# pszenher/Distributional_RL_Decision_and_Control

Measured on AMD Instinct MI355X. Metric: env-steps/sec/GPU @4096 envs; IQN learn-steps/sec at 1/2/4/8 GPUs, higher is better.
Workload: dtype f64-env/bf16-learner; 1 GPU; BASELINE config 2: 4096 envs x 5 robots, 4 buoys, 55m map; fused rollout + AC-IQN learn (B=4096, N=N'=32) per step; envs_per_gpu=4096, robots=5, obstacles=4, global_batch=4096, num_tau=32, parallelism=dp1, hip_graphs=True, dp_rehearsal=False, unroll=2, chained=True, fused_reset=True, env_groups=0, target_after_env=False, push_after_actor=True, target_in_fused=True

## Files before the change

distributional_rl_decision_and_control_amd/_abi.py:

```python
import ctypes as C
import os

import numpy as np

HERE = os.path.dirname(os.path.abspath(__file__))
LIB_PATH = os.environ.get("ASVRL_LIB", os.path.join(HERE, "lib", "libasvrl.so"))
LIB_PATH_F32 = os.path.join(HERE, "lib", "libasvrl_f32.so")
OPERANDS = {"bf16": (LIB_PATH, 2), "f32": (LIB_PATH_F32, 4)}
ABI_VERSION = 29

SELF_DIM, OBJ_DIM, MAX_OBJ = 7, 5, 5
OBS_DIM = 40
TR_DIM = 88
PER_DIM = 48

F_X, F_Y, F_THETA, F_VR0, F_VR1, F_VR2, F_V0, F_V1, F_V2, F_TL, F_TR, F_LP, F_RP, F_GX, F_GY, F_PHI, F_RET = range(17)
NUM_FIELDS = 17

FLAG_DEACTIVATED, FLAG_COLLISION, FLAG_REACH_GOAL, FLAG_COLREGS = 1, 2, 4, 8

INFO_NORMAL, INFO_TOO_LONG, INFO_COLLISION, INFO_REACH_GOAL, INFO_DEACT_COLLISION, INFO_DEACT_GOAL = range(6)
INFO_ABSENT = 255
INFO_STRINGS = {
    INFO_NORMAL: "normal",
# ... 25 lines not shown
    _fields_ = [("n_envs", C.c_int32), ("max_robots", C.c_int32), ("max_obs", C.c_int32), ("max_cores", C.c_int32),
                ("rs", C.c_void_p), ("rflags", C.c_void_p), ("n_robots", C.c_void_p), ("n_obs", C.c_void_p),
                ("n_cores", C.c_void_p), ("ep_ts", C.c_void_p), ("obstacles", C.c_void_p), ("cores", C.c_void_p),
                ("robot_params", C.c_void_p)]


class AsvStepCtl(C.Structure):
    _fields_ = [("is_continuous", C.c_int32), ("do_dynamics", C.c_int32), ("trainer_deactivate", C.c_int32),
                ("noise_mode", C.c_int32), ("seed", C.c_uint64), ("counter", C.c_uint64),
                ("counter_dev", C.c_void_p), ("gamma", C.c_double), ("env_mask", C.c_void_p)]


class AsvStepOut(C.Structure):
    _fields_ = [("obs", C.c_void_p), ("obs64", C.c_void_p), ("obj_cnt", C.c_void_p), ("reward", C.c_void_p),
                ("done", C.c_void_p), ("info", C.c_void_p), ("env_done", C.c_void_p), ("stats", C.c_void_p)]


class AsvResetCfg(C.Structure):
    _fields_ = [("num_robots", C.c_int32), ("num_obs", C.c_int32), ("num_cores", C.c_int32), ("_pad0", C.c_int32),
                ("min_start_goal_dis", C.c_double), ("width", C.c_double), ("height", C.c_double),
                ("clear_r", C.c_double), ("obs_r_lo", C.c_double), ("obs_r_hi", C.c_double), ("v_lo", C.c_double),
                ("v_hi", C.c_double), ("v_rel_max", C.c_double), ("p_rel", C.c_double)]


class AsvEnvLaunch(C.Structure):
    _fields_ = [("layout", C.c_int32), ("block", C.c_int32), ("envs_per_block", C.c_int32), ("max_groups", C.c_int32)]


ENV_LAYOUT_AUTO, ENV_LAYOUT_PAIRS, ENV_LAYOUT_SWEEP = 0, 1, 2


class AsvRollout(C.Structure):
    _fields_ = [("n_steps", C.c_int32), ("hold_done", C.c_int32)] + \
               [(n, C.c_void_p) for n in ("actions", "noise", "reward", "done", "info", "env_done", "obs", "obj_cnt",
                                          "rs", "steps_run")]


class AsvCriticWeights(C.Structure):
    _fields_ = [(n, C.c_void_p) for n in ("wc_frag", "w1_frag", "w2_frag", "w2t_frag", "w1t_frag", "bc", "b1", "b2",
                                          "wo", "bo", "self_w", "self_b", "obj_w", "obj_b", "ae_w", "ae_b")]


class AsvCriticActs(C.Structure):
    _fields_ = [(n, C.c_void_p) for n in ("cos", "h0", "dzc", "h1g", "dz1", "h2", "dz2", "dq", "wout_part")]


class AsvCriticParts(C.Structure):
    _fields_ = [(n, C.c_void_p) for n in ("cos_emb", "hidden", "hidden2", "out", "enc", "aenc")]


_VP, _I32, _I64, _U64, _F, _D = C.c_void_p, C.c_int32, C.c_int64, C.c_uint64, C.c_float, C.c_double
_SCHEDULE = [("step_dev", _VP), ("eps_steps_per_count", _D), ("eps_total", _D), ("eps_fraction", _D),
             ("eps_initial", _D), ("eps_final", _D), ("seed", _U64)]


def fill_schedule(s, step_dev, eps, seed):
    s.step_dev = step_dev.data_ptr() if step_dev is not None else None
    s.eps_steps_per_count, s.eps_total, s.eps_fraction, s.eps_initial, s.eps_final = (float(v) for v in eps)
    s.seed = int(seed) & 0xFFFFFFFFFFFFFFFF


class AsvCriticIO(C.Structure):
    _fields_ = [("F", _VP), ("G", _VP), ("obs", _VP), ("ld_obs", _I64), ("act", _VP), ("ld_act", _I64), ("xb", _VP),
                ("taus", _VP), ("B", _I32), ("N", _I32), ("Np", _I32), ("kappa", C.c_float),
                ("q_targets", _VP), ("q_next", _VP), ("rewards", _VP), ("dones", _VP), ("ld_rd", _I64),
                ("gamma", C.c_float), ("dq", C.c_float), ("q", _VP), ("row_loss", _VP), ("dF", _VP), ("dG", _VP),
                ("dzF", _VP), ("dzG", _VP), ("w_ae", _VP), ("dA", _VP), ("tile_loss", _VP),
                ("loss_scale", C.c_float)]


IQN_MAX_ACTIONS = 32


class AsvIqnHead(C.Structure):
    _fields_ = [("wo_frag", _VP), ("wo", _VP), ("bo", _VP), ("n_actions", _I32)]


class AsvIqnIO(C.Structure):
    _fields_ = [("F", _VP), ("obs", _VP), ("ld_obs", _I64), ("xb", _VP), ("taus", _VP), ("B", _I32), ("N", _I32),
                ("Np", _I32), ("kappa", C.c_float), ("q_next", _VP), ("actions", _VP), ("rewards", _VP),
                ("dones", _VP), ("ld_rd", _I64),
                ("gamma", C.c_float), ("q", _VP), ("row_loss", _VP), ("dzF", _VP), ("dz_out", _VP),
                ("tile_loss", _VP), ("loss_scale", C.c_float), ("act_out", _VP), ("ld_act", _I64)] + _SCHEDULE


class AsvIqnActEx(C.Structure):
    _fields_ = [("cvar", C.c_float), ("robots_per_env", _I32), ("step_add", _I64), ("act_pair", _VP),
                ("rec_row", _VP), ("env_mask", _VP), ("qmean_out", _VP), ("ld_q", _I64)]


class AsvIqnPolicy(C.Structure):
    _fields_ = [("w", AsvCriticWeights), ("head", AsvIqnHead), ("obs_in", _VP)] + _SCHEDULE + \
               [("actions", _VP), ("cvar", C.c_float), ("_pad0", _I32)]


MAX_SUM_SEGS = 24


SUM_PLAIN, SUM_FOLD_ENCODERS = 0, 1


MAX_WGRAD_SEGS = 24
MAX_PACK_SEGS = 16


class AsvPackSeg(C.Structure):
    _fields_ = [("flat_off", _I64), ("image", _VP), ("rows", _I32), ("cols", _I32), ("K", _I32), ("chained", _I32),
                ("transposed", _I32), ("f32", _I32), ("row0", _I32), ("col0", _I32), ("nrep", _I32),
                ("rep_row", _I32), ("rep_col", _I32), ("reserved", _I32)]
WGRAD_MFMA, WGRAD_VEC, WGRAD_SMALL = 0, 1, 2


class AsvWgradSeg(C.Structure):
    _fields_ = [("dz", _VP), ("ldz", _I64), ("x", _VP), ("ldx", _I64), ("R", _I32), ("M", _I32), ("K", _I32),
                ("kind", _I32), ("partial", _VP), ("partial_floats", _I64)]


class AsvActorGradIO(C.Structure):
    _fields_ = [(n, _VP) for n in ("xb", "h0", "h1", "h2", "dout", "dz2", "dz1", "dz0")] + \
               [("B", _I32), ("n_loss", _I32)] + \
               [(n, _VP) for n in ("tile_loss", "loss_out", "w1_grad", "b1_grad", "w2_grad", "b2_grad", "wo_grad",
                                   "bo_grad", "enc_grad", "norm_parts", "step", "work")] + \
               [("work_floats", _I64), ("counters", _VP)]


class AsvPartialSum(C.Structure):
    _fields_ = [("partial", _VP), ("dw", _VP), ("db", _VP), ("groups", _I32), ("nw", _I32), ("nb", _I32),
                ("accumulate", _I32), ("stride", _I32), ("boff", _I32), ("mode", _I32), ("norm", _I32)]


class AsvMlpSrc(C.Structure):
    _fields_ = [(n, _VP) for n in ("self_w", "self_b", "obj_w", "obj_b", "w1", "w2", "ae_w")]


class AsvMlpWeights(C.Structure):
    _fields_ = [(n, _VP) for n in ("enc_frag", "b_enc", "w1_frag", "w2_frag", "w2t_frag", "w1t_frag", "b1", "b2",
                                   "wout", "bout", "ae_frag", "b_ae")] + [("out_scale", C.c_float)]


class AsvMlpIO(C.Structure):
    _fields_ = [("x", _VP), ("ldx", _I64), ("act", _VP), ("lda", _I64), ("n", _I32), ("F", _VP), ("G", _VP),
                ("xb", _VP), ("a_out", _VP), ("ld_aout", _I64), ("a_out64", _VP), ("pre", _VP), ("h0", _VP),
                ("h1", _VP), ("h2", _VP), ("dA", _VP), ("dout", _VP), ("dz2", _VP), ("dz1", _VP), ("dz0", _VP)] + \
        _SCHEDULE


class AsvPolicy(C.Structure):
    _fields_ = [("w", AsvMlpWeights), ("obs_in", _VP)] + _SCHEDULE + [("actions", _VP)]


class AsvAutoReset(C.Structure):
    _fields_ = [("cfg", AsvResetCfg), ("reset_counter", _U64), ("obs_counter", _U64), ("obs_in", _VP),
                ("obs_prev", _VP), ("pushed", _VP), ("resets", _VP)]


class AsvEvalMetrics(C.Structure):
    _fields_ = [("n_steps", _I32), ("n_envs", _I32), ("max_robots", _I32), ("episode_limit", _I32), ("gamma", _D)] + \
               [(n, _VP) for n in ("reward", "info", "rs", "steps_run", "n_robots", "dt", "N", "pc", "length", "ended",
                                   "alive", "deact", "outcome", "ret", "time", "energy")]


HISTORY_ROW_TILE, HISTORY_STEP_TILE = 32, 16
TRAJ_DIM, HISTORY_OBS_DIM = 13, 32
TRAJ_FIELDS = (F_X, F_Y, F_THETA, F_VR0, F_VR1, F_VR2, F_V0, F_V1, F_V2, F_LP, F_RP, F_TL, F_TR)
HISTORY_ARRAYS = ("info", "length", "n_robots", "counts", "offsets", "rs0", "rs", "actions", "obs0", "obs", "cnt0",
                  "obj_cnt", "traj", "act", "obs_out", "cnt_out")


class AsvEvalHistory(C.Structure):
    _fields_ = [("n_steps", _I32), ("n_envs", _I32), ("max_robots", _I32), ("act_steps", _I32)] + \
               [(n, _VP) for n in HISTORY_ARRAYS] + [("traj_rows", _I64), ("act_rows", _I64), ("obs_rows", _I64)]


class AsvNoiseStreams(C.Structure):
    _fields_ = [("n_envs", _I32), ("max_robots", _I32), ("max_obs", _I32), ("_pad0", _I32)] + \
               [(n, _VP) for n in ("n_robots", "n_obs", "rflags", "env_mask", "robot_params", "key", "pos", "has_gauss",
                                   "gauss", "noise_out", "draws_n", "draws_sum", "draws_sq")]


RS_KEY_WORDS = 624


DQN_MAX_ACTIONS = 32


class AsvDqnWeights(C.Structure):
    _fields_ = [("trunk", AsvMlpWeights), ("head_frag", _VP), ("n_actions", _I32), ("_pad0", _I32)]


class AsvDqnActIO(C.Structure):
    _fields_ = [("x", _VP), ("ldx", _I64), ("n", _I32), ("_pad0", _I32), ("act_out", _VP), ("ld_act", _I64),
                ("q_out", _VP)] + _SCHEDULE


class AsvDqnPolicy(C.Structure):
    _fields_ = [("w", AsvDqnWeights), ("obs_in", _VP)] + _SCHEDULE + [("actions", _VP)]


DQN_GRAD_ARRAYS = ("xb", "h0", "h1", "h2", "q_sel", "q_next", "dz_out", "dz2", "dz1", "dz0", "tile_loss")


class AsvDqnGradIO(C.Structure):
    _fields_ = [("rows", _VP), ("ld_rows", _I64), ("B", _I32), ("gamma", _F)] + [(n, _VP) for n in DQN_GRAD_ARRAYS]


class AsvDdpgWeights(C.Structure):
    _fields_ = [("trunk", AsvMlpWeights), ("wae", _VP), ("bae", _VP)]


DDPG_GRAD_ARRAYS = ("xb", "h0", "h1", "p", "h2", "q", "q_next", "dq", "dz2", "dz1", "dzG", "dz0", "tile_loss")


class AsvDdpgGradIO(C.Structure):
    _fields_ = [("rows", _VP), ("ld_rows", _I64), ("B", _I32), ("gamma", _F), ("na", _VP), ("ld_na", _I64)] + \
               [(n, _VP) for n in DDPG_GRAD_ARRAYS]


class AsvDdpgActorIO(C.Structure):
    _fields_ = [("x", _VP), ("ldx", _I64), ("act", _VP), ("lda", _I64), ("B", _I32), ("_pad0", _I32), ("q", _VP),
                ("dA", _VP), ("tile_loss", _VP)]


class AsvSacActorWeights(C.Structure):
    _fields_ = [("trunk", AsvMlpWeights), ("head", _VP), ("bhead", _VP)]


class AsvSacActIO(C.Structure):
    _fields_ = [("x", _VP), ("ldx", _I64), ("n", _I32), ("_pad0", _I32), ("a_out64", _VP), ("eps_in", _VP),
                ("eps_out", _VP)] + _SCHEDULE


class AsvSacPolicy(C.Structure):
    _fields_ = [("w", AsvSacActorWeights), ("obs_in", _VP)] + _SCHEDULE + \
               [("actions", _VP), ("deterministic", _I32), ("_pad0", _I32)]


SAC_ACTOR_ARRAYS = ("xb", "h0", "h1", "h2", "mu", "ls", "sigma", "z", "a", "eps", "logp", "na", "logp_next",
                    "eps_next", "dA", "q_pi", "dhead", "dz2", "dz1", "dz0", "tile_loss")


class AsvSacActorIO(C.Structure):
    _fields_ = [("rows", _VP), ("ld_rows", _I64), ("B", _I32), ("alpha", _F), ("eps_local_in", _VP),
                ("eps_target_in", _VP), ("seed", _U64), ("counter", _U64), ("counter_dev", _VP)] + \
               [(n, _VP) for n in SAC_ACTOR_ARRAYS]


class AsvSacGradIO(C.Structure):
    _fields_ = [("c", AsvDdpgGradIO * 2), ("logp_next", _VP), ("y", _VP), ("alpha", _F), ("_pad0", _I32)]


class AsvSacActorGradIO(C.Structure):
    _fields_ = [("x", _VP), ("ldx", _I64), ("act", _VP), ("lda", _I64), ("B", _I32), ("_pad0", _I32), ("q_pi", _VP),
                ("dA", _VP)]


class AsvSampleArgs(C.Structure):
    _fields_ = [("ring", _VP), ("capacity", _I64), ("ring_state", _VP), ("seed", _U64), ("counter", _U64),
                ("counter_dev", _VP), ("guard", _I64), ("B", _I32), ("tau_sets", _I32), ("tau_n", _I32),
                ("_pad0", _I32), ("out", _VP), ("taus", _VP)]


class AsvPer(C.Structure):
    _fields_ = [("rows", _VP), ("tree", _VP), ("state", _VP), ("t", _VP), ("maxp", _VP), ("dirty", _VP),
                ("capacity", _I64), ("tree_leaves", _I64), ("stride", _I32), ("n_step", _I32), ("discount", _D),
                ("priority_weight", C.c_float), ("priority_exponent", C.c_float), ("deferred", _I32),
                ("_pad0", _I32)]


MAX_NOISY_SEGS = 16


class AsvNoisySeg(C.Structure):
    _fields_ = [(n, _VP) for n in ("mu", "sigma", "eps", "out", "dout", "dmu", "dsigma")]


class AsvNoisySegs(C.Structure):
    _fields_ = [("n", _I32), ("_pad0", _I32), ("off", _I64 * (MAX_NOISY_SEGS + 1)),
                ("seg", AsvNoisySeg * MAX_NOISY_SEGS)]


class AsvRainbowHeadIO(C.Structure):
    _fields_ = [("v", _VP), ("ldv", _I64), ("a", _VP), ("lda", _I64), ("N", _I32), ("atoms", _I32),
                ("actions_n", _I32), ("_pad0", _I32), ("support", _VP), ("act_out", _VP), ("ld_act", _I64),
                ("act_idx", _VP)] + _SCHEDULE + \
               [("p_out", _VP), ("actions", _VP), ("weights", _VP), ("ld_rd", _I64), ("m", _VP), ("loss", _VP),
                ("dv", _VP), ("da", _VP), ("grad_scale", C.c_float), ("_pad1", _I32)]


class AsvRainbowSrc(C.Structure):
    _fields_ = [(n, _VP) for n in ("self_w", "self_b", "obj_w", "obj_b", "w_v1", "b_v1", "w_a1", "b_a1", "w_v2", "b_v2",
                                   "w_a2", "b_a2", "w_vo", "b_vo", "w_ao", "b_ao")]


RAINBOW_IMG_FIELDS = ("enc", "v1", "a1", "v2", "a2", "vo", "mo", "ao")
RAINBOW_BIAS_FIELDS = ("b_enc", "b_v1p", "b_a1p", "b_v2p", "b_a2p", "b_vop", "b_mop", "b_aop")
RAINBOW_IMGT_FIELDS = ("vot", "mot", "aot", "v2t", "a2t", "v1t", "a1t")


class AsvRainbowImg(C.Structure):
    _fields_ = [(n, _VP) for n in RAINBOW_IMG_FIELDS + RAINBOW_BIAS_FIELDS + RAINBOW_IMGT_FIELDS]


class AsvRainbowNetIO(C.Structure):
    _fields_ = [("x", _VP), ("ldx", _I64), ("N", _I32), ("_pad0", _I32), ("support", _VP), ("act_out", _VP),
                ("ld_act", _I64), ("act_idx", _VP)] + _SCHEDULE + \
               [("p_out", _VP), ("actions", _VP), ("weights", _VP), ("ld_rd", _I64), ("m", _VP), ("grad_scale", _F),
                ("_pad1", _I32), ("loss", _VP)] + \
               [(n, _VP) for n in ("xb", "f", "hv1", "ha1", "hv2", "ha2", "dzv", "dza", "dz2v", "dz2a", "dz1v", "dz1a",
                                   "dzf")]


class AsvRainbowActEx(C.Structure):
    _fields_ = [("robots_per_env", _I32), ("_pad0", _I32), ("step_add", _I64), ("act_pair", _VP), ("rec_row", _VP),
                ("env_mask", _VP), ("q_out", _VP), ("ld_q", _I64)]


class AsvRainbowPolicy(C.Structure):
    _fields_ = [("w", AsvRainbowImg), ("support", _VP), ("obs_in", _VP)] + _SCHEDULE + [("actions", _VP)]


ROLLOUTS = {"actor": ("asvrl_policy_rollout", AsvPolicy), "dqn": ("asvrl_dqn_rollout", AsvDqnPolicy),
            "sac": ("asvrl_sac_rollout", AsvSacPolicy), "iqn": ("asvrl_iqn_rollout", AsvIqnPolicy),
            "rainbow": ("asvrl_rainbow_rollout", AsvRainbowPolicy)}


def _rollout_exports():
    head = [C.POINTER(t) for t in (AsvParams, AsvEnvState, AsvStepCtl, AsvStepOut, AsvRollout)]
    tail = [C.POINTER(AsvEnvLaunch), _VP]
    for name, policy in ROLLOUTS.values():
        yield name, C.c_int, head + [C.POINTER(policy)] + tail
        yield name + "_ar", C.c_int, head + [C.POINTER(policy), C.POINTER(AsvAutoReset)] + tail


EXPORTS = [
    ("asvrl_env_step", C.c_int, [C.POINTER(AsvParams), C.POINTER(AsvEnvState), _VP, _VP, C.POINTER(AsvStepCtl),
                                 C.POINTER(AsvStepOut), _VP]),
    ("asvrl_env_step_ex", C.c_int, [C.POINTER(AsvParams), C.POINTER(AsvEnvState), _VP, _VP, C.POINTER(AsvStepCtl),
                                    C.POINTER(AsvStepOut), C.POINTER(AsvEnvLaunch), _VP]),
    ("asvrl_env_rollout", C.c_int, [C.POINTER(AsvParams), C.POINTER(AsvEnvState), C.POINTER(AsvStepCtl),
                                    C.POINTER(AsvStepOut), C.POINTER(AsvRollout), C.POINTER(AsvEnvLaunch), _VP]),
    ("asvrl_env_reset", C.c_int, [C.POINTER(AsvParams), C.POINTER(AsvEnvState), C.POINTER(AsvResetCfg), _VP, _U64,
                                  _U64, _VP, _VP]),
    ("asvrl_env_reset_observe", C.c_int, [C.POINTER(AsvParams), C.POINTER(AsvEnvState), C.POINTER(AsvResetCfg), _VP,
                                          _U64, _U64, _VP, C.POINTER(AsvStepCtl), C.POINTER(AsvStepOut), _VP]),
    ("asvrl_current_field", C.c_int, [_VP, _I32, _D, _VP, _I32, _VP, _VP]),
    ("asvrl_quantile_huber", C.c_int, [_VP, _VP, _VP, _I32, _I32, _I32, _F, _F, _VP, _VP, _VP, _VP]),
    ("asvrl_c51_project", C.c_int, [_VP, _VP, _VP, _VP, _I32, _I32, _F, _F, _F, _F, _VP, _VP]),
    ("asvrl_c51_project_ex", C.c_int, [_VP, _VP, C.c_int64, _VP, C.c_int64, _VP, _I32, _I32, _F, _F, _F, _F, _VP,
                                       _VP]),
    ("asvrl_critic_pack", C.c_int, [_VP, _VP, _VP, C.POINTER(AsvCriticWeights), _VP]),
    ("asvrl_critic_forward", C.c_int, [C.POINTER(AsvCriticWeights), C.POINTER(AsvCriticIO), _VP]),
    ("asvrl_critic_train", C.c_int, [C.POINTER(AsvCriticWeights), C.POINTER(AsvCriticIO), C.POINTER(AsvCriticActs),
                                     _VP]),
    ("asvrl_critic_actor_grad", C.c_int, [C.POINTER(AsvCriticWeights), C.POINTER(AsvCriticIO), _VP]),
    ("asvrl_iqn_pack", C.c_int, [_VP, _VP, _VP, _VP, C.POINTER(AsvCriticWeights), C.POINTER(AsvIqnHead), _VP]),
    ("asvrl_iqn_forward_max", C.c_int, [C.POINTER(AsvCriticWeights), C.POINTER(AsvIqnHead), C.POINTER(AsvIqnIO), _VP]),
    ("asvrl_iqn_train", C.c_int, [C.POINTER(AsvCriticWeights), C.POINTER(AsvIqnHead), C.POINTER(AsvIqnIO),
                                  C.POINTER(AsvCriticActs), _VP]),
    ("asvrl_iqn_act", C.c_int, [C.POINTER(AsvCriticWeights), C.POINTER(AsvIqnHead), C.POINTER(AsvIqnIO), _VP]),
    ("asvrl_replay_push", C.c_int, [_VP, _VP, _VP, _VP, _I32, _VP, _VP, _I32, _VP, _I64, _VP, _VP, _VP]),
    ("asvrl_replay_push_ex", C.c_int, [_VP, _VP, _VP, _VP, _I32, _I64, _VP, _VP, _I32, _VP, _I64, _VP, _VP, _VP,
                                       _VP, _VP]),
    ("asvrl_replay_sample", C.c_int, [_VP, _I64, _VP, _VP, _I32, _U64, _U64, _VP, _I64, _VP, _VP, _VP, _I32, _I32,
                                      _VP]),
    ("asvrl_replay_write_rows", C.c_int, [_VP, _VP, _I32, _VP, _VP]),
    ("asvrl_per_push", C.c_int, [C.POINTER(AsvPer), _VP, _VP, _VP, _I32, _VP, _VP, _I32, _VP]),
    ("asvrl_per_sample", C.c_int, [C.POINTER(AsvPer), _I32, _VP, _U64, _U64, _VP, _VP, _VP, _VP]),
    ("asvrl_per_update", C.c_int, [C.POINTER(AsvPer), _VP, _VP, _I32, _I32, _VP]),
    ("asvrl_per_push_ex", C.c_int, [C.POINTER(AsvPer), _VP, _VP, _VP, _I32, _VP, _VP, _I32, _VP, _VP]),
    ("asvrl_per_update_ex", C.c_int, [C.POINTER(AsvPer), _VP, _VP, _I32, _I32, _VP, _VP, _VP]),
    ("asvrl_per_sample_ex", C.c_int, [C.POINTER(AsvPer), _I32, _VP, _U64, _U64, _VP, _VP, _VP, _VP, _VP]),
    ("asvrl_per_normalise", C.c_int, [_VP, _VP, _I32, _VP]),
    ("asvrl_noisy_compose", C.c_int, [C.POINTER(AsvNoisySegs), _I32, _VP]),
    ("asvrl_noisy_backward_norm_parts", _I32, [C.POINTER(AsvNoisySegs)]),
    ("asvrl_noisy_backward_norm", C.c_int, [C.POINTER(AsvNoisySegs), _VP, _VP]),
    ("asvrl_noisy_reset", C.c_int, [C.POINTER(AsvNoisySegs), _VP, _VP, _U64, _VP, _VP]),
    ("asvrl_rainbow_act", C.c_int, [C.POINTER(AsvRainbowHeadIO), _VP]),
    ("asvrl_rainbow_pick", C.c_int, [C.POINTER(AsvRainbowHeadIO), _VP]),
    ("asvrl_rainbow_loss", C.c_int, [C.POINTER(AsvRainbowHeadIO), _VP]),
    ("asvrl_rainbow_pack", C.c_int, [C.POINTER(AsvRainbowSrc), C.POINTER(AsvRainbowImg), _VP]),
    ("asvrl_rainbow_net_act", C.c_int, [C.POINTER(AsvRainbowImg), C.POINTER(AsvRainbowNetIO), _VP]),
    ("asvrl_rainbow_net_argmax", C.c_int, [C.POINTER(AsvRainbowImg), C.POINTER(AsvRainbowNetIO), _VP]),
    ("asvrl_rainbow_net_pick", C.c_int, [C.POINTER(AsvRainbowImg), C.POINTER(AsvRainbowNetIO), _VP]),
    ("asvrl_rainbow_net_train", C.c_int, [C.POINTER(AsvRainbowImg), C.POINTER(AsvRainbowNetIO), _VP]),
    ("asvrl_adam_clip", C.c_int, [_VP, _VP, _VP, _VP, _I64, _VP, _F, _F, _F, _F, _F, _VP, _VP, _VP]),
    ("asvrl_linear_wgrad_workspace", _I64, [_I32, _I32]),
    ("asvrl_critic_wout_groups", _I32, [_I32, _I32]),
    ("asvrl_critic_fused_groups", _I32, [_I32, _I32]),
    ("asvrl_critic_fused_variant", _I32, [_I32]),
    ("asvrl_critic_train_fused", C.c_int, [C.POINTER(AsvCriticWeights), C.POINTER(AsvCriticIO),
                                           C.POINTER(AsvCriticParts), _VP]),
    ("asvrl_critic_train_fused_tq", C.c_int, [C.POINTER(AsvCriticWeights), C.POINTER(AsvCriticIO),
                                              C.POINTER(AsvCriticParts), C.POINTER(AsvCriticWeights),
                                              C.POINTER(AsvCriticIO), _VP]),
    ("asvrl_iqn_train_fused", C.c_int, [C.POINTER(AsvCriticWeights), C.POINTER(AsvIqnHead), C.POINTER(AsvIqnIO),
                                        C.POINTER(AsvCriticParts), _VP]),
    ("asvrl_iqn_train_fused_tq", C.c_int, [C.POINTER(AsvCriticWeights), C.POINTER(AsvIqnHead), C.POINTER(AsvIqnIO),
                                           C.POINTER(AsvCriticParts), C.POINTER(AsvCriticWeights),
                                           C.POINTER(AsvIqnHead), C.POINTER(AsvIqnIO), _VP]),
    ("asvrl_linear_wgrad_groups", _I32, [_I32, _I32, _I32]),
    ("asvrl_linear_wgrad_vec_groups", _I32, [_I32]),
    ("asvrl_linear_wgrad_partial", C.c_int, [_VP, _I64, _VP, _I64, _I32, _I32, _I32, _VP, _I64, _VP, _VP]),
    ("asvrl_linear_wgrad_multi", C.c_int, [_VP, _I32, _VP, _VP]),
    ("asvrl_linear_wgrad_vec_partial", C.c_int, [_VP, _I64, _VP, _I64, _I32, _I32, _VP, _I64, _VP, _VP]),
    ("asvrl_small_wgrad_partial", C.c_int, [_VP, _I64, _VP, _I64, _I32, _I32, _I32, _VP, _I64, _VP, _VP]),
    ("asvrl_partial_sums", C.c_int, [_VP, _I32, _VP]),
    ("asvrl_partial_sums_norm", C.c_int, [_VP, _I32, _VP, _VP, _VP]),
    ("asvrl_partial_sums_norm_parts", _I32, [_VP, _I32]),
    ("asvrl_actor_grads_workspace", _I64, [_I32]),
    ("asvrl_actor_grads_counters", _I32, []),
    ("asvrl_actor_grads_norm_parts", _I32, []),
    ("asvrl_actor_grads", C.c_int, [C.POINTER(AsvActorGradIO), _VP]),
    ("asvrl_adam_step", C.c_int, [_VP, _VP, _VP, _VP, _I64, _VP, _F, _F, _F, _F, _F, _VP, _VP, _I32, _VP]),
    ("asvrl_adam_step_pack", C.c_int, [_VP, _VP, _VP, _VP, _I64, _VP, _F, _F, _F, _F, _F, _VP, _VP, _I32, _VP, _I32,
                                       _VP, _VP]),
    ("asvrl_target_update_pack", C.c_int, [_VP, _VP, _I64, _F, _F, _VP, _I64, _VP, _I32, _VP]),
    ("asvrl_linear_wgrad", C.c_int, [_VP, _I64, _VP, _I64, _I32, _I32, _I32, _VP, _VP, _I32, _VP, _I64, _VP]),
    ("asvrl_linear_wgrad_vec", C.c_int, [_VP, _I64, _VP, _I64, _I32, _I32, _VP, _VP, _I32, _VP, _I64, _VP]),
    ("asvrl_mlp_pack", C.c_int, [C.POINTER(AsvMlpSrc), C.POINTER(AsvMlpWeights), _VP]),
    ("asvrl_mlp_encode", C.c_int, [C.POINTER(AsvMlpWeights), C.POINTER(AsvMlpIO), _VP]),
    ("asvrl_actor_forward", C.c_int, [C.POINTER(AsvMlpWeights), C.POINTER(AsvMlpIO), _I32, _VP]),
    ("asvrl_actor_backward", C.c_int, [C.POINTER(AsvMlpWeights), C.POINTER(AsvMlpIO), _VP]),
    ("asvrl_learn_prologue", C.c_int, [C.POINTER(AsvSampleArgs), C.POINTER(AsvMlpWeights), C.POINTER(AsvMlpIO),
                                       C.POINTER(AsvMlpWeights), _VP, _VP]),
    ("asvrl_encoder_fold", C.c_int, [_VP, _VP, _VP, _VP, _VP, _VP, _I32, _VP]),
    ("asvrl_small_wgrad", C.c_int, [_VP, _I64, _VP, _I64, _I32, _I32, _I32, _VP, _VP, _I32, _VP, _I64, _VP]),
    ("asvrl_last_error", C.c_char_p, []),
    ("asvrl_abi_version", C.c_int, []),
    ("asvrl_operand_bytes", C.c_int32, []),
    ("asvrl_struct_sizes", None, [C.c_void_p]),
    ("asvrl_rollout_struct_size", _I64, []),
    *_rollout_exports(),
    ("asvrl_policy_struct_size", _I64, []),
    ("asvrl_env_rollout_ar", C.c_int, [C.POINTER(AsvParams), C.POINTER(AsvEnvState), C.POINTER(AsvStepCtl),
                                       C.POINTER(AsvStepOut), C.POINTER(AsvRollout), C.POINTER(AsvAutoReset),
                                       C.POINTER(AsvEnvLaunch), _VP]),
    ("asvrl_autoreset_struct_size", _I64, []),
    ("asvrl_replay_push_window", C.c_int, [_VP, _VP, _VP, _VP, _I32, _I64, _VP, _VP, _I32, _I32, _VP, _VP, _I64, _VP,
                                           _VP, _VP, _VP, _I64, _VP]),
    ("asvrl_eval_metrics", C.c_int, [C.POINTER(AsvEvalMetrics), _VP]),
    ("asvrl_eval_metrics_struct_size", _I64, []),
    ("asvrl_eval_history_count", C.c_int, [C.POINTER(AsvEvalHistory), _VP]),
    ("asvrl_eval_history_pack", C.c_int, [C.POINTER(AsvEvalHistory), _VP]),
    ("asvrl_eval_history_struct_size", _I64, []),
    ("asvrl_eval_history_step_tile", _I32, []),
    ("asvrl_noise_streams", C.c_int, [C.POINTER(AsvParams), C.POINTER(AsvNoiseStreams), _VP]),
    ("asvrl_noise_streams_host", C.c_int, [C.POINTER(AsvParams), C.POINTER(AsvNoiseStreams), _VP]),
    ("asvrl_noise_streams_struct_size", _I64, []),
    ("asvrl_dqn_pack", C.c_int, [C.POINTER(AsvMlpSrc), _VP, C.POINTER(AsvDqnWeights), _VP]),
    ("asvrl_dqn_act", C.c_int, [C.POINTER(AsvDqnWeights), C.POINTER(AsvDqnActIO), _VP]),
    ("asvrl_dqn_grad", C.c_int, [C.POINTER(AsvDqnWeights), C.POINTER(AsvDqnWeights), C.POINTER(AsvDqnGradIO), _VP]),
    ("asvrl_dqn_weights_struct_size", _I64, []),
    ("asvrl_dqn_act_struct_size", _I64, []),
    ("asvrl_dqn_grad_struct_size", _I64, []),
    ("asvrl_dqn_policy_struct_size", _I64, []),
    ("asvrl_ddpg_grad", C.c_int, [C.POINTER(AsvDdpgWeights), C.POINTER(AsvDdpgWeights), C.POINTER(AsvDdpgGradIO),
                                  _VP]),
    ("asvrl_ddpg_actor_grad", C.c_int, [C.POINTER(AsvDdpgWeights), C.POINTER(AsvDdpgActorIO), _VP]),
    ("asvrl_ddpg_weights_struct_size", _I64, []),
    ("asvrl_ddpg_grad_struct_size", _I64, []),
    ("asvrl_ddpg_actor_struct_size", _I64, []),
    ("asvrl_sac_act", C.c_int, [C.POINTER(AsvSacActorWeights), C.POINTER(AsvSacActIO), _VP]),
    ("asvrl_sac_actor_forward", C.c_int, [C.POINTER(AsvSacActorWeights), C.POINTER(AsvSacActorWeights),
                                          C.POINTER(AsvSacActorIO), _VP]),
    ("asvrl_sac_grad", C.c_int, [C.POINTER(AsvDdpgWeights), C.POINTER(AsvDdpgWeights), C.POINTER(AsvDdpgWeights),
                                 C.POINTER(AsvDdpgWeights), C.POINTER(AsvSacGradIO), _VP]),
    ("asvrl_sac_actor_grad", C.c_int, [C.POINTER(AsvDdpgWeights), C.POINTER(AsvDdpgWeights),
                                       C.POINTER(AsvSacActorGradIO), _VP]),
    ("asvrl_sac_actor_backward", C.c_int, [C.POINTER(AsvSacActorWeights), C.POINTER(AsvSacActorIO), _VP]),
    ("asvrl_sac_actor_weights_struct_size", _I64, []),
    ("asvrl_sac_act_struct_size", _I64, []),
    ("asvrl_sac_actor_struct_size", _I64, []),
    ("asvrl_sac_grad_struct_size", _I64, []),
    ("asvrl_sac_actor_grad_struct_size", _I64, []),
    ("asvrl_sac_policy_struct_size", _I64, []),
    ("asvrl_iqn_act_ex", C.c_int, [C.POINTER(AsvCriticWeights), C.POINTER(AsvIqnHead), C.POINTER(AsvIqnIO),
                                   C.POINTER(AsvIqnActEx), _VP]),
    ("asvrl_iqn_act_ex_struct_size", _I64, []),
    ("asvrl_iqn_policy_struct_size", _I64, []),
    ("asvrl_rainbow_net_act_ex", C.c_int, [C.POINTER(AsvRainbowImg), C.POINTER(AsvRainbowNetIO),
                                           C.POINTER(AsvRainbowActEx), _VP]),
    ("asvrl_rainbow_act_ex_struct_size", _I64, []),
    ("asvrl_rainbow_policy_struct_size", _I64, []),
    ("asvrl_per_push_window", C.c_int, [C.POINTER(AsvPer), _VP, _VP, _VP, _I32, _VP, _VP, _I32, _VP, _I64, _VP]),
]

_libs = {}


class AsvrlError(RuntimeError):
    pass


def lib(operands="bf16"):
    L = _libs.get(operands)
    if L is not None:
        return L
    if operands not in OPERANDS:
        raise ValueError(f"operands must be one of {sorted(OPERANDS)}")
    path, nbytes = OPERANDS[operands]
    if not os.path.exists(path):
        raise AsvrlError(f"{os.path.basename(path)} not found at {path}: build it with "
                         "`python -m distributional_rl_decision_and_control_amd.build` (hipcc, gfx950). "
                         "There is no CPU fallback.")
    L = C.CDLL(path)
    for name, res, args in EXPORTS:
        fn = getattr(L, name)
        fn.restype = res
        fn.argtypes = args
    v = L.asvrl_abi_version()
    if v != ABI_VERSION:
        raise AsvrlError(f"{os.path.basename(path)} ABI {v} != expected {ABI_VERSION}; rebuild")
    if L.asvrl_operand_bytes() != nbytes:
        raise AsvrlError(f"{path}: operand element of {L.asvrl_operand_bytes()} bytes, expected {nbytes}")
    _libs[operands] = L
    return L


def operand_dtype(operands="bf16"):
    import torch
    return {"bf16": torch.bfloat16, "f32": torch.float32}[operands]


def check(rc, what="", L=None):
    if rc != 0:
        msg = (L if L is not None else lib()).asvrl_last_error().decode(errors="replace")
        raise AsvrlError(f"{what} failed ({rc}): {msg}")


def ptr(t):
    if t is None:
        return None
    return C.c_void_p(t.data_ptr())


def stream_ptr(stream=None):
    import torch
    s = stream if stream is not None else torch.cuda.current_stream()
    return C.c_void_p(s.cuda_stream)


def params_from(robot=None, env=None, max_obj_num=5, episode_limit=1000):
    p = AsvParams()
    src = robot if robot is not None else _DefaultRobot()
    p.dt = float(src.dt)
    p.N = int(src.N)
    p.episode_limit = int(episode_limit)
    p.length, p.width = float(src.length), float(src.width)
    p.r = float(src.r)
    p.goal_dis = float(src.goal_dis)
    p.min_thrust, p.max_thrust = float(src.min_thrust), float(src.max_thrust)
    p.m, p.Izz = float(src.m), float(src.Izz)
    for n in _HYDRO:
        setattr(p, n, float(getattr(src, n)))
    import warnings
    warnings.filterwarnings("ignore", category=PendingDeprecationWarning, message=".*matrix subclass.*")
    M_RB = np.matrix([[src.m, 0.0, 0.0], [0.0, src.m, 0.0], [0.0, 0.0, src.Izz]])
    M_A = -1.0 * np.matrix([[src.xDotU, 0.0, 0.0], [0.0, src.yDotV, src.yDotR], [0.0, src.nDotV, src.nDotR]])
    A = M_RB + M_A
    P = np.asarray(np.linalg.inv(A.transpose() * A) * A.transpose(), dtype=np.float64).reshape(-1)
    for k in range(9):
        p.P[k] = float(P[k])
    for k in range(5):
        p.left_thrust_change[k] = float(src.left_thrust_change[k])
        p.right_thrust_change[k] = float(src.right_thrust_change[k])
    per = src.perception if hasattr(src, "perception") else src
    p.range, p.angle = float(per.range), float(per.angle)
    p.pos_std, p.vel_std = float(per.pos_std), float(per.vel_std)
    p.r_kappa, p.r_mean_ratio = float(per.r_kappa), float(per.r_mean_ratio)
    p.max_obj_num = int(getattr(per, "max_obj_num", max_obj_num))
    e = env if env is not None else _DefaultEnv()
    p.timestep_penalty = float(e.timestep_penalty)
    p.COLREGs_penalty = float(e.COLREGs_penalty)
    p.collision_penalty = float(e.collision_penalty)
    p.goal_reward = float(e.goal_reward)
    p.core_r = float(e.r)
    return p


class _DefaultRobot:
    dt, N, length, width = 0.05, 10, 5.0, 2.5
    r = 0.5 * np.sqrt(5.0 ** 2 + 2.5 ** 2)
    goal_dis, min_thrust, max_thrust = 2.0, -500.0, 1000.0
    m, Izz = 400, 450
    xDotU, yDotV, yDotR, nDotR, nDotV = 20, 0, 0, -980, 0
    xU, xUU, yV, yVV, yR, yRV, yVR, yRR = -100, -150, -100, -150, 0, 0, 0, 0
    nR, nRR, nV, nVV, nRV, nVR = -980, -950, 0, 0, 0, 0
    left_thrust_change = right_thrust_change = [0.0, -500.0, -1000.0, 500.0, 1000.0]
    range, angle, max_obj_num = 20.0, 2 * np.pi, 5
    pos_std, vel_std, r_kappa, r_mean_ratio = 0.05, 0.05, 1.0, 0.8
# ... 6 lines not shown
```

distributional_rl_decision_and_control_amd/csrc/asvrl_env.hip:

```cpp
#include <type_traits>

#include "asvrl_common.h"
#include "asvrl_vonmises_k1.h"
#include "asvrl_actor_tile.h"
#include "asvrl_dqn_tile.h"
#include "asvrl_sac_tile.h"

namespace asvrl {
namespace {

constexpr int kBlock = 256;
__host__ __device__ constexpr int step_block(int R) { return R <= 64 ? 64 : 256; }
__host__ __device__ constexpr size_t policy_rows_offset(size_t carve_bytes) { return (carve_bytes + 15) & ~size_t{15}; }
constexpr int kMaxCores = 16;
constexpr int kMaxCoresStep = 4096;

struct Regs {
  double x, y, th, vr0, vr1, vr2, v0, v1, v2, tl, tr, lp, rp;
};

struct PairsArgs {
  AsvParams p;
  AsvEnvState s;
  AsvStepCtl ctl;
// ... 406 lines not shown
  int cnt = -1;
  Cand t0{INFINITY, 0, 0, 0, 0, 0}, t1 = t0, t2 = t0, t3 = t0, t4 = t0;
  double so0 = 0, so1 = 0, so2 = 0, so3 = 0, so4 = 0;
  if (active) {
    double sn, cs;
    sincos(r.th, &sn, &cs);
    const double tx = -(cs * r.x + sn * r.y);
    const double ty = -(-sn * r.x + cs * r.y);
    so0 = (cs * gx + sn * gy) + tx;
    so1 = (-sn * gx + cs * gy) + ty;
    so2 = cs * r.v0 + sn * r.v1;
    so3 = -sn * r.v0 + cs * r.v1;
    so4 = r.v2;
    if (sqrt((gx - r.x) * (gx - r.x) + (gy - r.y) * (gy - r.y)) <= P.goal_dis) reach = true;

    int nkept = 0;
    const int no = s.n_obs[e];
    const int base = le * R;
    const uint64_t ctr = ctl.counter + (ctl.counter_dev != nullptr ? *ctl.counter_dev : 0ull);
    const int ncand = no + nrob;
    const bool full_circle = 0.5 * P.angle >= kPi;
    for (int k = 0; k < ncand; ++k) {
      double ox, oy, orad, vx0, vy0;
      int slot;
      if (k < no) {
        const double* ob = sob + (static_cast<size_t>(le) * O + k) * 3;
        ox = ob[0];
        oy = ob[1];
        orad = ob[2];
        vx0 = 0.0;
        vy0 = 0.0;
        slot = k;
      } else {
        const int j = k - no;
        if (j == i || soff[base + j]) continue;
        ox = sx[base + j];
        oy = sy[base + j];
        orad = PR ? s.robot_params[static_cast<size_t>(e) * R + j].r : p.r;
        vx0 = sv0[base + j];
        vy0 = sv1[base + j];
        slot = O + j;
      }
      double n0, n1, n2, n3, n4;
      draw_noise<-1>(P, ctl, ctr, noise, idx, slot, O + R, n0, n1, n2, n3, n4);
      const double pxn = ox + n0, pyn = oy + n1;
      const double vxn = vx0 + n2, vyn = vy0 + n3;
      const double rn = P.r_mean_ratio * orad + (1 - P.r_mean_ratio) * n4 / kPi * orad;
      const double qx = (cs * pxn + sn * pyn) + tx, qy = (-sn * pxn + cs * pyn) + ty;
      const double qn = sqrt(qx * qx + qy * qy);
      if (qn > P.range + rn) continue;
      if (!full_circle) {
        const double ang = atan2(qy, qx);
        if (ang < -0.5 * P.angle || ang > 0.5 * P.angle) continue;
      }
      if (!coll) {
        const double d = sqrt((r.x - ox) * (r.x - ox) + (r.y - oy) * (r.y - oy)) - orad - P.r;
        if (d <= 0.0) coll = true;
      }
      Cand cd{qn - rn - P.r, qx, qy, cs * vxn + sn * vyn, -sn * vxn + cs * vyn, rn};
      cswap(cd.key < t0.key, cd, t0);
      cswap(cd.key < t1.key, cd, t1);
      cswap(cd.key < t2.key, cd, t2);
      cswap(cd.key < t3.key, cd, t3);
      cswap(cd.key < t4.key, cd, t4);
      ++nkept;
    }
    cnt = nkept < P.max_obj_num ? nkept : P.max_obj_num;
    if (cnt > 0) apply = colregs(P.r, cs, sn, r.v0, r.v1, t0.a, t0.b, t0.c, t0.d, t0.e, phi);
    if (!apply && cnt > 1) apply = colregs(P.r, cs, sn, r.v0, r.v1, t1.a, t1.b, t1.c, t1.d, t1.e, phi);
    if (!apply && cnt > 2) apply = colregs(P.r, cs, sn, r.v0, r.v1, t2.a, t2.b, t2.c, t2.d, t2.e, phi);
    if (!apply && cnt > 3) apply = colregs(P.r, cs, sn, r.v0, r.v1, t3.a, t3.b, t3.c, t3.d, t3.e, phi);
    if (!apply && cnt > 4) apply = colregs(P.r, cs, sn, r.v0, r.v1, t4.a, t4.b, t4.c, t4.d, t4.e, phi);
  }

  const StepResult res = step_result(p, ctl, exists, deact, active, ep_ts, fl, coll, reach, apply, phi, reward,
                                     exists ? s.rs[ASVRL_F_RET * NT + idx] : 0.0);
  if (ctl.trainer_deactivate && ctl.do_dynamics && exists && !(res.nfl & ASVRL_FLAG_DEACTIVATED))
    atomicAdd(&salive[le], 1);

  if (exists) {
    double* rs = s.rs;
    if (ctl.do_dynamics) {
      rs[ASVRL_F_X * NT + idx] = r.x;
      rs[ASVRL_F_Y * NT + idx] = r.y;
      rs[ASVRL_F_THETA * NT + idx] = r.th;
      rs[ASVRL_F_VR0 * NT + idx] = r.vr0;
      rs[ASVRL_F_VR1 * NT + idx] = r.vr1;
      rs[ASVRL_F_VR2 * NT + idx] = r.vr2;
      rs[ASVRL_F_V0 * NT + idx] = r.v0;
      rs[ASVRL_F_V1 * NT + idx] = r.v1;
      rs[ASVRL_F_V2 * NT + idx] = r.v2;
      rs[ASVRL_F_TL * NT + idx] = r.tl;
      rs[ASVRL_F_TR * NT + idx] = r.tr;
      rs[ASVRL_F_RET * NT + idx] = res.ret;
    }
    rs[ASVRL_F_PHI * NT + idx] = phi;
    s.rflags[idx] = res.nfl;
  }
  if (env_on && i < R) {
    float4* o4 = reinterpret_cast<float4*>(out.obs + idx * ASVRL_OBS_DIM);
    const bool a = active;
    const float m0 = (a && cnt > 0) ? 1.f : 0.f, m1 = (a && cnt > 1) ? 1.f : 0.f,
                m2 = (a && cnt > 2) ? 1.f : 0.f, m3 = (a && cnt > 3) ? 1.f : 0.f,
                m4 = (a && cnt > 4) ? 1.f : 0.f;
    auto f = [](double v, float m) { return m != 0.f ? static_cast<float>(v) : 0.f; };
    const float sf = a ? 1.f : 0.f;
    o4[0] = make_float4(f(so0, sf), f(so1, sf), f(so2, sf), f(so3, sf));
    o4[1] = make_float4(f(so4, sf), f(r.tl, sf), f(r.tr, sf), f(t0.a, m0));
    o4[2] = make_float4(f(t0.b, m0), f(t0.c, m0), f(t0.d, m0), f(t0.e, m0));
    o4[3] = make_float4(f(t1.a, m1), f(t1.b, m1), f(t1.c, m1), f(t1.d, m1));
    o4[4] = make_float4(f(t1.e, m1), f(t2.a, m2), f(t2.b, m2), f(t2.c, m2));
    o4[5] = make_float4(f(t2.d, m2), f(t2.e, m2), f(t3.a, m3), f(t3.b, m3));
    o4[6] = make_float4(f(t3.c, m3), f(t3.d, m3), f(t3.e, m3), f(t4.a, m4));
    o4[7] = make_float4(f(t4.b, m4), f(t4.c, m4), f(t4.d, m4), f(t4.e, m4));
    o4[8] = make_float4(m0, m1, m2, m3);
    o4[9] = make_float4(m4, 0.f, 0.f, 0.f);
    if (out.obs64 != nullptr) {
      double* o = out.obs64 + idx * 32;
      const double v[32] = {so0, so1, so2, so3, so4, r.tl, r.tr,
                            t0.a, t0.b, t0.c, t0.d, t0.e, t1.a, t1.b, t1.c, t1.d, t1.e,
                            t2.a, t2.b, t2.c, t2.d, t2.e, t3.a, t3.b, t3.c, t3.d, t3.e,
                            t4.a, t4.b, t4.c, t4.d, t4.e};
#pragma unroll
      for (int k = 0; k < 32; ++k) {
        const bool keep = a && (k < 7 || (k - 7) / 5 < cnt);
        o[k] = keep ? v[k] : 0.0;
      }
    }
    out.obj_cnt[idx] = static_cast<int8_t>(exists ? cnt : -1);
    out.reward[idx] = res.reward;
    out.done[idx] = res.done;
    out.info[idx] = res.info;
  }
  __syncthreads();
  if (env_on && i == 0 && ctl.do_dynamics) env_end(p, s, ctl, out, e, ep_ts, nrob, salive[le], NT);
}

#ifndef ASVRL_ENV_PAIRS_WPE
#define ASVRL_ENV_PAIRS_WPE 4
#endif
constexpr int kResetWaves = 4;
constexpr int kResetMaxR = 32;
constexpr int kResetMaxO = 32;
struct ResetLds {
  double rob[4][kResetMaxR];
  double core[kMaxCores][4];
  double obs[kResetMaxO][3];
};
__device__ __forceinline__ void reset_env(const AsvParams& p, const AsvEnvState& s, const AsvResetCfg& cfg, int e,
                                          uint64_t seed, uint64_t ctr, int lane, ResetLds& W);
__host__ __device__ constexpr size_t autoreset_lds(int blk, int epb) {
  return static_cast<size_t>(blk / 64) * sizeof(ResetLds) + sizeof(int) * static_cast<size_t>(epb);
}
enum : int { kPolNone = 0, kPolActor = 1, kPolDqn = 2, kPolSac = 3 };
template <int POL> struct PolicyOf { using type = AsvPolicy; };
template <> struct PolicyOf<kPolDqn> { using type = AsvDqnPolicy; };
template <> struct PolicyOf<kPolSac> { using type = AsvSacPolicy; };
__device__ __forceinline__ const AsvMlpWeights& trunk_of(const AsvPolicy& p) { return p.w; }
__device__ __forceinline__ const AsvMlpWeights& trunk_of(const AsvDqnPolicy& p) { return p.w.trunk; }
__device__ __forceinline__ const AsvMlpWeights& trunk_of(const AsvSacPolicy& p) { return p.w.trunk; }
template <int BLOCK, int NM, bool DYN = true, bool ROLL = false, int POL = kPolNone, bool AR = false>
__device__ __forceinline__ void env_pairs_block(KArg<PairsArgs> A, int epb, int bid, unsigned char* smem,
                                                KArg<AsvRollout> RO = nullptr,
                                                KArg<typename PolicyOf<POL>::type> PI = nullptr,
                                                atile::ActorLds* AL = nullptr, KArg<AsvAutoReset> RS = nullptr,
                                                unsigned char* ar_lds = nullptr,
                                                sactile::SacHeadLds* HL = nullptr) {
  static_assert(POL == kPolNone || ROLL, "the policy runs inside the rollout's step loop");
  static_assert(!AR || ROLL, "the auto-reset runs inside the rollout's step loop");
  const int R = A->s.max_robots;
  const int O = A->s.max_obs;
  const int S = O + R;
  const int nrb = epb * R;
  const int npairs = nrb * S;
  const int nslot = npairs > 5 * nrb ? npairs : 5 * nrb;
  int tid = threadIdx.x;

  double* sx = reinterpret_cast<double*>(smem);
  double* sy = sx + nrb;
  double* sv0 = sy + nrb;
  double* sv1 = sv0 + nrb;
  double* scs = sv1 + nrb;
  double* ssn = scs + nrb;
  double* stx = ssn + nrb;
  double* sty = stx + nrb;
  double* pk = sty + nrb;
  double* sob = pk + nslot;
  using VmT = typename std::conditional<NM == 2, float, double>::type;
  VmT* pvm = reinterpret_cast<VmT*>(sob + static_cast<size_t>(epb) * O * 3);
  int* salive = reinterpret_cast<int*>(pvm + npairs);
  int* sno = salive + epb;
  int* snr = sno + epb;
  int* swt = snr + epb;
  unsigned short* skept = reinterpret_cast<unsigned short*>(swt + BLOCK / kWave);
  unsigned short* sitem = skept + 5 * nrb;
  unsigned char* pfl = reinterpret_cast<unsigned char*>(sitem + 5 * nrb);
  unsigned char* soff = pfl + nslot;
  unsigned char* sact = soff + nrb;
  signed char* scnt = reinterpret_cast<signed char*>(sact + nrb);
  float* sobs = reinterpret_cast<float*>(smem + policy_rows_offset(reinterpret_cast<unsigned char*>(scnt + nrb) - smem));
  double* sa64 = reinterpret_cast<double*>(sobs + static_cast<size_t>(nrb) * ASVRL_OBS_DIM);
  const size_t row0 = POL != kPolNone ? static_cast<size_t>(bid) * nrb : 0;

  const bool rlane = tid < nrb;
  int le = tid / R;
  const int i = tid - le * R;
  const int e = bid * epb + le;
  const bool lane_env = rlane && e < A->s.n_envs;
  const bool env_on0 = lane_env && (A->ctl.env_mask == nullptr || A->ctl.env_mask[e] != 0);
  if (A->ctl.env_mask != nullptr && !__syncthreads_or(env_on0 ? 1 : 0)) return;
  int nrob = lane_env ? A->s.n_robots[e] : 0;
  bool exists0 = env_on0 && i < nrob;
  const size_t NT = static_cast<size_t>(A->s.n_envs) * R;
  size_t idx = static_cast<size_t>(e) * R + i;
  uint8_t flv = exists0 ? A->s.rflags[idx] : 0;
  int ep_ts = env_on0 ? A->s.ep_ts[e] : 0;
  Regs r{};
  double gx = 0, gy = 0, phi = 0.0, ret = 0.0;
  bool on = env_on0;
  int taken = 0;
  int nreset = 0;
  bool rstl = false;
  const int n_steps = ROLL ? RO->n_steps : 1;
  const bool hold = ROLL && RO->hold_done != 0;
  auto load_state = [&] {
    const double* rs = A->s.rs;
    r.x = rs[ASVRL_F_X * NT + idx];
    r.y = rs[ASVRL_F_Y * NT + idx];
    r.th = rs[ASVRL_F_THETA * NT + idx];
    r.vr0 = rs[ASVRL_F_VR0 * NT + idx];
    r.vr1 = rs[ASVRL_F_VR1 * NT + idx];
    r.vr2 = rs[ASVRL_F_VR2 * NT + idx];
    r.v0 = rs[ASVRL_F_V0 * NT + idx];
    r.v1 = rs[ASVRL_F_V1 * NT + idx];
    r.v2 = rs[ASVRL_F_V2 * NT + idx];
    r.tl = rs[ASVRL_F_TL * NT + idx];
    r.tr = rs[ASVRL_F_TR * NT + idx];
    r.lp = rs[ASVRL_F_LP * NT + idx];
    r.rp = rs[ASVRL_F_RP * NT + idx];
    gx = rs[ASVRL_F_GX * NT + idx];
    gy = rs[ASVRL_F_GY * NT + idx];
  };
  auto store_state = [&] {
    double* rs = A->s.rs;
    rs[ASVRL_F_X * NT + idx] = r.x;
    rs[ASVRL_F_Y * NT + idx] = r.y;
    rs[ASVRL_F_THETA * NT + idx] = r.th;
    rs[ASVRL_F_VR0 * NT + idx] = r.vr0;
    rs[ASVRL_F_VR1 * NT + idx] = r.vr1;
    rs[ASVRL_F_VR2 * NT + idx] = r.vr2;
    rs[ASVRL_F_V0 * NT + idx] = r.v0;
    rs[ASVRL_F_V1 * NT + idx] = r.v1;
    rs[ASVRL_F_V2 * NT + idx] = r.v2;
    rs[ASVRL_F_TL * NT + idx] = r.tl;
    rs[ASVRL_F_TR * NT + idx] = r.tr;
  };
  if constexpr (ROLL) {
    if (exists0) {
      load_state();
      phi = A->s.rs[ASVRL_F_PHI * NT + idx];
      ret = A->s.rs[ASVRL_F_RET * NT + idx];
    }
  }
  if constexpr (POL != kPolNone) {
    atile::stage_actor<BLOCK>(*AL, trunk_of(kref(PI)), tid);
    if constexpr (POL == kPolSac) sactile::stage_head<BLOCK>(*HL, kref(PI).w, tid);
    constexpr int kRowV = ASVRL_OBS_DIM / 4;
    const float4* src = reinterpret_cast<const float4*>(PI->obs_in);
    for (int k = tid; k < nrb * kRowV; k += BLOCK) {
      const size_t g = row0 + k / kRowV;
      reinterpret_cast<float4*>(sobs)[k] = g < NT ? src[g * kRowV + k % kRowV] : make_float4(0.f, 0.f, 0.f, 0.f);
    }
    __syncthreads();
  }
  if constexpr (AR) {
    const KArg<AsvAutoReset> Q = kfresh(RS);
    const float* src0 = POL != kPolNone ? PI->obs_in : Q->obs_in;
    if (env_on0 && Q->obs_prev != nullptr) {
      const float4* src = reinterpret_cast<const float4*>(src0 + idx * ASVRL_OBS_DIM);
      float4* dst = reinterpret_cast<float4*>(Q->obs_prev + idx * ASVRL_OBS_DIM);
#pragma unroll
      for (int k = 0; k < ASVRL_OBS_DIM / 4; ++k) dst[k] = src[k];
    }
  }

  for (int t = 0; t < n_steps; ++t) {
  if constexpr (ROLL) {
    asm volatile("" : "+v"(tid), "+v"(le), "+v"(idx));
    if (hold && !__syncthreads_or(on ? 1 : 0)) break;
  }
  bool obsp = false;
  [[maybe_unused]] phases:
  if constexpr (AR) asm volatile("" : "+v"(tid), "+v"(le), "+v"(idx));
  const bool env_on = ROLL ? (on && (!obsp || rstl)) : env_on0;
  const bool exists = ROLL ? (exists0 && env_on) : exists0;
  const uint8_t fl = flv;
  const bool deact = (fl & ASVRL_FLAG_DEACTIVATED) != 0;
  const bool active = exists && !deact;
  bool coll = (fl & ASVRL_FLAG_COLLISION) != 0;
  bool reach = (fl & ASVRL_FLAG_REACH_GOAL) != 0;
  double reward = 0.0;
  const bool wlast = !ROLL || hold || t == n_steps - 1;
  auto rec_row = [&] {
    AsvStepOut o{};
    if constexpr (ROLL) {
      const KArg<AsvRollout> Q = kfresh(RO);
      const size_t t0 = static_cast<size_t>(t) * NT;
      o.obs = Q->obs != nullptr ? Q->obs + t0 * ASVRL_OBS_DIM : nullptr;
      o.obj_cnt = Q->obj_cnt != nullptr ? Q->obj_cnt + t0 : nullptr;
      o.reward = Q->reward != nullptr ? Q->reward + t0 : nullptr;
      o.done = Q->done != nullptr ? Q->done + t0 : nullptr;
      o.info = Q->info != nullptr ? Q->info + t0 : nullptr;
    }
    return o;
  };
  auto each_out = [&](KArg<PairsArgs> Ak, auto&& f) {
    if (wlast) f(kref(Ak).out, std::false_type{}, size_t{0});
    if constexpr (AR) {
      if (!obsp) f(rec_row(), std::true_type{}, size_t{0});
    } else if constexpr (ROLL) {
      f(rec_row(), std::true_type{}, size_t{0});
    }
    if constexpr (POL != kPolNone) {
      AsvStepOut o{};
      o.obs = sobs;
      f(o, std::true_type{}, row0);
    }
    if constexpr (AR) {
      const KArg<AsvAutoReset> Q = kfresh(RS);
      AsvStepOut o{};
      if (Q->obs_prev != nullptr && t + 1 < n_steps)
        o.obs = Q->obs_prev + static_cast<size_t>(t + 1) * NT * ASVRL_OBS_DIM;
      f(o, std::true_type{}, size_t{0});
    }
  };

  if constexpr (AR) {
    if (obsp) goto acted;
  }
  if constexpr (POL == kPolActor) {
    const KArg<AsvPolicy> P = kfresh(PI);
    const uint64_t step = (P->step_dev != nullptr ? static_cast<uint64_t>(*P->step_dev) : 0ull) + static_cast<uint64_t>(t);
    const int ln = tid & (kWave - 1), wv = __builtin_amdgcn_readfirstlane(tid / kWave);
    for (int tile = wv; tile * 32 < nrb; tile += BLOCK / kWave) {
      asm volatile("" ::: "memory");
      const int lr = tile * 32 + (ln & 31);
      const bool valid = lr < nrb;
      frag8 bx[2];
      float mk[atile::kObjN];
      atile::load_obs(sobs, ASVRL_OBS_DIM, valid ? lr : nrb - 1, ln >> 5, bx, mk);
      float z0, z1, a0, a1;
      atile::actor_chain<atile::MLP_ACT>(kref(P).w, AsvMlpIO{}, *AL, 0, false, ln, bx, mk, z0, z1, a0, a1);
      if (valid && ln < 32)
        atile::explore(step, atile::EpsSchedule{P->eps_steps_per_count, P->eps_total, P->eps_fraction, P->eps_initial,
                                                P->eps_final},
                       P->seed, static_cast<int>(row0 + lr), a0, a1, sa64[2 * lr], sa64[2 * lr + 1]);
    }
    __syncthreads();
    if (env_on && P->actions != nullptr) {
      double* rec = P->actions + (static_cast<size_t>(t) * NT + idx) * 2;
      rec[0] = sa64[2 * tid];
      rec[1] = sa64[2 * tid + 1];
    }
  } else if constexpr (POL == kPolDqn) {
    const KArg<AsvDqnPolicy> P = kfresh(PI);
    const uint64_t step = (P->step_dev != nullptr ? static_cast<uint64_t>(*P->step_dev) : 0ull) + static_cast<uint64_t>(t);
    const int ln = tid & (kWave - 1), wv = __builtin_amdgcn_readfirstlane(tid / kWave);
    for (int tile = wv; tile * 32 < nrb; tile += BLOCK / kWave) {
      asm volatile("" ::: "memory");
      const int lr = tile * 32 + (ln & 31);
      const bool valid = lr < nrb;
      frag8 bx[2];
      float mk[atile::kObjN];
      atile::load_obs(sobs, ASVRL_OBS_DIM, valid ? lr : nrb - 1, ln >> 5, bx, mk);
      float q[16];
      dqtile::dqn_q_tile<atile::MLP_ACT>(kref(P).w, AsvMlpIO{}, *AL, 0, false, ln, bx, mk, q);
      float best;
      int bi;
      const int nact = P->w.n_actions;
      dqtile::dqn_argmax(q, ln >> 5, nact, best, bi);
      if (valid && ln < 32) {
        const int act = dqtile::dqn_explore(step, atile::EpsSchedule{P->eps_steps_per_count, P->eps_total, P->eps_fraction,
                                                                     P->eps_initial, P->eps_final},
                                            P->seed, static_cast<int>(row0 + lr), bi, nact);
        sa64[2 * lr] = static_cast<double>(act);
        sa64[2 * lr + 1] = 0.0;
      }
    }
    __syncthreads();
    if (env_on && P->actions != nullptr) {
      double* rec = P->actions + (static_cast<size_t>(t) * NT + idx) * 2;
      rec[0] = sa64[2 * tid];
      rec[1] = sa64[2 * tid + 1];
    }
  } else if constexpr (POL == kPolSac) {
    const KArg<AsvSacPolicy> P = kfresh(PI);
    const uint64_t step = (P->step_dev != nullptr ? static_cast<uint64_t>(*P->step_dev) : 0ull) + static_cast<uint64_t>(t);
    const int ln = tid & (kWave - 1), wv = __builtin_amdgcn_readfirstlane(tid / kWave);
    for (int tile = wv; tile * 32 < nrb; tile += BLOCK / kWave) {
      asm volatile("" ::: "memory");
      const int lr = tile * 32 + (ln & 31);
      const bool valid = lr < nrb;
      const int rr = valid ? lr : nrb - 1;
      float eps[atile::kNa] = {0.f, 0.f};
      if (P->deterministic == 0)
        sactile::sac_eps(sactile::kSacActStream, static_cast<int>(row0 + rr), step, P->seed, eps[0], eps[1]);
      frag8 bx[2];
      float mk[atile::kObjN];
      atile::load_obs(sobs, ASVRL_OBS_DIM, rr, ln >> 5, bx, mk);
      float h2v[8][8];
      atile::trunk_chain<atile::MLP_ACT>(kref(P).w.trunk, AsvMlpIO{}, *AL, 0, false, ln, bx, mk, h2v);
      sactile::SacSample o;
      sactile::sac_head<false>(*HL, P->w.trunk.out_scale, h2v, ln, eps, o);
      if (valid && ln < 32)
        atile::explore(step, atile::EpsSchedule{P->eps_steps_per_count, P->eps_total, P->eps_fraction, P->eps_initial,
                                                P->eps_final},
                       P->seed, static_cast<int>(row0 + lr), o.a[0], o.a[1], sa64[2 * lr], sa64[2 * lr + 1]);
    }
    __syncthreads();
    if (env_on && P->actions != nullptr) {
      double* rec = P->actions + (static_cast<size_t>(t) * NT + idx) * 2;
      rec[0] = sa64[2 * tid];
      rec[1] = sa64[2 * tid + 1];
    }
  }
  [[maybe_unused]] acted:

  {
    if constexpr (!ROLL) {
      r = Regs{};
      gx = 0;
      gy = 0;
      if (exists) load_state();
    }
    if (active && (DYN && A->ctl.do_dynamics) && !obsp) {
      const double d_before = sqrt((gx - r.x) * (gx - r.x) + (gy - r.y) * (gy - r.y));
      const int nc = A->s.n_cores[e];
      const double* cores = A->s.cores + static_cast<size_t>(e) * A->s.max_cores * 4;
      const double* act = POL != kPolNone ? sa64 + 2 * tid : A->actions + (ROLL ? static_cast<size_t>(t) * 2 * NT : 0) + 2 * idx;
      robot_act(ParamsKArg{&A->p}, r, act[0], act[1], A->ctl.is_continuous, cores,
                nc < A->s.max_cores ? nc : A->s.max_cores);
      const double d_after = sqrt((gx - r.x) * (gx - r.x) + (gy - r.y) * (gy - r.y));
      reward = 0.0;
      reward += A->p.timestep_penalty;
      reward += d_before - d_after;
    }
    if constexpr (!ROLL) {
      if (exists && (DYN && A->ctl.do_dynamics)) store_state();
    }
    double so0 = 0, so1 = 0, so2 = 0, so3 = 0, so4 = 0;
    if (rlane) {
      sx[tid] = r.x;
      sy[tid] = r.y;
      sv0[tid] = r.v0;
      sv1[tid] = r.v1;
      soff[tid] = exists ? (deact ? 1 : 0) : 1;
      sact[tid] = active ? 1 : 0;
    }
    if (active) {
      double sn, cs;
      sincos(r.th, &sn, &cs);
      const double tx = -(cs * r.x + sn * r.y);
      const double ty = -(-sn * r.x + cs * r.y);
      scs[tid] = cs;
      ssn[tid] = sn;
      stx[tid] = tx;
      sty[tid] = ty;
      so0 = (cs * gx + sn * gy) + tx;
      so1 = (-sn * gx + cs * gy) + ty;
      so2 = cs * r.v0 + sn * r.v1;
      so3 = -sn * r.v0 + cs * r.v1;
      so4 = r.v2;
      if (sqrt((gx - r.x) * (gx - r.x) + (gy - r.y) * (gy - r.y)) <= A->p.goal_dis) reach = true;
    }
    if (env_on) {
      const bool a = active;
      each_out(A, [&](const AsvStepOut& o, auto opt, size_t base) {
        if (!opt || o.obs != nullptr) {
          float* of = o.obs + (idx - base) * ASVRL_OBS_DIM;
          *reinterpret_cast<float4*>(of) = a ? make_float4(static_cast<float>(so0), static_cast<float>(so1),
                                                            static_cast<float>(so2), static_cast<float>(so3))
                                             : make_float4(0.f, 0.f, 0.f, 0.f);
          of[4] = a ? static_cast<float>(so4) : 0.f;
          of[5] = a ? static_cast<float>(r.tl) : 0.f;
          of[6] = a ? static_cast<float>(r.tr) : 0.f;
        }
        if (o.obs64 != nullptr) {
          double* ob = o.obs64 + idx * 32;
          ob[0] = a ? so0 : 0.0;
          ob[1] = a ? so1 : 0.0;
          ob[2] = a ? so2 : 0.0;
          ob[3] = a ? so3 : 0.0;
          ob[4] = a ? so4 : 0.0;
          ob[5] = a ? r.tl : 0.0;
          ob[6] = a ? r.tr : 0.0;
        }
      });
    }
  }
  if (env_on) {
    if (!ROLL || t == 0 || obsp) {
      const int no = A->s.n_obs[e];
      for (int k = i; k < O; k += R) {
        const double* ob = A->s.obstacles + (static_cast<size_t>(e) * O + k) * 3;
        double* dst = sob + (static_cast<size_t>(le) * O + k) * 3;
        if (k < no) {
          dst[0] = ob[0];
          dst[1] = ob[1];
          dst[2] = ob[2];
        }
      }
      if (i == 0) {
        sno[le] = no;
        snr[le] = nrob;
      }
    }
    if (i == 0) salive[le] = 0;
  }
  __syncthreads();
  A = kfresh(A);

  auto candidate = [&](int qe, int qi, int c, double& ox, double& oy, double& orad, double& vx0, double& vy0) {
    if (c < O) {
      if (c >= sno[qe]) return false;
      const double* ob = sob + (static_cast<size_t>(qe) * O + c) * 3;
      ox = ob[0];
      oy = ob[1];
      orad = ob[2];
      vx0 = 0.0;
      vy0 = 0.0;
      return true;
    }
    const int j = c - O;
    if (!(j < snr[qe] && j != qi && !soff[qe * R + j])) return false;
    ox = sx[qe * R + j];
    oy = sy[qe * R + j];
    orad = A->p.r;
    vx0 = sv0[qe * R + j];
    vy0 = sv1[qe * R + j];
    return true;
  };
  uint64_t ctr = A->ctl.counter + (A->ctl.counter_dev != nullptr ? *A->ctl.counter_dev : 0ull) +
                 (ROLL ? static_cast<uint64_t>(t) : 0ull);
  if constexpr (AR) {
    if (obsp) ctr = ctr - A->ctl.counter + RS->obs_counter;
  }
  const size_t noise_t = (ROLL && NM == 0) ? static_cast<size_t>(t) * NT * S * 5 : 0;
  const bool full_circle = 0.5 * A->p.angle >= kPi;

  const KArg<PairsArgs> A_loop = A;
  for (int q = tid; q < npairs; q += BLOCK) {
    const KArg<PairsArgs> A = kfresh(A_loop);
    const int qr = q / S;
    const int c = q - qr * S;
    const int qe = qr / R;
    const int qi = qr - qe * R;
    unsigned char flag = 0;
    double key = INFINITY;
    double ox = 0, oy = 0, orad = 0, vx0 = 0, vy0 = 0;
    if (sact[qr] && candidate(qe, qi, c, ox, oy, orad, vx0, vy0)) {
      const size_t qidx = static_cast<size_t>(bid * epb + qe) * R + qi;
      double n0, n1, n2, n3, n4;
      draw_noise<NM>(kref(A).p, kref(A).ctl, ctr, A->noise + noise_t, qidx, c, S, n0, n1, n2, n3, n4);
      pvm[q] = static_cast<VmT>(n4);
      const double cs = scs[qr], sn = ssn[qr], tx = stx[qr], ty = sty[qr];
      const double pxn = ox + n0, pyn = oy + n1;
      const double rn = A->p.r_mean_ratio * orad + (1 - A->p.r_mean_ratio) * n4 / kPi * orad;
      const double qx = (cs * pxn + sn * pyn) + tx, qy = (-sn * pxn + cs * pyn) + ty;
      const double qn = sqrt(qx * qx + qy * qy);
      bool det = qn <= A->p.range + rn;
      if (det && !full_circle) {
        const double ang = atan2(qy, qx);
        det = !(ang < -0.5 * A->p.angle || ang > 0.5 * A->p.angle);
      }
      if (det) {
        flag = 1;
        const double rx = sx[qr], ry = sy[qr];
        const double d = sqrt((rx - ox) * (rx - ox) + (ry - oy) * (ry - oy)) - orad - A->p.r;
        if (d <= 0.0) flag |= 2;
        key = qn - rn - A->p.r;
      }
    }
    pk[q] = key;
    pfl[q] = flag;
  }
  __syncthreads();
  A = kfresh(A);

  int cnt = -1;
  if (active) {
    double k0 = INFINITY, k1 = INFINITY, k2 = INFINITY, k3 = INFINITY, k4 = INFINITY;
    int c0 = 0, c1 = 0, c2 = 0, c3 = 0, c4 = 0;
    int nkept = 0;
    const int q0 = tid * S;
    for (int c = 0; c < S; ++c) {
      const unsigned char f = pfl[q0 + c];
      if (!(f & 1)) continue;
      if (f & 2) coll = true;
      double kc = pk[q0 + c];
      int cc = c;
      auto ins = [&](double& kk, int& ck) {
        if (kc < kk) {
          const double tk = kk;
          const int tc = ck;
          kk = kc;
          ck = cc;
          kc = tk;
          cc = tc;
        }
      };
      ins(k0, c0);
      ins(k1, c1);
      ins(k2, c2);
      ins(k3, c3);
      ins(k4, c4);
      ++nkept;
    }
    cnt = nkept < A->p.max_obj_num ? nkept : A->p.max_obj_num;
    unsigned short* kp = skept + 5 * tid;
    kp[0] = static_cast<unsigned short>(c0);
    kp[1] = static_cast<unsigned short>(c1);
    kp[2] = static_cast<unsigned short>(c2);
    kp[3] = static_cast<unsigned short>(c3);
    kp[4] = static_cast<unsigned short>(c4);
  }
  if (rlane) scnt[tid] = static_cast<signed char>(cnt);
  const int lane = tid & (kWave - 1);
  int kin = cnt > 0 ? cnt : 0;
#pragma unroll
  for (int d = 1; d < kWave; d <<= 1) {
    const int t = __shfl_up(kin, d);
    if (lane >= d) kin += t;
  }
  if (lane == kWave - 1) swt[tid / kWave] = kin;
  __syncthreads();
  A = kfresh(A);
  int nitem = 0, ibase = 0;
#pragma unroll
  for (int w = 0; w < BLOCK / kWave; ++w) {
    ibase += w < tid / kWave ? swt[w] : 0;
    nitem += swt[w];
  }
  if (cnt > 0) {
    const int off = ibase + kin - cnt;
    for (int k = 0; k < cnt; ++k) sitem[off + k] = static_cast<unsigned short>(5 * tid + k);
  }
  __syncthreads();
  A = kfresh(A);

  const KArg<PairsArgs> A_loop4 = A;
  for (int it = tid; it < nitem; it += BLOCK) {
    const KArg<PairsArgs> A = kfresh(A_loop4);
    const int kq = sitem[it];
    const int qr = kq / 5;
    const int k = kq - 5 * qr;
    const int qe = qr / R;
    const int qi = qr - qe * R;
    const int e2 = bid * epb + qe;
    unsigned char cf = 0;
    double ph = 0.0;
    {
      const size_t qidx = static_cast<size_t>(e2) * R + qi;
      double ra, rb, rc, rd, re;
      {
        const int c = skept[kq];
        double ox = 0, oy = 0, orad = 0, vx0 = 0, vy0 = 0;
        candidate(qe, qi, c, ox, oy, orad, vx0, vy0);
        double n0, n1, n2, n3, n4 = static_cast<double>(pvm[qr * S + c]);
        draw_noise<NM, false>(kref(A).p, kref(A).ctl, ctr, A->noise + noise_t, qidx, c, S, n0, n1, n2, n3, n4);
        const double cs = scs[qr], sn = ssn[qr], tx = stx[qr], ty = sty[qr];
        const double pxn = ox + n0, pyn = oy + n1;
        const double vxn = vx0 + n2, vyn = vy0 + n3;
        const double rn = A->p.r_mean_ratio * orad + (1 - A->p.r_mean_ratio) * n4 / kPi * orad;
        ra = (cs * pxn + sn * pyn) + tx;
        rb = (-sn * pxn + cs * pyn) + ty;
        rc = cs * vxn + sn * vyn;
        rd = -sn * vxn + cs * vyn;
        re = rn;
        if (!(sqrt(rc * rc + rd * rd) < 0.5)) {
          bool ev;
          const bool hit = colregs_ev(A->p.r, cs, sn, sv0[qr], sv1[qr], ra, rb, rc, rd, re, ph, ev);
          cf = static_cast<unsigned char>((ev ? 1 : 0) | (hit ? 2 : 0));
        }
      }
      each_out(A, [&](const AsvStepOut& o, auto opt, size_t base) {
        if (!opt || o.obs != nullptr) {
          float* of = o.obs + (qidx - base) * ASVRL_OBS_DIM + 7 + 5 * k;
          of[0] = static_cast<float>(ra);
          of[1] = static_cast<float>(rb);
          of[2] = static_cast<float>(rc);
          of[3] = static_cast<float>(rd);
          of[4] = static_cast<float>(re);
        }
        if (o.obs64 != nullptr) {
          double* ob = o.obs64 + qidx * 32 + 7 + 5 * k;
          ob[0] = ra;
          ob[1] = rb;
          ob[2] = rc;
          ob[3] = rd;
          ob[4] = re;
        }
      });
    }
    pfl[kq] = cf;
    pk[kq] = ph;
  }
  __syncthreads();
  A = kfresh(A);

  bool apply = false;
  if constexpr (!ROLL) phi = exists ? A->s.rs[ASVRL_F_PHI * NT + idx] : 0.0;
  for (int k = 0; k < cnt; ++k) {
    const unsigned char f = pfl[5 * tid + k];
    if (f & 1) phi = pk[5 * tid + k];
    if (f & 2) {
      apply = true;
      break;
    }
  }
  if constexpr (!ROLL) ret = exists ? A->s.rs[ASVRL_F_RET * NT + idx] : 0.0;
  AsvStepCtl cobs{};
  if constexpr (AR) {
    if (!obsp) {
      cobs.do_dynamics = A->ctl.do_dynamics;
      cobs.trainer_deactivate = A->ctl.trainer_deactivate;
      cobs.gamma = A->ctl.gamma;
    }
  }
  const StepResult res = step_result(kref(A).p, AR ? cobs : kref(A).ctl, exists, deact, active, ep_ts, fl, coll, reach, apply, phi, reward,
                                     ret);
  if (A->ctl.trainer_deactivate && (DYN && A->ctl.do_dynamics) && !obsp && exists && !(res.nfl & ASVRL_FLAG_DEACTIVATED))
    atomicAdd(&salive[le], 1);
  if constexpr (AR) {
    if (!obsp && RS->pushed != nullptr) {
      const unsigned long long bal = __ballot(exists && cnt >= 0);
      if ((tid & (kWave - 1)) == 0 && bal != 0) atomicAdd(RS->pushed + t, static_cast<int32_t>(__popcll(bal)));
    }
  }
  if (exists) {
    if constexpr (!ROLL) {
      if ((DYN && A->ctl.do_dynamics)) A->s.rs[ASVRL_F_RET * NT + idx] = res.ret;
      A->s.rs[ASVRL_F_PHI * NT + idx] = phi;
      A->s.rflags[idx] = res.nfl;
    } else {
      ret = res.ret;
      flv = res.nfl;
      pk[5 * tid] = res.ret;
      pfl[5 * tid] = res.nfl;
    }
  }
  if (env_on) {
    const bool a = active;
    each_out(A, [&](const AsvStepOut& o, auto opt, size_t base) {
      if (!opt || o.obs != nullptr) {
        float4* o4 = reinterpret_cast<float4*>(o.obs + (idx - base) * ASVRL_OBS_DIM);
        for (int k = cnt > 0 ? cnt : 0; k < 5; ++k) {
          float* of = o.obs + (idx - base) * ASVRL_OBS_DIM + 7 + 5 * k;
          of[0] = 0.f;
          of[1] = 0.f;
          of[2] = 0.f;
          of[3] = 0.f;
          of[4] = 0.f;
        }
        o4[8] = make_float4((a && cnt > 0) ? 1.f : 0.f, (a && cnt > 1) ? 1.f : 0.f, (a && cnt > 2) ? 1.f : 0.f,
                            (a && cnt > 3) ? 1.f : 0.f);
        o4[9] = make_float4((a && cnt > 4) ? 1.f : 0.f, 0.f, 0.f, 0.f);
      }
      if (o.obs64 != nullptr) {
        for (int k = cnt > 0 ? cnt : 0; k < 5; ++k) {
          double* ob = o.obs64 + idx * 32 + 7 + 5 * k;
          ob[0] = 0.0;
          ob[1] = 0.0;
          ob[2] = 0.0;
          ob[3] = 0.0;
          ob[4] = 0.0;
        }
      }
      if (!opt || o.obj_cnt != nullptr) o.obj_cnt[idx] = static_cast<int8_t>(exists ? cnt : -1);
      if (!opt || o.reward != nullptr) o.reward[idx] = res.reward;
      if (!opt || o.done != nullptr) o.done[idx] = res.done;
      if (!opt || o.info != nullptr) o.info[idx] = res.info;
    });
  }
  __syncthreads();
  A = kfresh(A);
  if constexpr (AR) {
    if (obsp) {
      if (exists && t == n_steps - 1) {
        A->s.rs[ASVRL_F_PHI * NT + idx] = phi;
        A->s.rflags[idx] = flv;
      }
      continue;
    }
  }
  if constexpr (!ROLL) {
    if (env_on && i == 0 && (DYN && A->ctl.do_dynamics)) env_end(kref(A).p, kref(A).s, kref(A).ctl, kref(A).out, e, ep_ts, nrob, salive[le], NT);
  } else {
    const KArg<AsvRollout> Q = kfresh(RO);
    bool end = false;
    if (env_on && A->ctl.trainer_deactivate && (hold || AR || i == 0))
      end = (ep_ts >= A->p.episode_limit) || salive[le] == 0;
    if (env_on && i == 0) {
      env_end_from(kref(A).p, kref(A).s, kref(A).ctl, kref(A).out, e, ep_ts, nrob, salive[le],
                   [&](int j) { return pk[5 * (le * R + j)]; }, [&](int j) { return pfl[5 * (le * R + j)]; });
      if (Q->env_done != nullptr) Q->env_done[static_cast<size_t>(t) * A->s.n_envs + e] = end ? 1 : 0;
    }
    if (exists && (t == n_steps - 1 || ((hold || AR) && end))) {
      store_state();
      A->s.rs[ASVRL_F_RET * NT + idx] = ret;
      A->s.rs[ASVRL_F_PHI * NT + idx] = phi;
      A->s.rflags[idx] = flv;
    }
    if (exists && Q->rs != nullptr) {
      double* q = Q->rs + static_cast<size_t>(t) * ASVRL_NUM_FIELDS * NT + idx;
      const double v[ASVRL_NUM_FIELDS] = {r.x, r.y, r.th, r.vr0, r.vr1, r.vr2, r.v0, r.v1, r.v2, r.tl, r.tr,
                                          r.lp, r.rp, gx, gy, phi, ret};
#pragma unroll
      for (int f = 0; f < ASVRL_NUM_FIELDS; ++f) q[f * NT] = v[f];
    }
    if (env_on) {
      ++ep_ts;
      ++taken;
    }
    if (hold && end) on = false;
    if constexpr (AR) {
      rstl = env_on && end;
      int* srst = reinterpret_cast<int*>(ar_lds + (BLOCK / kWave) * sizeof(ResetLds));
      if (rlane && i == 0) srst[le] = rstl ? 1 : 0;
      if (!__syncthreads_or(rstl ? 1 : 0)) continue;
      __syncthreads();
      {
        const KArg<AsvAutoReset> Z = kfresh(RS);
        const uint64_t rctr = Z->reset_counter + (A->ctl.counter_dev != nullptr ? *A->ctl.counter_dev : 0ull) +
                              static_cast<uint64_t>(t);
        const int wv = __builtin_amdgcn_readfirstlane(tid / kWave);
        ResetLds* W = reinterpret_cast<ResetLds*>(ar_lds);
        for (int qe = wv; qe < epb; qe += BLOCK / kWave)
          if (__builtin_amdgcn_readfirstlane(srst[qe]) != 0)
            reset_env(kref(A).p, kref(A).s, kref(Z).cfg, bid * epb + qe, A->ctl.seed, rctr, tid & (kWave - 1), W[wv]);
      }
      __syncthreads();
      A = kfresh(A);
      if (rstl) {
        nrob = A->s.n_robots[e];
        exists0 = i < nrob;
        r = Regs{};
        gx = 0;
        gy = 0;
        phi = 0.0;
        ret = 0.0;
        flv = 0;
        if (exists0) {
          load_state();
          phi = A->s.rs[ASVRL_F_PHI * NT + idx];
          ret = A->s.rs[ASVRL_F_RET * NT + idx];
          flv = A->s.rflags[idx];
        }
        ep_ts = 0;
        if (i == 0) ++nreset;
      }
      obsp = true;
      goto phases;
    }
  }
  }
  if constexpr (ROLL) {
    if (lane_env && i == 0 && RO->steps_run != nullptr) RO->steps_run[e] = taken;
  }
  if constexpr (AR) {
    if (lane_env && i == 0 && RS->resets != nullptr) RS->resets[e] = nreset;
  }
}


__device__ __forceinline__ int xcd_group(int x, int n) {
  constexpr int kXcd = 8;
  const int q = n / kXcd, rr = n % kXcd, xcd = x % kXcd, k = x / kXcd;
  return (xcd < rr ? xcd * (q + 1) : rr * (q + 1) + (xcd - rr) * q) + k;
}
template <int BLOCK, int NM>
__global__ __launch_bounds__(BLOCK) __attribute__((amdgpu_waves_per_eu(NM == 1 ? 1 : ASVRL_ENV_PAIRS_WPE))) void env_pairs_kernel(PairsArgs) {
  extern __shared__ __attribute__((aligned(16))) unsigned char smem[];
  const KArg<PairsArgs> A = kargs<PairsArgs>();
  env_pairs_block<BLOCK, NM>(A, A->epb,
                             A->group0 + xcd_group(static_cast<int>(blockIdx.x), static_cast<int>(gridDim.x)), smem);
}

struct NoPolicy {};
template <int> struct Absent {};
template <class Pol, bool AR>
struct WindowArgs {
  PairsArgs k;
  AsvRollout ro;
  [[no_unique_address]] std::conditional_t<std::is_same_v<Pol, NoPolicy>, Absent<0>, Pol> pi;
  [[no_unique_address]] std::conditional_t<AR, AsvAutoReset, Absent<1>> ar;
  [[no_unique_address]] std::conditional_t<AR, int, Absent<2>> ar_off;
};
static_assert(sizeof(WindowArgs<NoPolicy, false>) == sizeof(PairsArgs) + sizeof(AsvRollout) &&
                  sizeof(WindowArgs<AsvPolicy, false>) == sizeof(WindowArgs<NoPolicy, false>) + sizeof(AsvPolicy) &&
                  sizeof(WindowArgs<NoPolicy, true>) == sizeof(WindowArgs<NoPolicy, false>) + sizeof(AsvAutoReset) + 8,
              "absent members take no room in the kernarg segment");

#ifndef ASVRL_ENV_ROLLOUT_WPE
#define ASVRL_ENV_ROLLOUT_WPE 2
#endif
template <int BLOCK, int NM, bool AR>
__global__ __launch_bounds__(BLOCK) __attribute__((amdgpu_waves_per_eu(NM == 1 ? 1 : ASVRL_ENV_ROLLOUT_WPE))) void env_rollout_kernel(WindowArgs<NoPolicy, AR>) {
  static_assert(!AR || NM != 0, "the auto-reset is Philox noise only");
  extern __shared__ __attribute__((aligned(16))) unsigned char smem[];
  const KArg<WindowArgs<NoPolicy, AR>> RA = kargs<WindowArgs<NoPolicy, AR>>();
  const int epb = RA->k.epb, bid = RA->k.group0 + xcd_group(static_cast<int>(blockIdx.x), static_cast<int>(gridDim.x));
  if constexpr (AR)
    env_pairs_block<BLOCK, NM, true, true, kPolNone, true>(&RA->k, epb, bid, smem, &RA->ro, nullptr, nullptr,
                                                           &RA->ar, smem + RA->ar_off);
  else
    env_pairs_block<BLOCK, NM, true, true>(&RA->k, epb, bid, smem, &RA->ro);
}

#ifndef ASVRL_ENV_POLICY_WPE
#define ASVRL_ENV_POLICY_WPE 1, 1
#endif
template <int BLOCK, int NM, int POL, bool AR>
__global__ __launch_bounds__(BLOCK) __attribute__((amdgpu_waves_per_eu(ASVRL_ENV_POLICY_WPE))) void env_policy_rollout_kernel(WindowArgs<typename PolicyOf<POL>::type, AR>) {
  static_assert(POL != kPolNone, "the open loop is env_rollout_kernel");
  static_assert(!AR || NM != 0, "the auto-reset is Philox noise only");
  using Args = WindowArgs<typename PolicyOf<POL>::type, AR>;
  extern __shared__ __attribute__((aligned(16))) unsigned char smem[];
  __shared__ __attribute__((aligned(16))) atile::ActorLds AL;
  sactile::SacHeadLds* head = nullptr;
  if constexpr (POL == kPolSac) {
    __shared__ __attribute__((aligned(16))) sactile::SacHeadLds HL;
    head = &HL;
  }
  const KArg<Args> PA = kargs<Args>();
  const int epb = PA->k.epb, bid = PA->k.group0 + xcd_group(static_cast<int>(blockIdx.x), static_cast<int>(gridDim.x));
  if constexpr (AR)
    env_pairs_block<BLOCK, NM, true, true, POL, true>(&PA->k, epb, bid, smem, &PA->ro, &PA->pi, &AL, &PA->ar,
                                                      smem + PA->ar_off, head);
  else
    env_pairs_block<BLOCK, NM, true, true, POL>(&PA->k, epb, bid, smem, &PA->ro, &PA->pi, &AL, nullptr, nullptr,
                                                head);
}

__global__ __launch_bounds__(kBlock) void autoreset_obs_prev_kernel(const float* __restrict__ src, float* __restrict__ row,
                                                                    const uint8_t* __restrict__ mask, int n_envs, int R) {
  constexpr int kQ = ASVRL_OBS_DIM / 4;
  const int q = blockIdx.x * blockDim.x + threadIdx.x;
  if (q >= n_envs * R * kQ) return;
  if (mask != nullptr && mask[q / (R * kQ)] == 0) return;
  reinterpret_cast<float4*>(row)[q] = reinterpret_cast<const float4*>(src)[q];
}
__global__ __launch_bounds__(kBlock) void autoreset_mask_kernel(const uint8_t* __restrict__ env_done,
                                                                const uint8_t* __restrict__ mask,
                                                                const int8_t* __restrict__ obj_cnt, int n_envs, int R,
                                                                uint8_t* __restrict__ reset_mask, int32_t* resets,
                                                                int32_t* pushed_t) {
  const int e = blockIdx.x * blockDim.x + threadIdx.x;
  if (e >= n_envs) return;
  const bool on = mask == nullptr || mask[e] != 0;
  const bool rst = on && env_done[e] != 0;
  reset_mask[e] = rst ? 1 : 0;
  if (rst && resets != nullptr) resets[e] += 1;
  if (on && pushed_t != nullptr) {
    int c = 0;
    for (int i = 0; i < R; ++i) c += obj_cnt[static_cast<size_t>(e) * R + i] >= 0 ? 1 : 0;
    if (c != 0) atomicAdd(pushed_t, c);
  }
}

__global__ void policy_step_count_kernel(const int64_t* src, int64_t* dst, int t) {
  *dst = (src != nullptr ? *src : 0) + t;
}
__global__ __launch_bounds__(kBlock) void policy_actions_kernel(const double* __restrict__ act, double* __restrict__ row,
                                                                const uint8_t* __restrict__ mask, int n_envs, int R) {
  const int k = blockIdx.x * blockDim.x + threadIdx.x;
  if (k >= n_envs * R) return;
  if (mask != nullptr && mask[k / R] == 0) return;
  row[2 * k] = act[2 * k];
  row[2 * k + 1] = act[2 * k + 1];
}

__global__ __launch_bounds__(kBlock) void rollout_record_kernel(AsvEnvState s, AsvStepOut out, AsvRollout ro, int t,
                                                                const uint8_t* mask, uint8_t* hold_mask) {
  const int e = blockIdx.x * blockDim.x + threadIdx.x;
  if (e >= s.n_envs) return;
  if (mask != nullptr && mask[e] == 0) return;
  const int R = s.max_robots;
  const size_t NT = static_cast<size_t>(s.n_envs) * R;
  const size_t t0 = static_cast<size_t>(t) * NT;
  const int nrob = s.n_robots[e];
  for (int i = 0; i < R; ++i) {
    const size_t idx = static_cast<size_t>(e) * R + i;
    if (ro.reward != nullptr) ro.reward[t0 + idx] = out.reward[idx];
    if (ro.done != nullptr) ro.done[t0 + idx] = out.done[idx];
    if (ro.info != nullptr) ro.info[t0 + idx] = out.info[idx];
    if (ro.obj_cnt != nullptr) ro.obj_cnt[t0 + idx] = out.obj_cnt[idx];
    if (ro.obs != nullptr)
      for (int k = 0; k < ASVRL_OBS_DIM; ++k) ro.obs[(t0 + idx) * ASVRL_OBS_DIM + k] = out.obs[idx * ASVRL_OBS_DIM + k];
    if (ro.rs != nullptr && i < nrob)
      for (int f = 0; f < ASVRL_NUM_FIELDS; ++f) ro.rs[(static_cast<size_t>(t) * ASVRL_NUM_FIELDS + f) * NT + idx] = s.rs[f * NT + idx];
  }
  if (ro.env_done != nullptr) ro.env_done[static_cast<size_t>(t) * s.n_envs + e] = out.env_done[e];
  if (ro.steps_run != nullptr) ro.steps_run[e] += 1;
  if (hold_mask != nullptr && out.env_done[e] != 0) hold_mask[e] = 0;
}

__device__ inline bool far_enough(double ax, double ay, double bx, double by, double lim, bool strict) {
  const double dx = ax - bx, dy = ay - by;
  const double d = sqrt(dx * dx + dy * dy);
  return strict ? !(d <= lim) : !(d < lim);
}

struct CandDraw {
  uint32_t k0, k1, e, ctr;
  __device__ double u(int phase, int cand, int j) const {
    const U4 r = philox4x32_10(U4{static_cast<uint32_t>(cand) * 4u + static_cast<uint32_t>(j >> 1), e,
                                  static_cast<uint32_t>(phase), ctr}, k0, k1);
    const uint64_t hi = (j & 1) ? r.z : r.x, lo = (j & 1) ? r.w : r.y;
    const uint64_t bits = ((hi << 32) | lo) >> 11;
    return (static_cast<double>(bits) + 1.0) * (1.0 / 9007199254740992.0);
  }
  __device__ void u2(int phase, int cand, int p, double& a, double& b) const {
    const U4 r = philox4x32_10(U4{static_cast<uint32_t>(cand) * 4u + static_cast<uint32_t>(p), e,
                                  static_cast<uint32_t>(phase), ctr}, k0, k1);
    a = (static_cast<double>(((static_cast<uint64_t>(r.x) << 32) | r.y) >> 11) + 1.0) * (1.0 / 9007199254740992.0);
    b = (static_cast<double>(((static_cast<uint64_t>(r.z) << 32) | r.w) >> 11) + 1.0) * (1.0 / 9007199254740992.0);
  }
};

__device__ __forceinline__ double bcast(double v, int f) {
  const uint64_t u = __builtin_bit_cast(uint64_t, v);
  const uint32_t lo = __builtin_amdgcn_readlane(static_cast<uint32_t>(u), f);
  const uint32_t hi = __builtin_amdgcn_readlane(static_cast<uint32_t>(u >> 32), f);
  return __builtin_bit_cast(double, (static_cast<uint64_t>(hi) << 32) | lo);
}

__device__ __forceinline__ bool core_conflict(const AsvResetCfg& cfg, double core_r, double qx, double qy, double qw,
                                              double qG, double cx, double cy, double cw, double Gamma) {
  const double dx = qx - cx, dy = qy - cy;
  const double dis = sqrt(dx * dx + dy * dy);
  if (qw == cw) {
    const double bi = qG / (2 * kPi * cfg.v_rel_max);
    const double bj = Gamma / (2 * kPi * cfg.v_rel_max);
    return dis < bi + bj;
  }
  const double gl = fmax(qG, Gamma), gs = fmin(qG, Gamma);
  const double v1 = gl / (2 * kPi * (dis - 2 * core_r));
  const double v2 = gs / (2 * kPi * core_r);
  return v1 > cfg.p_rel * v2;
}

__device__ __forceinline__ void reset_env(const AsvParams& p, const AsvEnvState& s, const AsvResetCfg& cfg, int e,
                                          uint64_t seed, uint64_t ctr, int lane, ResetLds& W) {
  double (*srob)[kResetMaxR] = W.rob;
  double (*score)[4] = W.core;
  double (*sobs)[3] = W.obs;
  const int R = s.max_robots, O = s.max_obs, Cmax = s.max_cores;
  const size_t NT = static_cast<size_t>(s.n_envs) * R;
  double* rs = s.rs;
  const uint64_t key = seed ^ (ctr >> 32) * 0x9E3779B97F4A7C15ull;
  const CandDraw g{static_cast<uint32_t>(key), static_cast<uint32_t>(key >> 32), static_cast<uint32_t>(e),
                   static_cast<uint32_t>(ctr)};
  constexpr int kDraws = 500;

  const int want_r = cfg.num_robots < R ? cfg.num_robots : R;
  int nr = 0;
  for (int base = 0; nr < want_r && base < kDraws; base += kWave) {
    const int c = base + lane;
    double u0, u1, u2, u3;
    g.u2(0, c, 0, u0, u1);
    g.u2(0, c, 1, u2, u3);
    const double sxv = 2.0 + (cfg.width - 4.0) * (1.0 - u0);
    const double syv = 2.0 + (cfg.height - 4.0) * (1.0 - u1);
    const double gxv = 2.0 + (cfg.width - 4.0) * (1.0 - u2);
    const double gyv = 2.0 + (cfg.height - 4.0) * (1.0 - u3);
    bool ok = c < kDraws && far_enough(gxv, gyv, sxv, syv, cfg.min_start_goal_dis, false);
    for (int k = 0; k < nr && ok; ++k)
      ok = far_enough(srob[0][k], srob[1][k], sxv, syv, cfg.clear_r, true) &&
           far_enough(srob[2][k], srob[3][k], gxv, gyv, cfg.clear_r, true);
    while (nr < want_r) {
      const uint64_t bal = __ballot(ok);
      if (bal == 0) break;
      const int f = __builtin_amdgcn_readfirstlane(__ffsll(static_cast<unsigned long long>(bal)) - 1);
      const double fx = bcast(sxv, f), fy = bcast(syv, f), fgx = bcast(gxv, f), fgy = bcast(gyv, f);
      if (lane == f) {
        srob[0][nr] = sxv;
        srob[1][nr] = syv;
        srob[2][nr] = gxv;
        srob[3][nr] = gyv;
        const size_t id = static_cast<size_t>(e) * R + nr;
        rs[ASVRL_F_X * NT + id] = sxv;
        rs[ASVRL_F_Y * NT + id] = syv;
        rs[ASVRL_F_GX * NT + id] = gxv;
        rs[ASVRL_F_GY * NT + id] = gyv;
// ... 344 lines not shown
static int env_checks(const char* who, bool roll, bool reset, const AsvParams* params, const AsvEnvState* state,
                      const double* actions, const double* noise, const AsvStepCtl* ctl, const AsvStepOut* out,
                      const AsvRollout* ro, const Pol* pi, const AsvAutoReset* ar, const AsvEnvLaunch* launch) {
  constexpr bool closed = !std::is_same_v<Pol, NoPolicy>;
  ENV_REQUIRE(params && state && ctl && out && (ro || !roll), "null argument");
  if (reset) {
    ENV_REQUIRE(ar != nullptr, "null ar (the auto-reset description)");
    ENV_REQUIRE(!ro->hold_done, "ro->hold_done cannot be combined with the auto-reset");
    ENV_REQUIRE(ctl->trainer_deactivate && out->env_done != nullptr,
                "the auto-reset needs ctl->trainer_deactivate and last->env_done");
    ENV_REQUIRE(ctl->noise_mode == 1 || ctl->noise_mode == 2,
                "noise_mode 0 (recorded noise) cannot cover a sampled reset; Philox noise only (mode 1 or 2)");
    ENV_REQUIRE(closed || ar->obs_prev == nullptr || ar->obs_in != nullptr,
                "ar->obs_prev needs ar->obs_in (the rows in front of step 0)");
    ENV_REQUIRE(ar->cfg.num_robots >= 0 && ar->cfg.num_robots <= kResetMaxR && state->max_robots <= kResetMaxR,
                "ar->cfg.num_robots / max_robots beyond the reset sampler's 32");
    ENV_REQUIRE(ar->cfg.num_obs >= 0 && ar->cfg.num_obs <= kResetMaxO && state->max_obs <= kResetMaxO,
                "ar->cfg.num_obs / max_obs beyond the reset sampler's 32");
    ENV_REQUIRE(ar->cfg.num_cores >= 0 && ar->cfg.num_cores <= kMaxCores && state->max_cores <= kMaxCores,
                "ar->cfg.num_cores / max_cores beyond the reset sampler's 16");
    ENV_REQUIRE(ar->cfg.width > 4.0 && ar->cfg.height > 4.0, "ar->cfg map too small");
  }
  if (roll) {
    ENV_REQUIRE(ro->n_steps >= 1, "n_steps must be >= 1");
    if (!closed) ENV_REQUIRE(ro->actions != nullptr, "null actions");
  }
  if constexpr (closed) {
    ENV_REQUIRE(ro->actions == nullptr, "ro->actions must be null (the policy supplies the actions)");
    ENV_REQUIRE(pi != nullptr, "null policy");
    ENV_REQUIRE(pi->obs_in != nullptr, "null obs_in");
    if (int rc = PolicyTraits<Pol>::checks(who, ctl, pi)) return rc;
  }
  if (roll) {
    ENV_REQUIRE(ctl->do_dynamics, "do_dynamics must be 1");
    ENV_REQUIRE(!ro->hold_done || ctl->trainer_deactivate, "hold_done needs trainer_deactivate");
    ENV_REQUIRE(ctl->noise_mode != 0 || ro->noise != nullptr, "noise_mode 0 needs injected noise");
    ENV_REQUIRE(!(ro->hold_done || ro->env_done) || (ctl->trainer_deactivate && out->env_done),
                "hold_done and the env_done record need trainer_deactivate and out->env_done");
  }
  ENV_REQUIRE(state->max_robots >= 1 && state->max_robots <= kBlock, "max_robots must be in [1, 256]");
  ENV_REQUIRE(state->max_obs >= 0 && state->max_cores >= 0 && state->max_cores <= kMaxCoresStep,
              "bad max_obs/max_cores");
  ENV_REQUIRE(params->max_obj_num >= 0 && params->max_obj_num <= ASVRL_MAX_OBJ, "max_obj_num > 5");
  ENV_REQUIRE(params->N >= 1, "N < 1");
  ENV_REQUIRE(out->obs && out->obj_cnt && out->reward && out->done && out->info, "null output");
  if (!roll) {
    ENV_REQUIRE(ctl->noise_mode != 0 || noise != nullptr, "noise_mode 0 needs injected noise");
    ENV_REQUIRE(!ctl->do_dynamics || actions != nullptr, "actions required");
  }
  ENV_REQUIRE(state->rs && state->rflags && state->n_robots && state->n_obs && state->n_cores && state->ep_ts,
              "null state array");
  if (launch != nullptr && state->n_envs != 0) {
    ENV_REQUIRE(launch->layout >= 0 && launch->layout <= 2, "layout must be 0 (auto), 1 (pairs) or 2 (sweep)");
    ENV_REQUIRE(launch->block == 0 || launch->block == 64 || launch->block == 128 || launch->block == 256,
                "block must be 0, 64, 128 or 256");
    ENV_REQUIRE(launch->envs_per_block >= 0 && launch->max_groups >= 0, "negative envs_per_block / max_groups");
  }
  if constexpr (closed)
    ENV_REQUIRE(reinterpret_cast<uintptr_t>(pi->obs_in) % 16 == 0 &&
                    reinterpret_cast<uintptr_t>(out->obs) % 16 == 0 &&
                    (!reset || reinterpret_cast<uintptr_t>(ar->obs_prev) % 16 == 0),
                "observation rows must be 16-byte aligned");
  else if (reset)
    ENV_REQUIRE(ar->obs_prev == nullptr || (reinterpret_cast<uintptr_t>(ar->obs_in) % 16 == 0 &&
                                            reinterpret_cast<uintptr_t>(ar->obs_prev) % 16 == 0),
                "ar->obs_in / ar->obs_prev rows must be 16-byte aligned");
  return 0;
}

struct PolicyLaunch {
  PairLaunch pl;
  size_t smem;
  bool fits;
};
static PolicyLaunch policy_launch(int R, int O, int n_envs, int blk_req, int epb_req, int vm_bytes, bool ar = false,
                                  size_t head_bytes = 0) {
  constexpr size_t kLdsBytes = 160 * 1024;
  constexpr size_t kLdsStatic = 1024;
  static_assert(sizeof(atile::ActorLds) + sizeof(sactile::SacHeadLds) + kLdsStatic < kLdsBytes,
                "the actor's images, the SAC head and the vote scratch leave room for a carve in one CU's LDS");
  constexpr int kCus = 256;
  auto total = [&](const PairLaunch& l) {
    const size_t rows = policy_rows_offset(l.smem) + static_cast<size_t>(l.epb) * R * (ASVRL_OBS_DIM * sizeof(float) + 2 * sizeof(double));
    return ar ? policy_rows_offset(rows) + autoreset_lds(l.blk, l.epb) : rows;
  };
  PolicyLaunch L;
  int blk = (blk_req == 64 || blk_req == 128) ? blk_req : 256;
  if (R > blk) blk = 256;
  int epb = epb_req;
  if (epb <= 0) {
    const int base = pair_launch(R, O, n_envs, blk, 0, vm_bytes).epb, per_cu = (n_envs + kCus - 1) / kCus;
    epb = per_cu > base ? per_cu : base;
  }
  for (;;) {
    L.pl = pair_launch(R, O, n_envs, blk, epb, vm_bytes);
    L.smem = total(L.pl);
    L.fits = sizeof(atile::ActorLds) + head_bytes + kLdsStatic + L.smem <= kLdsBytes;
    if (L.fits || epb_req > 0 || L.pl.epb <= 1) break;
    epb = L.pl.epb - 1;
  }
  return L;
}

struct EnvPlan {
  int nm;
  bool per_robot;
  bool fused;
  PairLaunch pl;
  size_t smem;
  int ar_off;
  int groups, chunk;
};
static int env_plan(const char* who, const AsvEnvState* state, const AsvStepCtl* ctl, const AsvEnvLaunch* launch,
                    bool closed, bool ar, EnvPlan* plan, size_t head_bytes = 0) {
  const AsvEnvLaunch lz{};
  const AsvEnvLaunch& lc = launch != nullptr ? *launch : lz;
  EnvPlan P{};
  P.nm = ctl->noise_mode == 0 ? 0 : (ctl->noise_mode == 1 ? 1 : 2);
  P.per_robot = state->robot_params != nullptr;
  const int vm_bytes = P.nm == 2 ? 4 : 8;
  if (!closed) {
    P.pl = pair_launch(state->max_robots, state->max_obs, state->n_envs, lc.block, lc.envs_per_block, vm_bytes);
    P.smem = P.pl.smem;
    if (ar) {
      P.ar_off = static_cast<int>(policy_rows_offset(P.pl.smem));
      P.smem = P.ar_off + autoreset_lds(P.pl.blk, P.pl.epb);
    }
    ENV_REQUIRE(lc.layout != 1 || P.smem <= 150 * 1024, "the pair layout's LDS does not fit");
    ENV_REQUIRE(lc.layout != 1 || !P.per_robot, "per-robot parameters take the sweep layout (2)");
    P.fused = lc.layout != 2 && !P.per_robot && P.smem <= 150 * 1024;
  } else if (lc.layout != 2 && !P.per_robot) {
    const PolicyLaunch L = policy_launch(state->max_robots, state->max_obs, state->n_envs, lc.block, lc.envs_per_block,
                                         vm_bytes, ar, head_bytes);
    P.pl = L.pl;
    P.smem = L.smem;
    if (ar) P.ar_off = static_cast<int>(L.smem - autoreset_lds(L.pl.blk, L.pl.epb));
    P.fused = L.fits;
  }
  if (P.fused) {
    P.groups = (state->n_envs + P.pl.epb - 1) / P.pl.epb;
    P.chunk = lc.max_groups > 0 && lc.max_groups < P.groups ? lc.max_groups : P.groups;
  }
  *plan = P;
  return 0;
}

template <int B, int NM> static auto kernel_of(const PairsArgs&) { return &env_pairs_kernel<B, NM>; }
template <int B, int NM, class Pol, bool AR> static auto kernel_of(const WindowArgs<Pol, AR>&) {
  if constexpr (std::is_same_v<Pol, NoPolicy>)
    return &env_rollout_kernel<B, NM, AR>;
  else
    return &env_policy_rollout_kernel<B, NM, PolicyTraits<Pol>::kPol, AR>;
}
template <class Args> constexpr bool kPhiloxOnly = false;
template <class Pol> constexpr bool kPhiloxOnly<WindowArgs<Pol, true>> = true;
static PairsArgs& pairs_of(PairsArgs& a) { return a; }
template <class Args> static PairsArgs& pairs_of(Args& a) { return a.k; }

template <int B, class Args>
static auto kernel_for_noise(int nm, const Args& a) -> void (*)(Args) {
  if constexpr (!kPhiloxOnly<Args>) {
    if (nm == 0) return kernel_of<B, 0>(a);
  }
  return nm == 1 ? kernel_of<B, 1>(a) : kernel_of<B, 2>(a);
}
template <class Args>
static int launch_groups(const char* who, const EnvPlan& P, Args a, hipStream_t st) {
  void (*const kern)(Args) = P.pl.blk == 64    ? kernel_for_noise<64>(P.nm, a)
                             : P.pl.blk == 128 ? kernel_for_noise<128>(P.nm, a)
                                               : kernel_for_noise<256>(P.nm, a);
  for (int g0 = 0; g0 < P.groups; g0 += P.chunk) {
    pairs_of(a).group0 = g0;
    hipLaunchKernelGGL(kern, dim3(P.groups - g0 < P.chunk ? P.groups - g0 : P.chunk), dim3(P.pl.blk), P.smem, st, a);
  }
  return check_launch(who);
}

extern "C" int asvrl_env_step_ex(const AsvParams* params, const AsvEnvState* state, const double* actions,
                                 const double* noise, const AsvStepCtl* ctl, const AsvStepOut* out,
                                 const AsvEnvLaunch* launch, void* stream) {
  const char* who = "asvrl_env_step";
  if (int rc = env_checks(who, false, false, params, state, actions, noise, ctl, out, nullptr, kOpenLoop, nullptr,
                          launch))
    return rc;
  if (state->n_envs == 0) return 0;
  EnvPlan P;
  if (int rc = env_plan(who, state, ctl, launch, false, false, &P)) return rc;
  if (P.fused)
    return launch_groups(who, P, PairsArgs{*params, *state, *ctl, *out, actions, noise, P.pl.epb, 0}, as_stream(stream));
  const int blk = step_block(state->max_robots);
  const int epb = blk / state->max_robots;
  const int grid = (state->n_envs + epb - 1) / epb;
  const size_t smem = env_sweep_smem(state->max_robots, state->max_obs);
  ASVRL_REQUIRE(smem <= 160 * 1024, "asvrl_env_step: max_obs too large for LDS");
  auto sweep = [&](auto kern) {
    hipLaunchKernelGGL(kern, dim3(grid), dim3(blk), smem, as_stream(stream), *params, *state, actions, noise, *ctl,
                       *out);
  };
  if (blk == 64)
    P.per_robot ? sweep(env_sweep_kernel<64, true>) : sweep(env_sweep_kernel<64, false>);
  else
    P.per_robot ? sweep(env_sweep_kernel<256, true>) : sweep(env_sweep_kernel<256, false>);
  return check_launch(who);
}

extern "C" int asvrl_env_step(const AsvParams* params, const AsvEnvState* state, const double* actions,
                              const double* noise, const AsvStepCtl* ctl, const AsvStepOut* out, void* stream) {
  return asvrl_env_step_ex(params, state, actions, noise, ctl, out, nullptr, stream);
}

template <class Pol>
static int rollout_fallback(const char* who, const AsvParams* params, const AsvEnvState* state, const AsvStepCtl* ctl,
                            const AsvStepOut* out, const AsvRollout* ro, const Pol* pi, const AsvAutoReset* ar,
                            const AsvEnvLaunch* launch, void* stream) {
  using T = PolicyTraits<Pol>;
  constexpr bool closed = !std::is_same_v<Pol, NoPolicy>;
  hipStream_t st = as_stream(stream);
  const int E = state->n_envs, R = state->max_robots;
  const size_t NT = static_cast<size_t>(E) * R;
  const size_t noise_row = NT * (static_cast<size_t>(state->max_obs) + R) * 5;
  const unsigned egrid = (static_cast<unsigned>(E) + kBlock - 1) / kBlock;
  const unsigned agrid = (static_cast<unsigned>(NT) + kBlock - 1) / kBlock;
  const unsigned qgrid = (static_cast<unsigned>(NT) * (ASVRL_OBS_DIM / 4) + kBlock - 1) / kBlock;
  const size_t pol_bytes = closed ? sizeof(double) * 2 * NT + sizeof(int64_t) : 0;
  const size_t eps_bytes = sizeof(float) * 2 * NT;
  const int eps_rows = T::eps_rows(pi);
  const size_t act_bytes = pol_bytes + eps_bytes * eps_rows;
  const size_t scratch_bytes = act_bytes + (ar != nullptr ? E : 0);
  unsigned char* scratch = nullptr;
  if (scratch_bytes != 0 && hipMallocAsync(reinterpret_cast<void**>(&scratch), scratch_bytes, st) != hipSuccess)
    return check_launch(who);
  double* act = reinterpret_cast<double*>(scratch);
  int64_t* step = closed ? reinterpret_cast<int64_t*>(act + 2 * NT) : nullptr;
  uint8_t* rmask = ar != nullptr ? scratch + act_bytes : nullptr;
  float* eps_out = eps_rows >= 1 ? reinterpret_cast<float*>(scratch + pol_bytes) : nullptr;
  float* eps_zero = eps_rows >= 2 ? eps_out + 2 * NT : nullptr;
  int rc = 0;
  if (eps_zero != nullptr && hipMemsetAsync(eps_zero, 0, eps_bytes, st) != hipSuccess) rc = check_launch(who);
  uint8_t* hold_mask = nullptr;
  if (ro->hold_done) {
    if (hipMallocAsync(reinterpret_cast<void**>(&hold_mask), E, st) != hipSuccess)
      rc = check_launch(who);
    else if (ctl->env_mask != nullptr)
      (void)hipMemcpyAsync(hold_mask, ctl->env_mask, E, hipMemcpyDeviceToDevice, st);
    else
      (void)hipMemsetAsync(hold_mask, 1, E, st);
  }
  bool one_launch = false;
  if (ar != nullptr) {
    const PairLaunch one = pair_launch(R, state->max_obs, E, kWave, 1, ctl->noise_mode == 2 ? 4 : 8);
    one_launch = state->robot_params == nullptr && one.blk == kWave && one.epb == 1 && one.smem <= 60 * 1024;
  }
  AsvStepOut oo = *out;
  oo.env_done = nullptr;
  oo.stats = nullptr;
  const float* obs_first = ar != nullptr ? ar->obs_in : nullptr;
  if constexpr (closed) obs_first = pi->obs_in;
  for (int t = 0; t < ro->n_steps && rc == 0; ++t) {
    AsvStepCtl c = *ctl;
    c.counter = ctl->counter + static_cast<uint64_t>(t);
    if (hold_mask != nullptr) c.env_mask = hold_mask;
    const float* obs_t = t == 0 ? obs_first : out->obs;
    const double* actions = act;
    if constexpr (closed) {
      double* rec_row = pi->actions != nullptr ? pi->actions + static_cast<size_t>(t) * 2 * NT : nullptr;
      if constexpr (T::kActRecords) {
        rc = T::act(pi, ActStep{obs_t, NT, act, pi->step_dev, t, R, rec_row, c.env_mask, eps_out, eps_zero}, stream);
      } else {
        hipLaunchKernelGGL(policy_step_count_kernel, dim3(1), dim3(1), 0, st, pi->step_dev, step, t);
        rc = T::act(pi, ActStep{obs_t, NT, act, step, 0, R, nullptr, nullptr, eps_out, eps_zero}, stream);
        if (rc == 0 && rec_row != nullptr)
          hipLaunchKernelGGL(policy_actions_kernel, dim3(agrid), dim3(kBlock), 0, st, act, rec_row, c.env_mask, E, R);
      }
    } else {
      actions = ro->actions + static_cast<size_t>(t) * 2 * NT;
    }
    if (rc == 0 && ar != nullptr && ar->obs_prev != nullptr)
      hipLaunchKernelGGL(autoreset_obs_prev_kernel, dim3(qgrid), dim3(kBlock), 0, st, obs_t,
                         ar->obs_prev + static_cast<size_t>(t) * NT * ASVRL_OBS_DIM, c.env_mask, E, R);
    const double* noise = ar == nullptr && ro->noise != nullptr ? ro->noise + static_cast<size_t>(t) * noise_row : nullptr;
    if (rc == 0) rc = asvrl_env_step_ex(params, state, actions, noise, &c, out, launch, stream);
    if (rc != 0) break;
    hipLaunchKernelGGL(rollout_record_kernel, dim3(egrid), dim3(kBlock), 0, st, *state, *out, *ro, t, c.env_mask,
                       hold_mask);
    if (ar != nullptr)
      hipLaunchKernelGGL(autoreset_mask_kernel, dim3(egrid), dim3(kBlock), 0, st, out->env_done, c.env_mask, out->obj_cnt,
                         E, R, rmask, ar->resets, ar->pushed != nullptr ? ar->pushed + t : nullptr);
    rc = check_launch(who);
    if (rc != 0 || ar == nullptr) continue;
    AsvStepCtl co{};
    co.is_continuous = ctl->is_continuous;
    co.noise_mode = ctl->noise_mode;
    co.seed = ctl->seed;
    co.counter = ar->obs_counter + static_cast<uint64_t>(t);
    co.counter_dev = ctl->counter_dev;
    co.env_mask = rmask;
    const uint64_t rctr = ar->reset_counter + static_cast<uint64_t>(t);
    if (one_launch) {
      rc = asvrl_env_reset_observe(params, state, &ar->cfg, rmask, ctl->seed, rctr, ctl->counter_dev, &co, &oo, stream);
    } else {
      rc = asvrl_env_reset(params, state, &ar->cfg, rmask, ctl->seed, rctr, ctl->counter_dev, stream);
      if (rc == 0) rc = asvrl_env_step_ex(params, state, nullptr, nullptr, &co, &oo, launch, stream);
    }
  }
  if (hold_mask != nullptr) (void)hipFreeAsync(hold_mask, st);
  if (scratch != nullptr) (void)hipFreeAsync(scratch, st);
  return rc;
}

template <bool AR, class Pol>
static int rollout_call(const char* who, const AsvParams* params, const AsvEnvState* state, const AsvStepCtl* ctl,
                        const AsvStepOut* out, const AsvRollout* ro, const Pol* pi, const AsvAutoReset* ar,
                        const AsvEnvLaunch* launch, void* stream) {
  using T = PolicyTraits<Pol>;
  if (int rc = env_checks(who, true, AR, params, state, nullptr, nullptr, ctl, out, ro, pi, ar, launch)) return rc;
  if (state->n_envs == 0) return 0;
  EnvPlan P{};
  if constexpr (T::kWindow) {
    if (int rc = env_plan(who, state, ctl, launch, !std::is_same_v<Pol, NoPolicy>, AR, &P, T::kHeadBytes)) return rc;
  }
  hipStream_t st = as_stream(stream);
  if (ro->steps_run != nullptr && hipMemsetAsync(ro->steps_run, 0, sizeof(int32_t) * state->n_envs, st) != hipSuccess)
    return check_launch(who);
  if (AR && ar->resets != nullptr &&
      hipMemsetAsync(ar->resets, 0, sizeof(int32_t) * state->n_envs, st) != hipSuccess)
    return check_launch(who);
  if constexpr (T::kWindow) {
    if (P.fused) {
      WindowArgs<Pol, AR> a{
          PairsArgs{*params, *state, *ctl, *out, ro->actions, AR ? nullptr : ro->noise, P.pl.epb, 0}, *ro};
      if constexpr (!std::is_same_v<Pol, NoPolicy>) a.pi = *pi;
      if constexpr (AR) {
        a.ar = *ar;
        a.ar_off = P.ar_off;
      }
      return launch_groups(who, P, a, st);
    }
  }
  return rollout_fallback(who, params, state, ctl, out, ro, pi, ar, launch, stream);
}

extern "C" int asvrl_env_rollout(const AsvParams* params, const AsvEnvState* state, const AsvStepCtl* ctl,
                                 const AsvStepOut* out, const AsvRollout* ro, const AsvEnvLaunch* launch,
                                 void* stream) {
  return rollout_call<false>("asvrl_env_rollout", params, state, ctl, out, ro, kOpenLoop, nullptr, launch, stream);
}

extern "C" int asvrl_policy_rollout(const AsvParams* params, const AsvEnvState* state, const AsvStepCtl* ctl,
                                    const AsvStepOut* out, const AsvRollout* ro, const AsvPolicy* pi,
                                    const AsvEnvLaunch* launch, void* stream) {
  return rollout_call<false>("asvrl_policy_rollout", params, state, ctl, out, ro, pi, nullptr, launch, stream);
}

extern "C" int64_t asvrl_policy_struct_size(void) { return sizeof(AsvPolicy); }

extern "C" int asvrl_env_rollout_ar(const AsvParams* params, const AsvEnvState* state, const AsvStepCtl* ctl,
                                    const AsvStepOut* out, const AsvRollout* ro, const AsvAutoReset* ar,
                                    const AsvEnvLaunch* launch, void* stream) {
  return rollout_call<true>("asvrl_env_rollout_ar", params, state, ctl, out, ro, kOpenLoop, ar, launch, stream);
}

extern "C" int asvrl_policy_rollout_ar(const AsvParams* params, const AsvEnvState* state, const AsvStepCtl* ctl,
// ... 116 lines not shown
```

distributional_rl_decision_and_control_amd/device_env.py:

```python
import ctypes as C
import types

import torch

from . import _abi
from ._abi import OBS_DIM, NUM_FIELDS


class DeviceEnvBatch:
    def __init__(self, n_envs, max_robots, max_obs, max_cores=0, device="cuda", params=None, obs64=False):
        _abi.lib()
        if max_robots < 1 or max_robots > 256:
            raise ValueError("max_robots must be in [1, 256]")
        self.n_envs, self.max_robots, self.max_obs, self.max_cores = n_envs, max_robots, max_obs, max_cores
        self.device = torch.device(device)
        self.params = params if params is not None else _abi.params_from()
        E, R, O, Cc = n_envs, max_robots, max(max_obs, 0), max(max_cores, 0)
        NT = E * R
        dev = self.device
        f64 = dict(dtype=torch.float64, device=dev)
        self.rs = torch.zeros((NUM_FIELDS, NT), **f64)
        self.rflags = torch.zeros(NT, dtype=torch.uint8, device=dev)
        self.n_robots = torch.zeros(E, dtype=torch.int32, device=dev)
        self.n_obs = torch.zeros(E, dtype=torch.int32, device=dev)
# ... 96 lines not shown
            if name not in specs:
                raise ValueError(f"{who}: unknown record {name!r}; choose from {sorted(specs)}")
            if name == "env_done" and not trainer_deactivate:
                raise ValueError(f"{who}: the env_done record needs trainer_deactivate")
            shape, dtype, fill = specs[name]
            t = given.get(name)
            if t is None:
                t = torch.full((K,) + shape, fill, dtype=dtype, device=self.device)
            assert t.dtype == dtype and t.is_contiguous() and tuple(t.shape) == (K,) + shape, name
            rec[name] = t
        steps_run = given.get("steps_run")
        if steps_run is None:
            steps_run = torch.zeros(self.n_envs, dtype=torch.int32, device=self.device)
        assert steps_run.dtype == torch.int32 and steps_run.numel() == self.n_envs
        return rec, steps_run

    def _auto_reset(self, who, auto_reset, K, specs):
        get = auto_reset.get if isinstance(auto_reset, dict) else (lambda k, d=None: getattr(auto_reset, k, d))
        NT = self.n_envs * self.max_robots
        specs["obs_prev"] = ((NT, OBS_DIM), torch.float32, 0)
        ar = _abi.AsvAutoReset()
        cfg = get("cfg")
        if cfg is None:
            raise ValueError(f"{who}: auto_reset needs cfg (an AsvResetCfg)")
        ar.cfg = cfg
        ar.reset_counter = int(get("reset_counter", 0)) & 0xFFFFFFFFFFFFFFFF
        ar.obs_counter = int(get("obs_counter", 0)) & 0xFFFFFFFFFFFFFFFF
        obs_in = get("obs_in")
        if obs_in is not None:
            assert obs_in.dtype == torch.float32 and obs_in.is_contiguous() and tuple(obs_in.shape) == (NT, OBS_DIM)
            ar.obs_in = obs_in.data_ptr()
        pushed, resets = get("pushed"), get("resets")
        if pushed is None:
            pushed = torch.zeros(K, dtype=torch.int32, device=self.device)
        else:
            assert pushed.dtype == torch.int32 and pushed.numel() == K and pushed.is_contiguous()
            pushed.zero_()
        if resets is None:
            resets = torch.zeros(self.n_envs, dtype=torch.int32, device=self.device)
        assert resets.dtype == torch.int32 and resets.numel() == self.n_envs and resets.is_contiguous()
        ar.pushed, ar.resets = pushed.data_ptr(), resets.data_ptr()
        return ar, pushed, resets

    def _rollout_args(self, who, K, extra_specs, *, noise, keep, hold_done, is_continuous, trainer_deactivate, seed,
                      counter, counter_dev, gamma, env_mask, obs, obj_cnt, fast_noise, launch, auto_reset):
        if noise is not None:
            assert noise.dtype == torch.float64 and noise.is_contiguous()
            assert noise.numel() == K * self.n_envs * self.max_robots * (self.max_obs + self.max_robots) * 5
        specs = self._record_specs()
        specs.update(extra_specs)
        ar = pushed = resets = None
        if auto_reset is not None:
            ar, pushed, resets = self._auto_reset(who, auto_reset, K, specs)
        rec, steps_run = self._records(who, keep, K, specs, trainer_deactivate)
        ctl = _abi.AsvStepCtl()
        ctl.is_continuous = int(bool(is_continuous))
        ctl.do_dynamics = 1
        ctl.trainer_deactivate = int(bool(trainer_deactivate))
        ctl.noise_mode = 0 if noise is not None else (2 if fast_noise else 1)
        ctl.seed = int(seed) & 0xFFFFFFFFFFFFFFFF
        ctl.counter = int(counter) & 0xFFFFFFFFFFFFFFFF
        ctl.counter_dev = counter_dev.data_ptr() if counter_dev is not None else None
        ctl.gamma = float(gamma)
        ctl.env_mask = env_mask.data_ptr() if env_mask is not None else None
        ro = _abi.AsvRollout()
        ro.n_steps, ro.hold_done = K, int(bool(hold_done))
        ro.noise = noise.data_ptr() if noise is not None else None
        for name, t in rec.items():
            if name not in ("actions", "obs_prev"):
                setattr(ro, name, t.data_ptr())
        ro.steps_run = steps_run.data_ptr()
        if ar is not None:
            ar.obs_prev = rec["obs_prev"].data_ptr() if "obs_prev" in rec else None
        ln = C.byref(_abi.AsvEnvLaunch(*(int(v) for v in launch))) if launch is not None else None
        return types.SimpleNamespace(ctl=ctl, ro=ro, ar=ar, pushed=pushed, resets=resets, specs=specs, rec=rec,
                                     steps_run=steps_run, st=self.state_struct(), ln=ln,
                                     out=self.out_struct(obs, obj_cnt, with_env_done=trainer_deactivate))

    def _rollout_call(self, b, L, name, extra, stream):
        args = [C.byref(self.params), C.byref(b.st), C.byref(b.ctl), C.byref(b.out), C.byref(b.ro)] + extra
        counts = {}
        if b.ar is not None:
            name += "_ar"
            args.append(C.byref(b.ar))
            counts = dict(resets=b.resets, pushed=b.pushed)
        rc = getattr(L, name)(*args, b.ln, _abi.stream_ptr(stream))
        _abi.check(rc, name, L)
        return types.SimpleNamespace(steps_run=b.steps_run, **counts, **{n: b.rec.get(n) for n in b.specs})

    def rollout(self, actions, noise=None, *, keep=("reward", "done", "info"), hold_done=False, is_continuous=True,
                trainer_deactivate=False, seed=0, counter=0, counter_dev=None, gamma=0.0, env_mask=None, obs=None,
                obj_cnt=None, fast_noise=False, launch=None, stream=None, auto_reset=None):
        assert actions.dtype == torch.float64 and actions.is_contiguous() and actions.dim() == 3
        K, NT = int(actions.shape[0]), self.n_envs * self.max_robots
        assert tuple(actions.shape[1:]) == (NT, 2)
        b = self._rollout_args("rollout", K, {}, noise=noise, keep=keep, hold_done=hold_done,
                               is_continuous=is_continuous, trainer_deactivate=trainer_deactivate, seed=seed,
                               counter=counter, counter_dev=counter_dev, gamma=gamma, env_mask=env_mask, obs=obs,
                               obj_cnt=obj_cnt, fast_noise=fast_noise, launch=launch, auto_reset=auto_reset)
        b.ro.actions = actions.data_ptr()
        return self._rollout_call(b, _abi.lib(), "asvrl_env_rollout", [], stream)

    def policy_rollout(self, pack, K, obs_in, *, noise=None, keep=("reward", "done", "info"), hold_done=False,
                       step_dev=None, eps=(1.0, 1.0, 1.0, 0.0, 0.0), policy_seed=0, trainer_deactivate=False, seed=0,
                       counter=0, counter_dev=None, gamma=0.0, env_mask=None, obs=None, obj_cnt=None,
                       fast_noise=False, launch=None, stream=None, auto_reset=None, deterministic=False,
                       cvar=1.0):
        K, NT = int(K), self.n_envs * self.max_robots
        assert pack.is_policy
        cvar = policy_options("policy_rollout", pack, cvar, deterministic)
        assert obs_in.dtype == torch.float32 and obs_in.is_contiguous() and tuple(obs_in.shape) == (NT, OBS_DIM)
        if step_dev is not None:
            assert step_dev.dtype == torch.int64 and step_dev.numel() >= 1
        b = self._rollout_args("policy_rollout", K, {"actions": ((NT, 2), torch.float64, 0)}, noise=noise, keep=keep,
                               hold_done=hold_done, is_continuous=pack.continuous, trainer_deactivate=trainer_deactivate,
                               seed=seed, counter=counter, counter_dev=counter_dev, gamma=gamma, env_mask=env_mask,
                               obs=obs, obj_cnt=obj_cnt, fast_noise=fast_noise, launch=launch, auto_reset=auto_reset)
        if b.ar is not None:
            b.ar.obs_in = None
        pi = pack.policy(cvar=cvar, deterministic=deterministic)
        pi.obs_in = obs_in.data_ptr()
        _abi.fill_schedule(pi, step_dev, eps, policy_seed)
        pi.actions = b.rec["actions"].data_ptr() if "actions" in b.rec else None
        return self._rollout_call(b, pack.L, pack.rollout, [C.byref(pi)], stream)

    def reset(self, cfg, env_mask=None, seed=0, counter=0, counter_dev=None, stream=None):
        st = self.state_struct()
        rc = _abi.lib().asvrl_env_reset(C.byref(self.params), C.byref(st), C.byref(cfg), _abi.ptr(env_mask),
                                        int(seed) & 0xFFFFFFFFFFFFFFFF, int(counter) & 0xFFFFFFFFFFFFFFFF,
                                        _abi.ptr(counter_dev), _abi.stream_ptr(stream))
        _abi.check(rc, "asvrl_env_reset")


    def reset_observe(self, cfg, env_mask, seed=0, counter=0, counter_dev=None, obs_counter=0, obs=None,
                      obj_cnt=None, fast_noise=True, stream=None):
        ctl = _abi.AsvStepCtl()
        ctl.is_continuous = 1
        ctl.do_dynamics = 0
        ctl.trainer_deactivate = 0
        ctl.noise_mode = 2 if fast_noise else 1
        ctl.seed = int(seed) & 0xFFFFFFFFFFFFFFFF
        ctl.counter = int(obs_counter) & 0xFFFFFFFFFFFFFFFF
        ctl.counter_dev = counter_dev.data_ptr() if counter_dev is not None else None
        ctl.gamma = 0.0
        ctl.env_mask = env_mask.data_ptr()
        st = self.state_struct()
        out = self.out_struct(obs, obj_cnt, with_env_done=False)
        rc = _abi.lib().asvrl_env_reset_observe(C.byref(self.params), C.byref(st), C.byref(cfg), _abi.ptr(env_mask),
                                                int(seed) & 0xFFFFFFFFFFFFFFFF, int(counter) & 0xFFFFFFFFFFFFFFFF,
                                                _abi.ptr(counter_dev), C.byref(ctl), C.byref(out),
                                                _abi.stream_ptr(stream))
        _abi.check(rc, "asvrl_env_reset_observe")


def policy_options(who, pack, cvar, deterministic):
    cvar = float(cvar)
    if not 0.0 < cvar <= 1.0:
        raise ValueError(f"{who}: cvar must be in (0, 1]")
    if cvar != 1.0 and not getattr(pack, "takes_cvar", False):
        raise ValueError(f"{who}: cvar is the risk distortion of IQN's quantile fractions (an IqnPack); "
                         "the other policies have no quantiles to distort")
    if deterministic and not getattr(pack, "takes_deterministic", False):
        raise ValueError(f"{who}: deterministic=True is the sampled actor's mean action (a SacActorPack); "
                         "the Actor and DQN_Policy have no sample to switch off")
    return cvar


def reset_cfg(num_robots=5, num_obs=4, num_cores=0, min_start_goal_dis=40.0, width=55.0, height=55.0,
              clear_r=10.0, obs_r_range=(1.0, 1.0), v_range=(3.0, 3.0), v_rel_max=1.0, p=0.8):
    c = _abi.AsvResetCfg()
    c.num_robots, c.num_obs, c.num_cores = int(num_robots), int(num_obs), int(num_cores)
    c.min_start_goal_dis, c.width, c.height, c.clear_r = float(min_start_goal_dis), float(width), float(height), float(clear_r)
    c.obs_r_lo, c.obs_r_hi = float(obs_r_range[0]), float(obs_r_range[1])
    c.v_lo, c.v_hi = float(v_range[0]), float(v_range[1])
    c.v_rel_max, c.p_rel = float(v_rel_max), float(p)
    return c


def current_field(cores, core_r, xy, stream=None):
    n = xy.shape[0]
    out = torch.empty((n, 3), dtype=torch.float64, device=xy.device)
    nc = 0 if cores is None else int(cores.shape[0])
    rc = _abi.lib().asvrl_current_field(_abi.ptr(cores) if nc else None, nc, float(core_r), _abi.ptr(xy), n,
                                        _abi.ptr(out), _abi.stream_ptr(stream))
    _abi.check(rc, "asvrl_current_field")
    return out
```

distributional_rl_decision_and_control_amd/learn_ops.py:

```python
import ctypes as C

import torch

from . import _abi
from ._abi import OBS_DIM, TR_DIM


class _QuantileHuber(torch.autograd.Function):

    @staticmethod
    def forward(ctx, qt, qe, tau, kappa):
        qt = qt.detach().float().contiguous()
        qe_c = qe.detach().float().contiguous()
        tau = tau.detach().float().contiguous()
        B, N = qe_c.shape
        Np = qt.shape[1]
        assert qt.shape[0] == B and tau.shape == (B, N)
        row = torch.empty(B, dtype=torch.float32, device=qe.device)
        loss = torch.empty((), dtype=torch.float32, device=qe.device)
        dqe = torch.empty_like(qe_c)
        rc = _abi.lib().asvrl_quantile_huber(_abi.ptr(qt), _abi.ptr(qe_c), _abi.ptr(tau), B, N, Np, float(kappa), 1.0,
                                             _abi.ptr(row), _abi.ptr(loss), _abi.ptr(dqe), _abi.stream_ptr())
        _abi.check(rc, "asvrl_quantile_huber")
        ctx.save_for_backward(dqe)
        return loss

    @staticmethod
    def backward(ctx, g):
        (dqe,) = ctx.saved_tensors
        return None, dqe * g, None, None


def quantile_huber_loss(q_targets, q_expected, taus, kappa=1.0):
    if taus.dim() == 3:
        taus = taus.squeeze(-1)
    return _QuantileHuber.apply(q_targets, q_expected, taus, kappa)


def c51_project(pns_a, returns, nonterminal, support, vmin=-1.0, vmax=1.0, gamma_n=0.99 ** 3, out=None):
    pns_a = pns_a.float().contiguous()
    B, atoms = pns_a.shape

    def col(t):
        t = t.float()
        if t.dim() == 2 and t.shape[1] == 1:
            t = t[:, 0]
        if t.dim() != 1 or t.shape[0] != B or t.stride(0) < 1:
            t = t.reshape(B).contiguous()
        return t
    R, nt = col(returns), col(nonterminal)
    sup = support.float().contiguous()
    m = out if out is not None else torch.empty_like(pns_a)
    dz = float(torch.tensor((vmax - vmin) / (atoms - 1), dtype=torch.float32))
    g32 = float(torch.tensor(gamma_n, dtype=torch.float32))
    rc = _abi.lib().asvrl_c51_project_ex(_abi.ptr(pns_a), _abi.ptr(R), R.stride(0), _abi.ptr(nt), nt.stride(0),
                                         _abi.ptr(sup), B, atoms, float(vmin), float(vmax), dz, g32, _abi.ptr(m),
                                         _abi.stream_ptr())
    _abi.check(rc, "asvrl_c51_project")
    return m


class DeviceReplay:

    def __init__(self, capacity, device="cuda"):
        _abi.lib()
        self.capacity = int(capacity)
        self.device = torch.device(device)
        self.ring = torch.zeros((self.capacity, TR_DIM), dtype=torch.float32, device=self.device)
        self.state = torch.zeros(2, dtype=torch.int64, device=self.device)
        self._work = None
        self._work_w = None
        self._n_host = 0

    def push(self, obs_prev, obs_next, obj_cnt_next, actions, reward, done, stream=None, snap=None,
             counter_inc=None):
        n = obs_prev.shape[0]
        if self._work is None or self._work.numel() < (n + 255) // 256 + 1:
            self._work = torch.zeros((n + 255) // 256 + 1, dtype=torch.int32, device=self.device)
        if actions.dim() == 1:
            adim, ald = 1, 1
        else:
            assert actions.stride(1) == 1, "action rows must be contiguous"
            adim, ald = min(actions.shape[1], 2), actions.stride(0)
        assert actions.dtype == torch.float64 and reward.dtype == torch.float64
        rc = _abi.lib().asvrl_replay_push_ex(_abi.ptr(obs_prev), _abi.ptr(obs_next), _abi.ptr(obj_cnt_next),
                                             _abi.ptr(actions), adim, ald, _abi.ptr(reward), _abi.ptr(done), n,
                                             _abi.ptr(self.ring), self.capacity, _abi.ptr(self.state),
                                             _abi.ptr(self._work), _abi.ptr(snap), _abi.ptr(counter_inc),
                                             _abi.stream_ptr(stream))
        _abi.check(rc, "asvrl_replay_push")

    def push_window(self, records, K, pushed=None, stream=None, snap=None, counter_inc=None, counter_by=None):
        get = records.get if isinstance(records, dict) else (lambda k: getattr(records, k))
        obs_prev, obs_next, cnt, actions, reward, done = (get(k) for k in ("obs_prev", "obs", "obj_cnt", "actions",
                                                                            "reward", "done"))
        K = int(K)
        n = obs_prev.shape[1]
        for t in (obs_prev, obs_next, cnt, actions, reward, done):
            assert t.is_contiguous() and t.shape[0] == K and t.shape[1] == n
        assert obs_prev.dtype == torch.float32 and obs_next.dtype == torch.float32 and cnt.dtype == torch.int8
        assert actions.dtype == torch.float64 and reward.dtype == torch.float64 and done.dtype == torch.uint8
        if K * n > self.capacity:
            raise ValueError(f"push_window: {K} x {n} rows exceed the ring's capacity {self.capacity}")
        adim = 1 if actions.dim() == 2 else min(actions.shape[2], 2)
        ald = 1 if actions.dim() == 2 else actions.shape[2]
        if pushed is not None:
            assert pushed.dtype == torch.int32 and pushed.numel() == K and pushed.is_contiguous()
        if self._work_w is None or self._work_w.numel() < K + 2:
            self._work_w = torch.zeros(K + 2, dtype=torch.int32, device=self.device)
        rc = _abi.lib().asvrl_replay_push_window(_abi.ptr(obs_prev), _abi.ptr(obs_next), _abi.ptr(cnt),
                                                 _abi.ptr(actions), adim, ald, _abi.ptr(reward), _abi.ptr(done), n, K,
                                                 _abi.ptr(pushed), _abi.ptr(self.ring), self.capacity,
                                                 _abi.ptr(self.state), _abi.ptr(self._work_w), _abi.ptr(snap),
                                                 _abi.ptr(counter_inc), int(K if counter_by is None else counter_by),
                                                 _abi.stream_ptr(stream))
        _abi.check(rc, "asvrl_replay_push_window")

    def write_rows(self, rows, slots, stream=None):
        rc = _abi.lib().asvrl_replay_write_rows(_abi.ptr(rows), _abi.ptr(slots), rows.shape[0], _abi.ptr(self.ring),
                                                _abi.stream_ptr(stream))
        _abi.check(rc, "asvrl_replay_write_rows")

    def size(self):
        return int(self.state[1].item())

    def gather(self, indices, out=None, stream=None):
        B = indices.shape[0]
        out = out if out is not None else torch.empty((B, TR_DIM), dtype=torch.float32, device=self.device)
        rc = _abi.lib().asvrl_replay_sample(_abi.ptr(self.ring), self.capacity, _abi.ptr(self.state),
                                            _abi.ptr(indices), B, 0, 0, None, 0, _abi.ptr(out), None, None, 0, 0,
                                            _abi.stream_ptr(stream))
        _abi.check(rc, "asvrl_replay_sample")
        return out

    def sample(self, B, seed=0, counter=0, counter_dev=None, out=None, stream=None, state=None, guard=0, taus=None):
        out = out if out is not None else torch.empty((B, TR_DIM), dtype=torch.float32, device=self.device)
        st = state if state is not None else self.state
        ts, tn = (taus.shape[0], taus.shape[2]) if taus is not None else (0, 0)
        if taus is not None:
            assert taus.is_contiguous() and taus.shape[1] == B and taus.dtype == torch.float32
        rc = _abi.lib().asvrl_replay_sample(_abi.ptr(self.ring), self.capacity, _abi.ptr(st), None, B,
                                            int(seed) & 0xFFFFFFFFFFFFFFFF, int(counter) & 0xFFFFFFFFFFFFFFFF,
                                            _abi.ptr(counter_dev), int(guard), _abi.ptr(out), None, _abi.ptr(taus),
                                            ts, tn, _abi.stream_ptr(stream))
        _abi.check(rc, "asvrl_replay_sample")
        return out


def split_rows(rows):
    B = rows.shape[0]
    s = (rows[:, 0:7], rows[:, 7:32].reshape(B, 5, 5), rows[:, 32:37])
    ns = (rows[:, OBS_DIM:OBS_DIM + 7], rows[:, OBS_DIM + 7:OBS_DIM + 32].reshape(B, 5, 5),
          rows[:, OBS_DIM + 32:OBS_DIM + 37])
    return s, rows[:, 80:82], rows[:, 82:83], ns, rows[:, 83:84]


def rows_from_batch(states, actions, rewards, next_states, dones):
    B = states[0].shape[0]
    rows = torch.zeros(B, 88, dtype=torch.float32, device=states[0].device)
    for c, st in ((0, states), (OBS_DIM, next_states)):
        rows[:, c:c + 7] = st[0]
        if st[1] is not None:
            rows[:, c + 7:c + 32] = st[1].reshape(B, 25)
            rows[:, c + 32:c + 37] = st[2]
    a = actions.reshape(B, -1)
    rows[:, 80:80 + a.shape[1]] = a
    rows[:, 82] = rewards.reshape(B)
    rows[:, 83] = dones.reshape(B)
    return rows


class DevicePER:

    def __init__(self, capacity, stride=1, n_step=3, discount=0.99, priority_weight=0.4, priority_exponent=0.5,
                 deferred=False, device="cuda"):
        _abi.lib()
        self.device = torch.device(device)
        self.stride = int(stride)
        self.capacity = (int(capacity) // self.stride) * self.stride
        P = 1 << (self.capacity - 1).bit_length()
        if self.capacity < 2 or P > (1 << 22):
            raise ValueError(f"DevicePER capacity {capacity} (stride {stride}) outside [2, 2^22]")
        self.tree_leaves = P
        self.n_step, self.discount = int(n_step), float(discount)
        self.priority_weight, self.priority_exponent = float(priority_weight), float(priority_exponent)
        dev = self.device
        self.rows = torch.zeros((self.capacity, _abi.PER_DIM), dtype=torch.float32, device=dev)
        self.tree = torch.zeros(2 * P - 1, dtype=torch.float32, device=dev)
        self.state = torch.zeros(4, dtype=torch.int64, device=dev)
        self.t = torch.zeros(self.stride, dtype=torch.int32, device=dev)
        self.maxp = torch.ones(1, dtype=torch.float32, device=dev)
        self._weights = {}
        self.dirty = torch.zeros(max(1, P // 2048), dtype=torch.uint8, device=dev)
        s = _abi.AsvPer()
        s.rows, s.tree, s.state, s.t = self.rows.data_ptr(), self.tree.data_ptr(), self.state.data_ptr(), \
            self.t.data_ptr()
        s.maxp, s.dirty = self.maxp.data_ptr(), self.dirty.data_ptr()
        s.capacity, s.tree_leaves, s.stride, s.n_step = self.capacity, P, self.stride, self.n_step
        s.discount, s.priority_weight, s.priority_exponent = self.discount, self.priority_weight, \
            self.priority_exponent
        s.deferred = 1 if deferred else 0
        self.deferred = bool(deferred)
        self._s = s
        self.pushed = 0

    def push(self, obs, obj_cnt, actions, reward, done, stream=None, step_counter=None):
        n = obs.shape[0]
        adim = 1
        if actions.dim() == 2:
            assert actions.stride(1) == 1, "action rows must be contiguous"
            adim = actions.stride(0) if n > 1 else actions.shape[1]
        rc = _abi.lib().asvrl_per_push_ex(C.byref(self._s), _abi.ptr(obs), _abi.ptr(obj_cnt), _abi.ptr(actions),
                                          adim, _abi.ptr(reward), _abi.ptr(done), n, _abi.ptr(step_counter),
                                          _abi.stream_ptr(stream))
        _abi.check(rc, "asvrl_per_push")
        self.pushed += n

    def push_window(self, buf, K, counter_inc=None, counter_by=None, stream=None):
        get = buf.get if isinstance(buf, dict) else (lambda k: getattr(buf, k))
        obs, cnt, actions, reward, done = (get(k) for k in ("obs_prev", "obj_cnt", "actions", "reward", "done"))
        K = int(K)
        NT = obs.shape[1]
        for t in (obs, cnt, actions, reward, done):
            assert t.is_contiguous() and t.shape[0] == K and t.shape[1] == NT
        assert obs.dtype == torch.float32 and obs.shape[2] == OBS_DIM and cnt.dtype == torch.int8
        assert actions.dtype == torch.float64 and actions.dim() == 3 and actions.shape[2] == 2
        assert reward.dtype == torch.float64 and done.dtype == torch.uint8
        n = K * NT
        rc = _abi.lib().asvrl_per_push_window(C.byref(self._s), _abi.ptr(obs), _abi.ptr(cnt), _abi.ptr(actions), 2,
                                              _abi.ptr(reward), _abi.ptr(done), n, _abi.ptr(counter_inc),
                                              int(K if counter_by is None else counter_by), _abi.stream_ptr(stream))
# ... 38 lines not shown
```

distributional_rl_decision_and_control_amd/vec_env.py:

```python
import numpy as np
import torch

from . import _abi
from .device_env import DeviceEnvBatch, reset_cfg


class VecMarineNavEnv:
    def __init__(self, n_envs, num_robots=5, num_obs=4, num_cores=0, min_start_goal_dis=40.0, width=55.0,
                 height=None, schedule=None, seed=0, device="cuda", is_continuous=True, gamma=0.99,
                 max_robots=None, max_obs=None, max_cores=None):
        self.n_envs = int(n_envs)
        self.schedule = schedule
        self.max_groups = 0
        R = max_robots or (max(schedule["num_robots"]) if schedule else num_robots)
        O = max_obs if max_obs is not None else (max(schedule["num_obstacles"]) if schedule else num_obs)
        Cc = max_cores if max_cores is not None else (max(schedule["num_cores"]) if schedule else num_cores)
        self.batch = DeviceEnvBatch(self.n_envs, R, O, Cc, device=device)
        self.max_robots = R
        self.device = self.batch.device
        self.seed = int(seed)
        self.is_continuous = is_continuous
        self.gamma = gamma
        self.width = float(width)
        self.height = float(height if height is not None else width)
        self.cfg = reset_cfg(num_robots, num_obs, num_cores, min_start_goal_dis, self.width, self.height)
        NT = self.n_envs * R
        self.obs = [torch.zeros((NT, _abi.OBS_DIM), dtype=torch.float32, device=self.device) for _ in range(2)]
        self.cnt = [torch.full((NT,), -1, dtype=torch.int8, device=self.device) for _ in range(2)]
        self.counter = torch.zeros(1, dtype=torch.int64, device=self.device)
        self.total_timesteps = 0

    swap = False
    _p = 0
    fused_reset = True

    @property
    def obs_cur(self):
        return self.obs[self._p]

    @property
    def cnt_cur(self):
        return self.cnt[self._p]

    @property
    def obs_next(self):
        return self.obs[1 - self._p]

    @property
    def cnt_next(self):
        return self.cnt[1 - self._p]

    def apply_schedule(self, total_timesteps):
        if self.schedule is None:
            return
        steps = np.array(self.schedule["timesteps"])
        idx = len(steps[steps - total_timesteps <= 0]) - 1
        self.cfg = reset_cfg(self.schedule["num_robots"][idx], self.schedule["num_obstacles"][idx],
                             self.schedule["num_cores"][idx], self.schedule["min_start_goal_dis"][idx], self.width,
                             self.height)

    def reset(self):
        b = self.batch
        b.reset(self.cfg, None, seed=self.seed, counter=0x40000000, counter_dev=self.counter)
        b.step(None, do_dynamics=False, seed=self.seed, counter=0x80000000, counter_dev=self.counter,
               fast_noise=True, obs=self.obs_cur, obj_cnt=self.cnt_cur)
        return self.obs_cur

    def step(self, actions):
        self.batch.step(actions, is_continuous=self.is_continuous, trainer_deactivate=True, seed=self.seed,
                        counter=0, counter_dev=self.counter, gamma=self.gamma, obs=self.obs_next,
                        obj_cnt=self.cnt_next, fast_noise=True,
                        launch=self._launch())

    def _auto_reset(self, auto_reset, open_loop):
        if not auto_reset:
            return None
        ar = dict(auto_reset) if isinstance(auto_reset, dict) else {}
        ar.update(cfg=self.cfg, reset_counter=0x40000000, obs_counter=0x80000000)
        if open_loop:
            ar["obs_in"] = self.obs_cur
        return ar

    def rollout(self, actions, hold_done=True, keep=("reward", "done", "info"), auto_reset=False, count=True):
        ar = self._auto_reset(auto_reset, True)
        rec = self.batch.rollout(actions, keep=keep, hold_done=hold_done and ar is None,
                                 is_continuous=self.is_continuous,
                                 trainer_deactivate=True, seed=self.seed, counter=0, counter_dev=self.counter,
                                 gamma=self.gamma, obs=self.obs_next, obj_cnt=self.cnt_next, fast_noise=True,
                                 launch=self._launch(), auto_reset=ar)
        if count:
            self.counter += int(actions.shape[0])
        return rec

    def policy_rollout(self, pack, K, hold_done=True, keep=("reward", "done", "info"), eps=(1.0, 1.0, 1.0, 0.0, 0.0),
                       policy_seed=0, env_mask=None, auto_reset=False, count=True, deterministic=False, cvar=1.0):
        if not pack.continuous:
            if self.is_continuous:
                raise ValueError("policy_rollout: a DqnPack, IqnPack or RainbowPack picks discrete actions, this env "
                                 "was built with is_continuous=True")
        elif not self.is_continuous:
            raise ValueError("policy_rollout: the Actor drives continuous-action envs")
        ar = self._auto_reset(auto_reset, False)
        rec = self.batch.policy_rollout(pack, K, self.obs_cur, keep=keep, hold_done=hold_done and ar is None,
                                        step_dev=self.counter,
                                        eps=eps, policy_seed=policy_seed, trainer_deactivate=True, seed=self.seed,
                                        counter=0, counter_dev=self.counter, gamma=self.gamma, env_mask=env_mask,
                                        obs=self.obs_next, obj_cnt=self.cnt_next, fast_noise=True,
                                        launch=self._launch(), auto_reset=ar, deterministic=deterministic, cvar=cvar)
        if count:
            self.counter += int(K)
        return rec

    def _launch(self):
        return (0, 0, 0, self.max_groups) if self.max_groups > 0 else None

    def auto_reset(self, counted=False, events=None):
        b = self.batch
        d = 1 if counted else 0
        if events is not None:
            events[0].record()
        if self.fused_reset and b.robot_params is None and self.max_groups <= 0:
            b.reset_observe(self.cfg, b.env_done, seed=self.seed, counter=0x40000000 - d, counter_dev=self.counter,
                            obs_counter=0x80000000 - d, obs=self.obs_next, obj_cnt=self.cnt_next)
            if events is not None:
                events[1].record()
            return
        b.reset(self.cfg, b.env_done, seed=self.seed, counter=0x40000000 - d, counter_dev=self.counter)
        if events is not None:
            events[1].record()
        b.step(None, do_dynamics=False, seed=self.seed, counter=0x80000000 - d, counter_dev=self.counter,
               fast_noise=True, env_mask=b.env_done, obs=self.obs_next, obj_cnt=self.cnt_next, launch=self._launch())
        if events is not None:
            events[2].record()

    def advance_device(self, counted=False):
        if self.swap:
            self._p ^= 1
        else:
            self.obs[0].copy_(self.obs[1])
            self.cnt[0].copy_(self.cnt[1])
        if not counted:
            self.counter += 1

    def advance_host(self):
        self.total_timesteps += self.n_envs

    def episode_stats(self):
        s = self.batch.stats.cpu().numpy()
        n = max(s[1], 1.0)
        return dict(mean_return=s[0] / n, success=s[2] / n, collision=s[3] / n, timeout=s[4] / n,
                    robot_episodes=int(s[1]), env_episodes=int(s[5]))


def split_obs(obs_rows):
    M = obs_rows.shape[0]
    return obs_rows[:, 0:7], obs_rows[:, 7:32].reshape(M, 5, 5), obs_rows[:, 32:37]
```

distributional_rl_decision_and_control_amd/vec_trainer.py:

```python
import time

import torch

from . import streams
from .learn_ops import DevicePER, DeviceReplay
from .learner import FlatParams, FusedAdam
from .learners import LEARNERS, policy_modules, policy_parameters
from .vec_env import VecMarineNavEnv

DEFAULT_NET = dict(self_dimension=7, object_dimension=5, max_object_num=5, self_feature_dimension=56,
                   object_feature_dimension=40, concat_feature_dimension=256, hidden_dimension=128)


class VecTrainer:
    def __init__(self, n_envs=4096, agent_type="AC-IQN", num_robots=5, num_obs=4, num_cores=0, min_start_goal_dis=40.0,
                 width=55.0, batch_size=4096, num_tau=32, buffer_size=4_000_000, lr=1e-4, gamma=0.99,
                 learning_starts=None, target_update_interval=2500, total_timesteps=6_000_000,
                 exploration_fraction=0.25, initial_eps=0.6, final_eps=0.05, seed=0,
                 device="cuda", sync=None, graphs=False, schedule=None, net_seed=100, overlap=True, unroll=1,
                 chain=None, operands="bf16", target_after_env=False, push_after_actor=None, tau=1.0,
                 target_update="host"):
        if not 0.0 < float(tau) <= 1.0:
            raise ValueError(f"tau must be in (0, 1], not {tau!r}")
        if target_update not in ("host", "device"):
# ... 22 lines not shown
        self.learning_starts = learning_starts if learning_starts is not None else batch_size
        self.local = spec.make_policy(DEFAULT_NET.values(), self.device, net_seed)
        self.target = spec.make_policy(DEFAULT_NET.values(), self.device, net_seed)
        for p in policy_parameters(self.target):
            p.requires_grad_(False)
        if spec.refusal is not None and not spec.supported(self.local, batch_size, num_tau):
            raise ValueError(spec.refusal.format(B=batch_size, N=num_tau))
        if spec.actor_critic:
            self.actor_opt = FusedAdam(self.local.actor.parameters(), lr=lr, operands=operands)
            self.actor_grads = self.actor_opt.grads
            if spec.twin:
                self.critic_opts = [FusedAdam(c.parameters(), lr=lr, operands=operands)
                                    for c in (self.local.critic_1, self.local.critic_2)]
            else:
                self.critic_opt = FusedAdam(self.local.critic.parameters(), lr=lr, operands=operands)
                self.critic_grads = self.critic_opt.grads
        else:
            self.opt = FusedAdam(self.local.parameters(), lr=lr, operands=operands)
            self.grads = self.opt.grads
        self._target_flat = None
        if target_update == "device":
            self._target_flat = [FlatParams(m.parameters(), operands) for m in policy_modules(self.target)]
            assert [f.n for f in self._target_flat] == [o.n for o in self.local_opts()]
        self.action_dim = spec.action_dim
        self.n_step = 3 if spec.per else None
        self.support = torch.linspace(-1.0, 1.0, 51, device=self.device) if spec.per else None
        self.fused2 = self.fused_iqn = self.fused_rb = self.fused_dqn = self.fused_ddpg = self.fused_sac = None
        self.learner = spec.state(self.local, self.target, batch_size, num_tau, operands, support=self.support,
                                  batched=(graphs, max(1, int(unroll))))
        setattr(self, spec.field, self.learner)
        NT = self.E * self.R
        self.per = None
        if spec.per:
            slots = max(min(buffer_size, 1 << 22) // NT, self.n_step + 3)
            self.per = DevicePER(slots * NT, stride=NT, n_step=self.n_step, discount=gamma, deferred=True,
                                 device=self.device)
            self.replay = None
            self.per_idx = torch.zeros(self.B, dtype=torch.int64, device=self.device)
            self.learning_starts = max(self.learning_starts, (self.n_step + 1) * NT + self.B)
        else:
            self.replay = DeviceReplay(max(buffer_size, 2 * NT), device=self.device)
        self.actions = torch.zeros((NT, 2), dtype=torch.float64, device=self.device)
        self.learn_counter = torch.zeros(1, dtype=torch.int64, device=self.device)
        self.loss_mean = torch.zeros(1, dtype=torch.float32, device=self.device)
        self.batch_rows = torch.zeros((self.B, 88), dtype=torch.float32, device=self.device)
        self.taus = torch.zeros((3, self.B, self.num_tau), dtype=torch.float32, device=self.device)
        self.learn_steps = 0
        self.iterations = 0
        self.last_losses = None
        self.graphs = graphs
        self._graph = None
        self.unroll = max(1, int(unroll))
        self.env.swap = not graphs or self.unroll % 2 == 0
        self._phase = 0
        self._graph_learn = None
        self.overlap = bool(overlap)
        self.ring_snap = torch.zeros(2, dtype=torch.int64, device=self.device)
        self._streams = None
        self.chain = (agent_type == "AC-IQN") if chain is None else bool(chain)
        if self.chain and agent_type in ("DDPG", "SAC"):
            raise ValueError(f"the dependency-chained schedule is not available for {agent_type} (chain=None or "
                             "False: the joined schedule)")
        paa_ok = agent_type == "AC-IQN" and self.graphs and self._chained()
        if self.target_after_env and not paa_ok:
            raise ValueError("target_after_env applies only to the chained, graph-captured AC-IQN schedule")
        if self._paa_arg is None:
            self.push_after_actor = paa_ok
        elif self.push_after_actor and not paa_ok:
            raise ValueError("push_after_actor applies only to the chained, graph-captured AC-IQN schedule")
        self.ring_snap2 = torch.zeros((2, 2), dtype=torch.int64, device=self.device)
        self._gen = torch.Generator(device=self.device)
        self._gen.manual_seed(seed + 12345)
        self.env.reset()

    def epsilon(self):
        steps = self.env.counter.to(torch.float32) * float(self.E)
        progress = steps / float(self.total_timesteps)
        r = progress / self.exploration_fraction
        eps = self.initial_eps + r * (self.final_eps - self.initial_eps)
        return torch.where(progress < self.exploration_fraction, eps, torch.full_like(eps, self.final_eps))

    @torch.no_grad()
    def act(self):
        args = (self.env.obs_cur, self.actions, self.env.counter, self.E, self.total_timesteps,
                self.exploration_fraction, self.initial_eps, self.final_eps, self.seed + 4242)
        self.learner.act(*args)

    def _eval_env(self):
        from . import _abi
        src = self.env
        c = src.cfg
        env = VecMarineNavEnv(self.E, c.num_robots, c.num_obs, c.num_cores, c.min_start_goal_dis, c.width, c.height,
                              seed=self.seed + 7919, device=self.device, is_continuous=True, gamma=self.gamma,
                              max_robots=src.max_robots, max_obs=src.batch.max_obs, max_cores=src.batch.max_cores)
        env.batch.params = _abi.AsvParams.from_buffer_copy(src.batch.params)
        env.reset()
        return env

    @torch.no_grad()
    def greedy_episodes(self, max_steps=1000, chunk=64):
        if self.learner.actor_pack is None:
            raise NotImplementedError("greedy_episodes runs the AC-IQN / DDPG actor; IQN, Rainbow and DQN act inside "
                                      "their own kernels (the learner's window_pack / eval_pack with "
                                      "device_evaluator(...).run is the route for IQN and Rainbow)")
        env = self._eval_env()
        alive = torch.ones(self.E, dtype=torch.uint8, device=self.device)
        steps_run = torch.zeros(self.E, dtype=torch.int32, device=self.device)
        done = 0
        while done < max_steps:
            k = min(int(chunk), max_steps - done)
            rec = env.policy_rollout(self.learner.actor_pack, k, hold_done=True, keep=("env_done",), env_mask=alive)
            env.advance_device(counted=True)
            steps_run += rec.steps_run
            alive *= (rec.env_done.sum(0) == 0).to(torch.uint8)
            done += k
            if not bool(alive.any().item()):
                break
        return dict(env.episode_stats(), steps_run=steps_run.cpu().numpy())

    @torch.no_grad()
    def evaluate(self, configs, chunk=64, template_env=None, **kw):
        if self.learner.actor_pack is None:
            raise NotImplementedError("evaluate runs the AC-IQN / DDPG actor; IQN, Rainbow and DQN act inside their "
                                      "own kernels (device_evaluator(...).run(policy_pack()) for DQN, "
                                      "run(fused_iqn.window_pack) for IQN, run(fused_rb.eval_pack) for Rainbow)")
        return self.device_evaluator(configs, chunk, template_env).run(self.learner.actor_pack, **kw)

    def policy_pack(self):
        if self.learner.policy_pack is not None:
            return self.learner.policy_pack
        raise NotImplementedError(f"policy_pack: the closed-loop windows run the AC-IQN / DDPG actor or DQN_Policy, not "
                                  f"{self.agent_type} (its learner's window_pack, and Rainbow's eval_pack, go to "
                                  "policy_rollout / DeviceEvaluator.run / _collect_window directly)")

    def device_evaluator(self, configs, chunk=64, template_env=None):
        from .policy.device_eval import DeviceEvaluator
        cached = getattr(self, "_dev_eval", None)
        if cached is None or cached[0] is not configs or cached[1] != (len(configs), int(chunk), template_env):
            ev = DeviceEvaluator(configs, template_env=template_env, device=self.device, chunk=chunk,
                                 gamma=self.gamma)
            cached = self._dev_eval = (configs, (len(configs), int(chunk), template_env), ev)
        return cached[2]

    def _push(self, snap=None):
        env = self.env
        if self.per is not None:
            self.per.push(env.obs_cur, env.cnt_next, self.actions[:, :1], env.batch.reward, env.batch.done,
                          step_counter=env.counter)
            return True
        self.replay.push(env.obs_cur, env.obs_next, env.cnt_next, self.actions[:, :self.action_dim],
                         env.batch.reward, env.batch.done, snap=snap, counter_inc=env.counter)
        return True

    def rollout(self, snap=None):
        self.act()
        self.env.step(self.actions)
        counted = self._push(snap)
        self.env.auto_reset(counted)
        self.env.advance_device(counted)

    def _collect_buffers(self, K):
        bufs = getattr(self, "_collect_bufs", None)
        if bufs is None:
            bufs = self._collect_bufs = {}
        if K not in bufs:
            NT, dev = self.E * self.R, self.device
            bufs[K] = dict(
                obs=torch.zeros((K, NT, 40), dtype=torch.float32, device=dev),
                obs_prev=torch.zeros((K, NT, 40), dtype=torch.float32, device=dev),
                obj_cnt=torch.full((K, NT), -1, dtype=torch.int8, device=dev),
                reward=torch.zeros((K, NT), dtype=torch.float64, device=dev),
                done=torch.ones((K, NT), dtype=torch.uint8, device=dev),
                actions=torch.zeros((K, NT, 2), dtype=torch.float64, device=dev),
                steps_run=torch.zeros(self.E, dtype=torch.int32, device=dev),
                pushed=torch.zeros(K, dtype=torch.int32, device=dev),
                resets=torch.zeros(self.E, dtype=torch.int32, device=dev))
        return bufs[K]

    @torch.no_grad()
    def collect(self, K, snap=None):
        if self.learner.actor_pack is None or self.per is not None:
            raise NotImplementedError("collect runs the AC-IQN / DDPG actor and pushes into the uniform ring; IQN, "
                                      "Rainbow and DQN act inside their own kernels (_collect_window takes the "
                                      "learner's window_pack for SAC, IQN and Rainbow)")
        return self._collect_window(self.learner.actor_pack, K, snap)

    @torch.no_grad()
    def _collect_window(self, pack, K, snap=None):
        K = int(K)
        buf = self._collect_buffers(K)
        buf["obj_cnt"].fill_(-1)
        if self.per is not None:
            pack.refresh()
        keep = {k: buf[k] for k in ("obs", "obs_prev", "obj_cnt", "reward", "done", "actions", "steps_run")}
        rec = self.env.policy_rollout(pack, K, hold_done=False, keep=keep,
                                      eps=(self.E, self.total_timesteps, self.exploration_fraction, self.initial_eps,
                                           self.final_eps), policy_seed=self.seed + 4242,
                                      auto_reset=dict(pushed=buf["pushed"], resets=buf["resets"]), count=False)
        if self.per is not None:
            self.per.push_window(buf, K, counter_inc=self.env.counter, counter_by=K)
        else:
            self.replay.push_window(buf, K, pushed=buf["pushed"], snap=snap, counter_inc=self.env.counter,
                                    counter_by=K)
        self.env.advance_device(True)
        return rec

    def learn(self, state=None, guard=0, actor_wait=None, target_wait=None, actor_done=None, target_step=True):
        out = self.learner.learn(self, state, guard, actor_wait, target_wait, actor_done)
        if target_step:
            self._target_step()
        return out

    def local_opts(self):
        if not LEARNERS[self.agent_type].actor_critic:
            return [self.opt]
        return [self.actor_opt] + (list(self.critic_opts) if LEARNERS[self.agent_type].twin else [self.critic_opt])

    def _target_step(self):
        if self._target_flat is not None:
            self.learner.target_step(self)

    def hard_update(self):
        with torch.no_grad():
            torch._foreach_copy_(policy_parameters(self.target), policy_parameters(self.local))
            self.learner.target_changed()

    def soft_update(self):
        tau = self.tau
        with torch.no_grad():
            for t, l in zip(policy_parameters(self.target), policy_parameters(self.local)):
                t.copy_(tau * l + (1.0 - tau) * t)
            self.learner.target_changed()

    @torch.no_grad()
    def load_policies(self, local, target):
        assert self._graph is None, "load_policies before the first captured iteration"
        for dst, src in ((self.local, local), (self.target, target)):
            for d, s in zip(policy_modules(dst), policy_modules(src)):
                sd = s.state_dict()
                for name, t in d.state_dict(keep_vars=True).items():
                    t.data.copy_(sd[name].to(device=t.device, dtype=t.dtype))
        self.learner.refresh_local()
        self.learner.target_changed()

    def _iteration_body(self, do_learn):
        if not (do_learn and self.overlap and self.per is None):
            self.rollout()
            return self.learn() if do_learn else None
        main = torch.cuda.current_stream(self.device)
        if self._streams is None:
            self._streams = (self.roll_stream(),) + self._roll_events()
        s_roll, ev_snap, ev_act = self._streams
        self.ring_snap.copy_(self.replay.state)
        s_roll.wait_stream(main)
        with torch.cuda.stream(s_roll):
            self.act()
            ev_act.record(s_roll)
            env = self.env
            env.step(self.actions)
            counted = self._push()
            env.auto_reset(counted)
            env.advance_device(counted)
        out = self.learn(state=self.ring_snap, guard=self.E * self.R, actor_wait=ev_act)
        main.wait_stream(s_roll)
        return out

    def iteration(self, timing=None):
        do_learn = self.replay_size_host() >= self.learning_starts
        if self.graphs and do_learn and self._graph is None:
            try:
                self._capture()
            except RuntimeError as e:
                import sys
                print(f"VecTrainer: HIP graph capture failed ({e}); continuing without graphs", file=sys.stderr)
                self.graphs, self._graph = False, None
        if self.graphs and do_learn:
            if self._phase == 0:
                self._graph.replay()
            self._phase = (self._phase + 1) % self.unroll
            out = self._graph_out
        else:
            out = self._iteration_body(do_learn)
        self.env.advance_host()
        self.iterations += 1
        if do_learn:
            self.learn_steps += 1
            if self._target_flat is None and self.learn_steps % self.target_update_interval == 0:
                if self.tau == 1.0:
                    self.hard_update()
                else:
                    self.soft_update()
        self.last_losses = out
        return out

    def replay_size_host(self):
        if getattr(self, "_replay_ready", False):
            return self.learning_starts
        n = self.per.pushed if self.per is not None else self.replay.size()
        if n >= self.learning_starts:
            self._replay_ready = True
        return n

    def roll_stream(self):
        return streams.stream(self.device, "roll")

    def _roll_events(self):
        return torch.cuda.Event(), torch.cuda.Event()

    def _chained(self):
        return self.chain and self.overlap and self.per is None and self.unroll % 2 == 0

    def _chain_body(self):
        main = torch.cuda.current_stream(self.device)
        if self._streams is None:
            self._streams = (self.roll_stream(),) + self._roll_events()
        s_roll = self._streams[0]
        U = self.unroll
        ev_act = [torch.cuda.Event() for _ in range(U)]
        ev_snap = [torch.cuda.Event() for _ in range(U)]
        ev_learn = [torch.cuda.Event() for _ in range(U)]
        ev_env = [torch.cuda.Event() for _ in range(U)]
        ev_actor = [torch.cuda.Event() for _ in range(U)]
        self._chain_events = (ev_act, ev_snap, ev_learn, ev_env, ev_actor)
        tae, paa = self.target_after_env, self.push_after_actor
        s_roll.wait_stream(main)
        out = None

        def push_reset(k):
            self._push(snap=self.ring_snap2[k % 2])
            ev_snap[k].record(s_roll)
            self.env.auto_reset(True)
            self.env.advance_device(True)

        for k in range(U):
            with torch.cuda.stream(s_roll):
                if k > 0:
                    s_roll.wait_event(ev_learn[k - 1])
                self.act()
                ev_act[k].record(s_roll)
                self.env.step(self.actions)
                if tae:
                    ev_env[k].record(s_roll)
                if not paa:
                    push_reset(k)
            if k > 0:
                main.wait_event(ev_snap[k - 1])
            out = self.learn(state=self.ring_snap2[(k - 1) % 2], guard=self.E * self.R, actor_wait=ev_act[k],
                             target_wait=ev_env[k] if tae else None, actor_done=ev_actor[k] if paa else None,
                             target_step=False)
            ev_learn[k].record(main)
            self._target_step()
            if paa:
                with torch.cuda.stream(s_roll):
                    s_roll.wait_event(ev_actor[k])
                    push_reset(k)
        main.wait_stream(s_roll)
        return out

    def _capture(self):
        s = streams.stream(self.device, "warmup")
        s.wait_stream(torch.cuda.current_stream(self.device))
        with torch.cuda.stream(s):
            for _ in range(3):
                self._iteration_body(True)
                self.env.advance_host()
        torch.cuda.current_stream(self.device).wait_stream(s)
        g = torch.cuda.CUDAGraph()
        chained = self._chained()
        if chained:
            self.ring_snap2[(self.unroll - 1) % 2].copy_(self.replay.state)
        with torch.cuda.graph(g, stream=streams.capture_stream(self.device), capture_error_mode="thread_local"):
            if chained:
                self._graph_out = self._chain_body()
            else:
                for _ in range(self.unroll):
                    self._graph_out = self._iteration_body(True)
        self._graph = g

    def run(self, iterations):
        t0 = time.time()
        for _ in range(iterations):
            self.iteration()
        torch.cuda.synchronize(self.device)
        return time.time() - t0
```

include/asvrl.h:

```cpp
#ifndef ASVRL_H
#define ASVRL_H

#include <stddef.h>
#include <stdint.h>

#ifdef __cplusplus
extern "C" {
#endif

#define ASVRL_ABI_VERSION 29

#define ASVRL_SELF_DIM 7
#define ASVRL_OBJ_DIM 5
#define ASVRL_MAX_OBJ 5
#define ASVRL_OBS_DIM 40
#define ASVRL_TR_DIM 88
#define ASVRL_PER_DIM 48

enum AsvRobotField {
  ASVRL_F_X = 0, ASVRL_F_Y, ASVRL_F_THETA,
  ASVRL_F_VR0, ASVRL_F_VR1, ASVRL_F_VR2,
  ASVRL_F_V0, ASVRL_F_V1, ASVRL_F_V2,
  ASVRL_F_TL, ASVRL_F_TR, ASVRL_F_LP, ASVRL_F_RP,
  ASVRL_F_GX, ASVRL_F_GY,
// ... 547 lines not shown
} AsvActorGradIO;
int64_t asvrl_actor_grads_workspace(int32_t B);
int32_t asvrl_actor_grads_counters(void);
int32_t asvrl_actor_grads_norm_parts(void);
int asvrl_actor_grads(const AsvActorGradIO* io, void* stream);

int asvrl_linear_wgrad_vec(const float* dq, int64_t ldq, const void* x, int64_t ldx, int32_t R, int32_t K, float* dw,
                           float* db, int32_t accumulate, float* work, int64_t work_floats, void* stream);

int32_t asvrl_linear_wgrad_vec_groups(int32_t R);
int asvrl_linear_wgrad_vec_partial(const float* dq, int64_t ldq, const void* x, int64_t ldx, int32_t R,
                                   int32_t K, float* partial, int64_t partial_floats, int32_t* groups_out,
                                   void* stream);

#define ASVRL_MAX_SUM_SEGS 24
#define ASVRL_SUM_PLAIN 0
#define ASVRL_SUM_FOLD_ENCODERS 1
typedef struct AsvPartialSum {
  const float* partial;
  float* dw;
  float* db;
  int32_t groups, nw, nb, accumulate;
  int32_t stride;
  int32_t boff;
  int32_t mode;
  int32_t norm;
} AsvPartialSum;
int asvrl_partial_sums(const AsvPartialSum* segs, int32_t nseg, void* stream);

int asvrl_partial_sums_norm(const AsvPartialSum* segs, int32_t nseg, double* norm_parts, float* step,
                            void* stream);
int32_t asvrl_partial_sums_norm_parts(const AsvPartialSum* segs, int32_t nseg);


typedef struct AsvMlpSrc {
  const float* self_w;
  const float* self_b;
  const float* obj_w;
  const float* obj_b;
  const float* w1;
  const float* w2;
  const float* ae_w;
} AsvMlpSrc;

typedef struct AsvMlpWeights {
  const void* enc_frag;
  const float* b_enc;
  const void* w1_frag;
  const void* w2_frag;
  const void* w2t_frag;
  const void* w1t_frag;
  const float* b1;
  const float* b2;
  const float* wout;
  const float* bout;
  const void* ae_frag;
  const float* b_ae;
  float out_scale;
} AsvMlpWeights;

typedef struct AsvMlpIO {
  const float* x;
  int64_t ldx;
  const float* act;
  int64_t lda;
  int32_t n;
  float* F;
  float* G;
  void* xb;
  float* a_out;
  int64_t ld_aout;
  double* a_out64;
  float* pre;
  void* h0;
  void* h1;
  void* h2;
  const float* dA;
  float* dout;
  void* dz2;
  void* dz1;
  void* dz0;
  const int64_t* step_dev;
  double eps_steps_per_count;
  double eps_total, eps_fraction, eps_initial, eps_final;
  uint64_t seed;
} AsvMlpIO;

int asvrl_mlp_pack(const AsvMlpSrc* src, const AsvMlpWeights* w, void* stream);
int asvrl_mlp_encode(const AsvMlpWeights* w, const AsvMlpIO* io, void* stream);
int asvrl_actor_forward(const AsvMlpWeights* w, const AsvMlpIO* io, int32_t mode, void* stream);
typedef struct AsvSampleArgs {
  const float* ring;
  int64_t capacity;
  const int64_t* ring_state;
  uint64_t seed, counter;
  const uint64_t* counter_dev;
  int64_t guard;
  int32_t B, tau_sets, tau_n, _pad0;
  float* out;
  float* taus;
} AsvSampleArgs;
int asvrl_learn_prologue(const AsvSampleArgs* s, const AsvMlpWeights* actor, const AsvMlpIO* train_io,
                         const AsvMlpWeights* target_actor, float* na, void* stream);
int asvrl_actor_backward(const AsvMlpWeights* w, const AsvMlpIO* io, void* stream);
int asvrl_encoder_fold(const float* dw, const float* db, float* self_w, float* self_b, float* obj_w,
                       float* obj_b, int32_t accumulate, void* stream);
int asvrl_small_wgrad(const float* dz, int64_t ldz, const float* x, int64_t ldx, int32_t R, int32_t M,
                      int32_t K, float* dw, float* db, int32_t accumulate, float* work,
                      int64_t work_floats, void* stream);
int asvrl_small_wgrad_partial(const float* dz, int64_t ldz, const float* x, int64_t ldx, int32_t R,
                              int32_t M, int32_t K, float* partial, int64_t partial_floats,
                              int32_t* groups_out, void* stream);


typedef struct AsvPolicy {
  AsvMlpWeights w;
  const float* obs_in;
  const int64_t* step_dev;
  double eps_steps_per_count, eps_total, eps_fraction, eps_initial, eps_final;
  uint64_t seed;
  double* actions;
} AsvPolicy;

int asvrl_policy_rollout(const AsvParams* params, const AsvEnvState* state, const AsvStepCtl* ctl,
                         const AsvStepOut* last, const AsvRollout* ro, const AsvPolicy* pi,
                         const AsvEnvLaunch* launch , void* stream);
int64_t asvrl_policy_struct_size(void);


typedef struct AsvAutoReset {
  AsvResetCfg cfg;
  uint64_t reset_counter, obs_counter;
  const float* obs_in;
  float* obs_prev;
  int32_t* pushed;
  int32_t* resets;
} AsvAutoReset;

int asvrl_env_rollout_ar(const AsvParams* params, const AsvEnvState* state, const AsvStepCtl* ctl,
                         const AsvStepOut* last, const AsvRollout* ro, const AsvAutoReset* ar,
                         const AsvEnvLaunch* launch , void* stream);
int asvrl_policy_rollout_ar(const AsvParams* params, const AsvEnvState* state, const AsvStepCtl* ctl,
                            const AsvStepOut* last, const AsvRollout* ro, const AsvPolicy* pi,
                            const AsvAutoReset* ar, const AsvEnvLaunch* launch , void* stream);
int64_t asvrl_autoreset_struct_size(void);

int asvrl_replay_push_window(const float* obs_prev, const float* obs_next, const int8_t* obj_cnt_next,
                             const double* actions, int32_t action_dim, int64_t action_ld, const double* reward,
                             const uint8_t* done, int32_t n, int32_t K, const int32_t* pushed, float* ring,
                             int64_t capacity, int64_t* ring_state, int32_t* work, int64_t* snap,
                             int64_t* counter_inc, int64_t counter_by, void* stream);


typedef struct AsvEvalMetrics {
  int32_t n_steps;
  int32_t n_envs;
  int32_t max_robots;
  int32_t episode_limit;
  double gamma;
  const double*  reward;
  const uint8_t* info;
  const double*  rs;
  const int32_t* steps_run;
  const int32_t* n_robots;
  const double*  dt;
  const double*  N;
  const double*  pc;
  int32_t* length;
  uint8_t* ended;
  uint8_t* alive;
  uint8_t* deact;
  uint8_t* outcome;
  double*  ret;
  double*  time;
  double*  energy;
} AsvEvalMetrics;

int asvrl_eval_metrics(const AsvEvalMetrics* m, void* stream);
int64_t asvrl_eval_metrics_struct_size(void);

#define ASVRL_HISTORY_ROW_TILE 32
#define ASVRL_HISTORY_STEP_TILE 16
#define ASVRL_TRAJ_DIM 13
#define ASVRL_HISTORY_OBS_DIM 32

typedef struct AsvEvalHistory {
  int32_t n_steps;
  int32_t n_envs;
  int32_t max_robots;
  int32_t act_steps;
  const uint8_t* info;
  const int32_t* length;
  const int32_t* n_robots;
  int32_t*       counts;
  const int64_t* offsets;
  const double*  rs0;
  const double*  rs;
  const double*  actions;
  const float*   obs0;
  const float*   obs;
  const int8_t*  cnt0;
  const int8_t*  obj_cnt;
  double* traj;
  double* act;
  float*  obs_out;
  int8_t* cnt_out;
  int64_t traj_rows, act_rows, obs_rows;
} AsvEvalHistory;

int asvrl_eval_history_count(const AsvEvalHistory* h, void* stream);
int asvrl_eval_history_pack(const AsvEvalHistory* h, void* stream);
int64_t asvrl_eval_history_struct_size(void);
int32_t asvrl_eval_history_step_tile(void);


typedef struct AsvNoiseStreams {
  int32_t n_envs;
  int32_t max_robots;
  int32_t max_obs;
  int32_t _pad0;
  const int32_t* n_robots;
  const int32_t* n_obs;
  const uint8_t* rflags;
  const uint8_t* env_mask;
  const AsvParams* robot_params;
  uint32_t* key;
  int32_t*  pos;
  int32_t*  has_gauss;
  double*   gauss;
  double*   noise_out;
  int64_t*  draws_n;
  double*   draws_sum;
  double*   draws_sq;
} AsvNoiseStreams;

int asvrl_noise_streams(const AsvParams* p, const AsvNoiseStreams* ns, void* stream);
int asvrl_noise_streams_host(const AsvParams* p, const AsvNoiseStreams* ns, void* stream);
int64_t asvrl_noise_streams_struct_size(void);

#define ASVRL_DQN_MAX_ACTIONS 32
typedef struct AsvDqnWeights {
  AsvMlpWeights trunk;
  const void* head_frag;
  int32_t n_actions;
  int32_t _pad0;
} AsvDqnWeights;

typedef struct AsvDqnActIO {
  const float* x;
  int64_t ldx;
  int32_t n;
  int32_t _pad0;
  double* act_out;
  int64_t ld_act;
  float* q_out;
  const int64_t* step_dev;
  double eps_steps_per_count;
  double eps_total, eps_fraction, eps_initial, eps_final;
  uint64_t seed;
} AsvDqnActIO;

typedef struct AsvDqnGradIO {
  const float* rows;
  int64_t ld_rows;
  int32_t B;
  float gamma;
  void* xb;
  void* h0;
  void* h1;
  void* h2;
  float* q_sel;
  float* q_next;
  void* dz_out;
  void* dz2;
  void* dz1;
  void* dz0;
  float* tile_loss;
} AsvDqnGradIO;

int asvrl_dqn_pack(const AsvMlpSrc* src, const float* wout, const AsvDqnWeights* w, void* stream);
int asvrl_dqn_act(const AsvDqnWeights* w, const AsvDqnActIO* io, void* stream);
int asvrl_dqn_grad(const AsvDqnWeights* local, const AsvDqnWeights* target, const AsvDqnGradIO* io, void* stream);
int64_t asvrl_dqn_weights_struct_size(void);
int64_t asvrl_dqn_act_struct_size(void);
int64_t asvrl_dqn_grad_struct_size(void);


typedef struct AsvDqnPolicy {
  AsvDqnWeights w;
  const float* obs_in;
  const int64_t* step_dev;
  double eps_steps_per_count, eps_total, eps_fraction, eps_initial, eps_final;
  uint64_t seed;
  double* actions;
} AsvDqnPolicy;

int asvrl_dqn_rollout(const AsvParams* params, const AsvEnvState* state, const AsvStepCtl* ctl,
                      const AsvStepOut* last, const AsvRollout* ro, const AsvDqnPolicy* pi,
                      const AsvEnvLaunch* launch , void* stream);
int asvrl_dqn_rollout_ar(const AsvParams* params, const AsvEnvState* state, const AsvStepCtl* ctl,
                         const AsvStepOut* last, const AsvRollout* ro, const AsvDqnPolicy* pi,
                         const AsvAutoReset* ar, const AsvEnvLaunch* launch , void* stream);
int64_t asvrl_dqn_policy_struct_size(void);

typedef struct AsvDdpgWeights {
  AsvMlpWeights trunk;
// ... 200 lines not shown
```

Before: 16.59 million env-steps/s.

## Fuse env step, replay push and auto-reset into one kernel

Adds a single-step kernel that runs the env step, writes transitions straight into the replay ring, and performs the auto-reset in the same launch. Ring slots are ordered by a per-env acting-count prefix kept in a double-buffered array, and the last block to finish advances the ring head. The trainer routes step/push/reset through this path when it is eligible. This removes separate push and reset launches and the intermediate obs/reward traffic between them. In exchange it adds a grid-wide last-block atomic, a prefix scan over the acting counts in every block, and more LDS use.

```diff
diff --git a/distributional_rl_decision_and_control_amd/_abi.py b/distributional_rl_decision_and_control_amd/_abi.py
--- a/distributional_rl_decision_and_control_amd/_abi.py
+++ b/distributional_rl_decision_and_control_amd/_abi.py
@@ -201,6 +201,16 @@
 class AsvAutoReset(C.Structure):
     _fields_ = [("cfg", AsvResetCfg), ("reset_counter", _U64), ("obs_counter", _U64), ("obs_in", _VP),
                 ("obs_prev", _VP), ("pushed", _VP), ("resets", _VP)]
+
+
+class AsvStepPush(C.Structure):
+    _fields_ = [("cfg", AsvResetCfg), ("reset_counter", _U64), ("obs_counter", _U64), ("obs_prev", _VP),
+                ("ring", _VP), ("capacity", _I64), ("ring_state", _VP), ("work", _VP), ("snap", _VP),
+                ("counter_inc", _VP), ("acting", _VP), ("action_dim", _I32), ("_pad0", _I32)]
+
+
+def acting_stride(n_envs):
+    return (int(n_envs) + 15) & ~15
 
 
 class AsvEvalMetrics(C.Structure):
@@ -485,6 +495,9 @@
                                        C.POINTER(AsvStepOut), C.POINTER(AsvRollout), C.POINTER(AsvAutoReset),
                                        C.POINTER(AsvEnvLaunch), _VP]),
     ("asvrl_autoreset_struct_size", _I64, []),
+    ("asvrl_env_step_push_ar", C.c_int, [C.POINTER(AsvParams), C.POINTER(AsvEnvState), _VP, C.POINTER(AsvStepCtl),
+                                         C.POINTER(AsvStepOut), C.POINTER(AsvStepPush), C.POINTER(AsvEnvLaunch), _VP]),
+    ("asvrl_step_push_struct_size", _I64, []),
     ("asvrl_replay_push_window", C.c_int, [_VP, _VP, _VP, _VP, _I32, _I64, _VP, _VP, _I32, _I32, _VP, _VP, _I64, _VP,
                                            _VP, _VP, _VP, _I64, _VP]),
     ("asvrl_eval_metrics", C.c_int, [C.POINTER(AsvEvalMetrics), _VP]),
diff --git a/distributional_rl_decision_and_control_amd/csrc/asvrl_env.hip b/distributional_rl_decision_and_control_amd/csrc/asvrl_env.hip
--- a/distributional_rl_decision_and_control_amd/csrc/asvrl_env.hip
+++ b/distributional_rl_decision_and_control_amd/csrc/asvrl_env.hip
@@ -582,6 +582,10 @@
 __host__ __device__ constexpr size_t autoreset_lds(int blk, int epb) {
   return static_cast<size_t>(blk / 64) * sizeof(ResetLds) + sizeof(int) * static_cast<size_t>(epb);
 }
+__host__ __device__ constexpr size_t step_push_off(int blk, int epb) { return (autoreset_lds(blk, epb) + 7) & ~size_t{7}; }
+__host__ __device__ constexpr size_t step_push_lds(int blk, int epb, int R) {
+  return step_push_off(blk, epb) + sizeof(int64_t) * static_cast<size_t>(epb) * R + sizeof(int) * (2 * (blk / 64) + 2);
+}
 enum : int { kPolNone = 0, kPolActor = 1, kPolDqn = 2, kPolSac = 3 };
 template <int POL> struct PolicyOf { using type = AsvPolicy; };
 template <> struct PolicyOf<kPolDqn> { using type = AsvDqnPolicy; };
@@ -595,9 +599,11 @@
                                                 KArg<typename PolicyOf<POL>::type> PI = nullptr,
                                                 atile::ActorLds* AL = nullptr, KArg<AsvAutoReset> RS = nullptr,
                                                 unsigned char* ar_lds = nullptr,
-                                                sactile::SacHeadLds* HL = nullptr) {
+                                                sactile::SacHeadLds* HL = nullptr,
+                                                KArg<AsvStepPush> SP = nullptr) {
   static_assert(POL == kPolNone || ROLL, "the policy runs inside the rollout's step loop");
-  static_assert(!AR || ROLL, "the auto-reset runs inside the rollout's step loop");
+  static_assert(!AR || ROLL || DYN, "the auto-reset follows a step, in the rollout's step loop or behind the single step");
+  constexpr bool PUSH = AR && !ROLL;
   const int R = A->s.max_robots;
   const int O = A->s.max_obs;
   const int S = O + R;
@@ -651,6 +657,8 @@
   int taken = 0;
   int nreset = 0;
   bool rstl = false;
+  [[maybe_unused]] int par = 0, npush = 0;
+  [[maybe_unused]] bool acts_next = false;
   const int n_steps = ROLL ? RO->n_steps : 1;
   const bool hold = ROLL && RO->hold_done != 0;
   auto load_state = [&] {
@@ -703,7 +711,7 @@
     }
     __syncthreads();
   }
-  if constexpr (AR) {
+  if constexpr (AR && ROLL) {
     const KArg<AsvAutoReset> Q = kfresh(RS);
     const float* src0 = POL != kPolNone ? PI->obs_in : Q->obs_in;
     if (env_on0 && Q->obs_prev != nullptr) {
@@ -722,8 +730,8 @@
   bool obsp = false;
   [[maybe_unused]] phases:
   if constexpr (AR) asm volatile("" : "+v"(tid), "+v"(le), "+v"(idx));
-  const bool env_on = ROLL ? (on && (!obsp || rstl)) : env_on0;
-  const bool exists = ROLL ? (exists0 && env_on) : exists0;
+  const bool env_on = (ROLL || AR) ? (on && (!obsp || rstl)) : env_on0;
+  const bool exists = (ROLL || AR) ? (exists0 && env_on) : exists0;
   const uint8_t fl = flv;
   const bool deact = (fl & ASVRL_FLAG_DEACTIVATED) != 0;
   const bool active = exists && !deact;
@@ -746,7 +754,7 @@
   };
   auto each_out = [&](KArg<PairsArgs> Ak, auto&& f) {
     if (wlast) f(kref(Ak).out, std::false_type{}, size_t{0});
-    if constexpr (AR) {
+    if constexpr (AR && ROLL) {
       if (!obsp) f(rec_row(), std::true_type{}, size_t{0});
     } else if constexpr (ROLL) {
       f(rec_row(), std::true_type{}, size_t{0});
@@ -756,7 +764,7 @@
       o.obs = sobs;
       f(o, std::true_type{}, row0);
     }
-    if constexpr (AR) {
+    if constexpr (AR && ROLL) {
       const KArg<AsvAutoReset> Q = kfresh(RS);
       AsvStepOut o{};
       if (Q->obs_prev != nullptr && t + 1 < n_steps)
@@ -876,7 +884,7 @@
       reward += d_before - d_after;
     }
     if constexpr (!ROLL) {
-      if (exists && (DYN && A->ctl.do_dynamics)) store_state();
+      if (exists && (DYN && A->ctl.do_dynamics) && !obsp) store_state();
     }
     double so0 = 0, so1 = 0, so2 = 0, so3 = 0, so4 = 0;
     if (rlane) {
@@ -972,7 +980,9 @@
   };
   uint64_t ctr = A->ctl.counter + (A->ctl.counter_dev != nullptr ? *A->ctl.counter_dev : 0ull) +
                  (ROLL ? static_cast<uint64_t>(t) : 0ull);
-  if constexpr (AR) {
+  if constexpr (PUSH) {
+    if (obsp) ctr = ctr - A->ctl.counter + SP->obs_counter;
+  } else if constexpr (AR) {
     if (obsp) ctr = ctr - A->ctl.counter + RS->obs_counter;
   }
   const size_t noise_t = (ROLL && NM == 0) ? static_cast<size_t>(t) * NT * S * 5 : 0;
@@ -1161,7 +1171,10 @@
                                      ret);
   if (A->ctl.trainer_deactivate && (DYN && A->ctl.do_dynamics) && !obsp && exists && !(res.nfl & ASVRL_FLAG_DEACTIVATED))
     atomicAdd(&salive[le], 1);
-  if constexpr (AR) {
+  if constexpr (PUSH) {
+    if (env_on) acts_next = exists && !(res.nfl & ASVRL_FLAG_DEACTIVATED);
+  }
+  if constexpr (AR && ROLL) {
     if (!obsp && RS->pushed != nullptr) {
       const unsigned long long bal = __ballot(exists && cnt >= 0);
       if ((tid & (kWave - 1)) == 0 && bal != 0) atomicAdd(RS->pushed + t, static_cast<int32_t>(__popcll(bal)));
@@ -1169,7 +1182,7 @@
   }
   if (exists) {
     if constexpr (!ROLL) {
-      if ((DYN && A->ctl.do_dynamics)) A->s.rs[ASVRL_F_RET * NT + idx] = res.ret;
+      if ((DYN && A->ctl.do_dynamics) && !obsp) A->s.rs[ASVRL_F_RET * NT + idx] = res.ret;
       A->s.rs[ASVRL_F_PHI * NT + idx] = phi;
       A->s.rflags[idx] = res.nfl;
     } else {
@@ -1216,18 +1229,86 @@
   A = kfresh(A);
   if constexpr (AR) {
     if (obsp) {
-      if (exists && t == n_steps - 1) {
-        A->s.rs[ASVRL_F_PHI * NT + idx] = phi;
-        A->s.rflags[idx] = flv;
+      if constexpr (ROLL) {
+        if (exists && t == n_steps - 1) {
+          A->s.rs[ASVRL_F_PHI * NT + idx] = phi;
+          A->s.rflags[idx] = flv;
+        }
       }
       continue;
     }
   }
+  [[maybe_unused]] bool end = false;
   if constexpr (!ROLL) {
     if (env_on && i == 0 && (DYN && A->ctl.do_dynamics)) env_end(kref(A).p, kref(A).s, kref(A).ctl, kref(A).out, e, ep_ts, nrob, salive[le], NT);
+    if constexpr (PUSH) {
+      end = env_on && ((ep_ts >= A->p.episode_limit) || salive[le] == 0);
+      const KArg<AsvStepPush> Q = kfresh(SP);
+      int64_t* sslot = reinterpret_cast<int64_t*>(ar_lds + step_push_off(BLOCK, epb));
+      int* spw = reinterpret_cast<int*>(sslot + nrb);
+      int* sfr = spw + BLOCK / kWave;
+      const int ln = tid & (kWave - 1), wv = tid / kWave;
+      par = static_cast<int>(*Q->counter_inc & 1);
+      const uint8_t* ahead = Q->acting + static_cast<size_t>(par) * ASVRL_ACTING_STRIDE(A->s.n_envs);
+      const int lim = bid * epb;
+      int front = 0;
+      for (int q = tid; q < lim / 16; q += BLOCK) {
+        const uint4 v = reinterpret_cast<const uint4*>(ahead)[q];
+        const uint32_t w4[4] = {v.x, v.y, v.z, v.w};
+#pragma unroll
+        for (int k = 0; k < 4; ++k) {
+          const uint32_t h = (w4[k] & 0x00FF00FFu) + ((w4[k] >> 8) & 0x00FF00FFu);
+          front += static_cast<int>((h & 0xFFFFu) + (h >> 16));
+        }
+      }
+      for (int k = lim / 16 * 16 + tid; k < lim; k += BLOCK) front += ahead[k];
+      for (int off = 32; off > 0; off >>= 1) front += __shfl_xor(front, off, kWave);
+      const bool pushes = exists && cnt >= 0;
+      const unsigned long long bal = __ballot(pushes);
+      if (ln == 0) {
+        spw[wv] = __popcll(bal);
+        sfr[wv] = front;
+      }
+      __syncthreads();
+      int before = 0;
+      npush = 0;
+#pragma unroll
+      for (int w = 0; w < BLOCK / kWave; ++w) {
+        before += sfr[w] + (w < wv ? spw[w] : 0);
+        npush += spw[w];
+      }
+      const int64_t cap = Q->capacity;
+      const int64_t head_in = Q->ring_state[0];
+      int64_t slot = -1;
+      if (pushes) {
+        slot = (head_in + before + __popcll(bal & ((1ull << ln) - 1ull))) % cap;
+        float4* dst = reinterpret_cast<float4*>(Q->ring + slot * ASVRL_TR_DIM);
+        const double* act = A->actions + 2 * idx;
+        dst[2 * ASVRL_OBS_DIM / 4] = make_float4(static_cast<float>(act[0]), Q->action_dim > 1 ? static_cast<float>(act[1]) : 0.f,
+                                                 static_cast<float>(res.reward), res.done ? 1.f : 0.f);
+        dst[2 * ASVRL_OBS_DIM / 4 + 1] = make_float4(0.f, 0.f, 0.f, 0.f);
+      }
+      if (rlane) sslot[tid] = slot;
+      __syncthreads();
+      {
+        constexpr int kQ = ASVRL_OBS_DIM / 4;
+        const size_t g0 = static_cast<size_t>(bid) * nrb;
+        const int nr = NT - g0 < static_cast<size_t>(nrb) ? static_cast<int>(NT - g0) : nrb;
+        const float4* a4 = reinterpret_cast<const float4*>(Q->obs_prev) + g0 * kQ;
+        const float4* b4 = reinterpret_cast<const float4*>(A->out.obs) + g0 * kQ;
+        for (int q = tid; q < nr * kQ; q += BLOCK) {
+          const int rr = q / kQ;
+          const int64_t sl = sslot[rr];
+          if (sl >= 0) {
+            float4* dst = reinterpret_cast<float4*>(Q->ring + sl * ASVRL_TR_DIM) + (q - rr * kQ);
+            dst[0] = a4[q];
+            dst[kQ] = b4[q];
+          }
+        }
+      }
+    }
   } else {
     const KArg<AsvRollout> Q = kfresh(RO);
-    bool end = false;
     if (env_on && A->ctl.trainer_deactivate && (hold || AR || i == 0))
       end = (ep_ts >= A->p.episode_limit) || salive[le] == 0;
     if (env_on && i == 0) {
@@ -1253,52 +1334,85 @@
       ++taken;
     }
     if (hold && end) on = false;
-    if constexpr (AR) {
-      rstl = env_on && end;
-      int* srst = reinterpret_cast<int*>(ar_lds + (BLOCK / kWave) * sizeof(ResetLds));
-      if (rlane && i == 0) srst[le] = rstl ? 1 : 0;
-      if (!__syncthreads_or(rstl ? 1 : 0)) continue;
-      __syncthreads();
-      {
-        const KArg<AsvAutoReset> Z = kfresh(RS);
-        const uint64_t rctr = Z->reset_counter + (A->ctl.counter_dev != nullptr ? *A->ctl.counter_dev : 0ull) +
-                              static_cast<uint64_t>(t);
-        const int wv = __builtin_amdgcn_readfirstlane(tid / kWave);
-        ResetLds* W = reinterpret_cast<ResetLds*>(ar_lds);
-        for (int qe = wv; qe < epb; qe += BLOCK / kWave)
-          if (__builtin_amdgcn_readfirstlane(srst[qe]) != 0)
-            reset_env(kref(A).p, kref(A).s, kref(Z).cfg, bid * epb + qe, A->ctl.seed, rctr, tid & (kWave - 1), W[wv]);
-      }
-      __syncthreads();
-      A = kfresh(A);
-      if (rstl) {
-        nrob = A->s.n_robots[e];
-        exists0 = i < nrob;
-        r = Regs{};
-        gx = 0;
-        gy = 0;
-        phi = 0.0;
-        ret = 0.0;
-        flv = 0;
-        if (exists0) {
-          load_state();
-          phi = A->s.rs[ASVRL_F_PHI * NT + idx];
-          ret = A->s.rs[ASVRL_F_RET * NT + idx];
-          flv = A->s.rflags[idx];
-        }
-        ep_ts = 0;
-        if (i == 0) ++nreset;
-      }
-      obsp = true;
-      goto phases;
-    }
+  }
+  if constexpr (AR) {
+    rstl = env_on && end;
+    int* srst = reinterpret_cast<int*>(ar_lds + (BLOCK / kWave) * sizeof(ResetLds));
+    if (rlane && i == 0) srst[le] = rstl ? 1 : 0;
+    if (!__syncthreads_or(rstl ? 1 : 0)) continue;
+    __syncthreads();
+    {
+      KArg<std::conditional_t<ROLL, AsvAutoReset, AsvStepPush>> Z;
+      if constexpr (ROLL) Z = kfresh(RS); else Z = kfresh(SP);
+      const uint64_t rctr = Z->reset_counter + (A->ctl.counter_dev != nullptr ? *A->ctl.counter_dev : 0ull) +
+                            static_cast<uint64_t>(t);
+      const int wv = __builtin_amdgcn_readfirstlane(tid / kWave);
+      ResetLds* W = reinterpret_cast<ResetLds*>(ar_lds);
+      for (int qe = wv; qe < epb; qe += BLOCK / kWave)
+        if (__builtin_amdgcn_readfirstlane(srst[qe]) != 0)
+          reset_env(kref(A).p, kref(A).s, kref(Z).cfg, bid * epb + qe, A->ctl.seed, rctr, tid & (kWave - 1), W[wv]);
+    }
+    __syncthreads();
+    A = kfresh(A);
+    if (rstl) {
+      nrob = A->s.n_robots[e];
+      exists0 = i < nrob;
+      r = Regs{};
+      gx = 0;
+      gy = 0;
+      phi = 0.0;
+      ret = 0.0;
+      flv = 0;
+      if (exists0) {
+        load_state();
+        phi = A->s.rs[ASVRL_F_PHI * NT + idx];
+        ret = A->s.rs[ASVRL_F_RET * NT + idx];
+        flv = A->s.rflags[idx];
+      }
+      ep_ts = 0;
+      if (i == 0) ++nreset;
+    }
+    obsp = true;
+    goto phases;
   }
   }
   if constexpr (ROLL) {
     if (lane_env && i == 0 && RO->steps_run != nullptr) RO->steps_run[e] = taken;
   }
-  if constexpr (AR) {
+  if constexpr (AR && ROLL) {
     if (lane_env && i == 0 && RS->resets != nullptr) RS->resets[e] = nreset;
+  }
+  if constexpr (PUSH) {
+    const KArg<AsvStepPush> Q = kfresh(SP);
+    if (rlane) sact[tid] = acts_next ? 1 : 0;
+    __syncthreads();
+    if (lane_env && i == 0) {
+      int c = 0;
+      for (int j = 0; j < R; ++j) c += sact[le * R + j];
+      Q->acting[static_cast<size_t>(par ^ 1) * ASVRL_ACTING_STRIDE(A->s.n_envs) + e] = static_cast<uint8_t>(c);
+    }
+    int* slast = reinterpret_cast<int*>(ar_lds + step_push_off(BLOCK, epb) + sizeof(int64_t) * nrb) + 2 * (BLOCK / kWave);
+    if (tid == 0) {
+      atomicAdd(Q->work + 1, npush);
+      __threadfence();
+      *slast = atomicAdd(Q->work, 1) == static_cast<int>(gridDim.x) - 1;
+    }
+    __syncthreads();
+    if (*slast == 0) return;
+    if (tid == 0) {
+      const int tot = atomicExch(Q->work + 1, 0);
+      const int64_t cap = Q->capacity;
+      const int64_t nh = (Q->ring_state[0] + tot) % cap, ns0 = Q->ring_state[1] + tot;
+      const int64_t ns = ns0 < cap ? ns0 : cap;
+      Q->ring_state[0] = nh;
+      Q->ring_state[1] = ns;
+      if (Q->snap != nullptr) {
+        Q->snap[0] = nh;
+        Q->snap[1] = ns;
+      }
+      *Q->counter_inc += 1;
+      *Q->work = 0;
+    }
   }
 }
 
@@ -1370,6 +1484,24 @@
   else
     env_pairs_block<BLOCK, NM, true, true, POL>(&PA->k, epb, bid, smem, &PA->ro, &PA->pi, &AL, nullptr, nullptr,
                                                 head);
+}
+
+#ifndef ASVRL_ENV_STEP_PUSH_WPE
+#define ASVRL_ENV_STEP_PUSH_WPE 2
+#endif
+struct StepPushArgs {
+  PairsArgs k;
+  AsvStepPush sp;
+  int ar_off;
+};
+template <int BLOCK, int NM>
+__global__ __launch_bounds__(BLOCK) __attribute__((amdgpu_waves_per_eu(NM == 1 ? 1 : ASVRL_ENV_STEP_PUSH_WPE))) void env_step_push_kernel(StepPushArgs) {
+  static_assert(NM != 0, "the auto-reset is Philox noise only");
+  extern __shared__ __attribute__((aligned(16))) unsigned char smem[];
+  const KArg<StepPushArgs> SA = kargs<StepPushArgs>();
+  env_pairs_block<BLOCK, NM, true, false, kPolNone, true>(
+      &SA->k, SA->k.epb, SA->k.group0 + xcd_group(static_cast<int>(blockIdx.x), static_cast<int>(gridDim.x)), smem,
+      nullptr, nullptr, nullptr, nullptr, smem + SA->ar_off, nullptr, &SA->sp);
 }
 
 __global__ __launch_bounds__(kBlock) void autoreset_obs_prev_kernel(const float* __restrict__ src, float* __restrict__ row,
@@ -2020,8 +2152,10 @@
   else
     return &env_policy_rollout_kernel<B, NM, PolicyTraits<Pol>::kPol, AR>;
 }
+template <int B, int NM> static auto kernel_of(const StepPushArgs&) { return &env_step_push_kernel<B, NM>; }
 template <class Args> constexpr bool kPhiloxOnly = false;
 template <class Pol> constexpr bool kPhiloxOnly<WindowArgs<Pol, true>> = true;
+template <> constexpr bool kPhiloxOnly<StepPushArgs> = true;
 static PairsArgs& pairs_of(PairsArgs& a) { return a; }
 template <class Args> static PairsArgs& pairs_of(Args& a) { return a.k; }
 
@@ -2076,6 +2210,49 @@
                               const double* noise, const AsvStepCtl* ctl, const AsvStepOut* out, void* stream) {
   return asvrl_env_step_ex(params, state, actions, noise, ctl, out, nullptr, stream);
 }
+
+extern "C" int asvrl_env_step_push_ar(const AsvParams* params, const AsvEnvState* state, const double* actions,
+                                      const AsvStepCtl* ctl, const AsvStepOut* out, const AsvStepPush* sp,
+                                      const AsvEnvLaunch* launch, void* stream) {
+  const char* who = "asvrl_env_step_push_ar";
+  ENV_REQUIRE(params && state && ctl && out && sp, "null argument");
+  ENV_REQUIRE(ctl->noise_mode == 1 || ctl->noise_mode == 2,
+              "noise_mode 0 (recorded noise rows) cannot cover a sampled reset; Philox noise only (mode 1 or 2)");
+  ENV_REQUIRE(state->robot_params == nullptr, "per-robot parameters take the composed calls (the sweep layout)");
+  ENV_REQUIRE(launch == nullptr || launch->max_groups == 0,
+              "a workgroup cap (launch->max_groups) splits the step into launches; the push needs all groups in one");
+  ENV_REQUIRE(launch == nullptr || launch->layout != 2, "layout 2 (the sweep) has no pushing step");
+  ENV_REQUIRE(sp->capacity > 0 && sp->capacity >= static_cast<int64_t>(state->n_envs) * state->max_robots,
+              "sp->capacity: a ring smaller than one step's rows");
+  ENV_REQUIRE(ctl->env_mask == nullptr, "ctl->env_mask cannot be combined with the push (every group arrives)");
+  ENV_REQUIRE(ctl->do_dynamics && ctl->trainer_deactivate && out->env_done != nullptr,
+              "the pushing step needs ctl->do_dynamics, ctl->trainer_deactivate and out->env_done");
+  ENV_REQUIRE(sp->action_dim == 1 || sp->action_dim == 2, "sp->action_dim must be 1 or 2");
+  ENV_REQUIRE(sp->cfg.num_robots >= 0 && sp->cfg.num_robots <= kResetMaxR && state->max_robots <= kResetMaxR,
+              "sp->cfg.num_robots / max_robots beyond the reset sampler's 32");
+  ENV_REQUIRE(sp->cfg.num_obs >= 0 && sp->cfg.num_obs <= kResetMaxO && state->max_obs <= kResetMaxO,
+              "sp->cfg.num_obs / max_obs beyond the reset sampler's 32");
+  ENV_REQUIRE(sp->cfg.num_cores >= 0 && sp->cfg.num_cores <= kMaxCores && state->max_cores <= kMaxCores,
+              "sp->cfg.num_cores / max_cores beyond the reset sampler's 16");
+  ENV_REQUIRE(sp->cfg.width > 4.0 && sp->cfg.height > 4.0, "sp->cfg map too small");
+  if (int rc = env_checks(who, false, false, params, state, actions, nullptr, ctl, out, nullptr, kOpenLoop, nullptr,
+                          launch))
+    return rc;
+  ENV_REQUIRE(sp->obs_prev && sp->ring && sp->ring_state && sp->work && sp->counter_inc && sp->acting,
+              "null sp array (obs_prev, ring, ring_state, work, counter_inc, acting)");
+  ENV_REQUIRE(reinterpret_cast<uintptr_t>(sp->obs_prev) % 16 == 0 && reinterpret_cast<uintptr_t>(out->obs) % 16 == 0 &&
+                  reinterpret_cast<uintptr_t>(sp->ring) % 16 == 0 && reinterpret_cast<uintptr_t>(sp->acting) % 16 == 0,
+              "sp->obs_prev, out->obs, sp->ring and sp->acting must be 16-byte aligned");
+  if (state->n_envs == 0) return 0;
+  EnvPlan P;
+  if (int rc = env_plan(who, state, ctl, launch, false, true, &P)) return rc;
+  P.smem = P.ar_off + step_push_lds(P.pl.blk, P.pl.epb, state->max_robots);
+  ENV_REQUIRE(P.fused && P.smem <= 150 * 1024, "the pair layout's LDS does not fit");
+  return launch_groups(who, P, StepPushArgs{PairsArgs{*params, *state, *ctl, *out, actions, nullptr, P.pl.epb, 0}, *sp, P.ar_off},
+                       as_stream(stream));
+}
+
+extern "C" int64_t asvrl_step_push_struct_size(void) { return sizeof(AsvStepPush); }
 
 template <class Pol>
 static int rollout_fallback(const char* who, const AsvParams* params, const AsvEnvState* state, const AsvStepCtl* ctl,
diff --git a/distributional_rl_decision_and_control_amd/device_env.py b/distributional_rl_decision_and_control_amd/device_env.py
--- a/distributional_rl_decision_and_control_amd/device_env.py
+++ b/distributional_rl_decision_and_control_amd/device_env.py
@@ -272,6 +272,52 @@
                                                 _abi.stream_ptr(stream))
         _abi.check(rc, "asvrl_env_reset_observe")
 
+    def acting_rows(self, acting=None):
+        E, R = self.n_envs, self.max_robots
+        if acting is None:
+            acting = torch.zeros((2, _abi.acting_stride(E)), dtype=torch.uint8, device=self.device)
+        placed = torch.arange(R, device=self.device)[None, :] < self.n_robots[:, None]
+        live = (self.rflags.view(E, R) & _abi.FLAG_DEACTIVATED) == 0
+        acting[:, :E] = (placed & live).sum(1).to(torch.uint8)
+        return acting
+
+    def step_push_ar(self, actions, obs_prev, replay, cfg, acting, counter_inc, *, action_dim=2, snap=None,
+                     is_continuous=True, seed=0, counter=0, counter_dev=None, reset_counter=0, obs_counter=0, gamma=0.0,
+                     obs=None, obj_cnt=None, fast_noise=False, launch=None, stream=None, L=None):
+        NT = self.n_envs * self.max_robots
+        assert actions.dtype == torch.float64 and actions.is_contiguous() and tuple(actions.shape) == (NT, 2)
+        assert obs_prev.dtype == torch.float32 and obs_prev.is_contiguous() and tuple(obs_prev.shape) == (NT, OBS_DIM)
+        assert acting.dtype == torch.uint8 and acting.is_contiguous() and \
+            tuple(acting.shape) == (2, _abi.acting_stride(self.n_envs))
+        assert counter_inc.dtype == torch.int64 and counter_inc.numel() >= 1
+        ctl = _abi.AsvStepCtl()
+        ctl.is_continuous = int(bool(is_continuous))
+        ctl.do_dynamics = 1
+        ctl.trainer_deactivate = 1
+        ctl.noise_mode = 2 if fast_noise else 1
+        ctl.seed = int(seed) & 0xFFFFFFFFFFFFFFFF
+        ctl.counter = int(counter) & 0xFFFFFFFFFFFFFFFF
+        ctl.counter_dev = counter_dev.data_ptr() if counter_dev is not None else None
+        ctl.gamma = float(gamma)
+        sp = _abi.AsvStepPush()
+        sp.cfg = cfg
+        sp.reset_counter = int(reset_counter) & 0xFFFFFFFFFFFFFFFF
+        sp.obs_counter = int(obs_counter) & 0xFFFFFFFFFFFFFFFF
+        sp.obs_prev = obs_prev.data_ptr()
+        sp.ring, sp.capacity, sp.ring_state = replay.ring.data_ptr(), replay.capacity, replay.state.data_ptr()
+        sp.work = replay.work(NT).data_ptr()
+        sp.snap = snap.data_ptr() if snap is not None else None
+        sp.counter_inc = counter_inc.data_ptr()
+        sp.acting = acting.data_ptr()
+        sp.action_dim = int(action_dim)
+        st = self.state_struct()
+        out = self.out_struct(obs, obj_cnt, with_env_done=True)
+        ln = C.byref(_abi.AsvEnvLaunch(*(int(v) for v in launch))) if launch is not None else None
+        L = L if L is not None else _abi.lib()
+        rc = L.asvrl_env_step_push_ar(C.byref(self.params), C.byref(st), _abi.ptr(actions), C.byref(ctl), C.byref(out),
+                                      C.byref(sp), ln, _abi.stream_ptr(stream))
+        _abi.check(rc, "asvrl_env_step_push_ar", L)
+
 
 def policy_options(who, pack, cvar, deterministic):
     cvar = float(cvar)
diff --git a/distributional_rl_decision_and_control_amd/learn_ops.py b/distributional_rl_decision_and_control_amd/learn_ops.py
--- a/distributional_rl_decision_and_control_amd/learn_ops.py
+++ b/distributional_rl_decision_and_control_amd/learn_ops.py
@@ -72,11 +72,15 @@
         self._work_w = None
         self._n_host = 0
 
+    def work(self, n):
+        if self._work is None or self._work.numel() < (n + 255) // 256 + 1:
+            self._work = torch.zeros((n + 255) // 256 + 1, dtype=torch.int32, device=self.device)
+        return self._work
+
     def push(self, obs_prev, obs_next, obj_cnt_next, actions, reward, done, stream=None, snap=None,
              counter_inc=None):
         n = obs_prev.shape[0]
-        if self._work is None or self._work.numel() < (n + 255) // 256 + 1:
-            self._work = torch.zeros((n + 255) // 256 + 1, dtype=torch.int32, device=self.device)
+        self.work(n)
         if actions.dim() == 1:
             adim, ald = 1, 1
         else:
diff --git a/distributional_rl_decision_and_control_amd/vec_env.py b/distributional_rl_decision_and_control_amd/vec_env.py
--- a/distributional_rl_decision_and_control_amd/vec_env.py
+++ b/distributional_rl_decision_and_control_amd/vec_env.py
@@ -29,6 +29,8 @@
         self.cnt = [torch.full((NT,), -1, dtype=torch.int8, device=self.device) for _ in range(2)]
         self.counter = torch.zeros(1, dtype=torch.int64, device=self.device)
         self.total_timesteps = 0
+        self._acting = None
+        self._acting_ok = False
 
     swap = False
     _p = 0
@@ -61,16 +63,31 @@
 
     def reset(self):
         b = self.batch
+        self._acting_ok = False
         b.reset(self.cfg, None, seed=self.seed, counter=0x40000000, counter_dev=self.counter)
         b.step(None, do_dynamics=False, seed=self.seed, counter=0x80000000, counter_dev=self.counter,
                fast_noise=True, obs=self.obs_cur, obj_cnt=self.cnt_cur)
         return self.obs_cur
 
     def step(self, actions):
+        self._acting_ok = False
         self.batch.step(actions, is_continuous=self.is_continuous, trainer_deactivate=True, seed=self.seed,
                         counter=0, counter_dev=self.counter, gamma=self.gamma, obs=self.obs_next,
                         obj_cnt=self.cnt_next, fast_noise=True,
                         launch=self._launch())
+
+    def can_step_push_reset(self):
+        return bool(self.fused_reset) and self.batch.robot_params is None and self.max_groups <= 0
+
+    def step_push_reset(self, actions, replay, action_dim=2, snap=None):
+        b = self.batch
+        if not self._acting_ok:
+            self._acting = b.acting_rows(self._acting)
+        b.step_push_ar(actions, self.obs_cur, replay, self.cfg, self._acting, self.counter, action_dim=action_dim,
+                       snap=snap, is_continuous=self.is_continuous, seed=self.seed, counter=0, counter_dev=self.counter,
+                       reset_counter=0x40000000, obs_counter=0x80000000, gamma=self.gamma, obs=self.obs_next,
+                       obj_cnt=self.cnt_next, fast_noise=True)
+        self._acting_ok = True
 
     def _auto_reset(self, auto_reset, open_loop):
         if not auto_reset:
@@ -83,6 +100,7 @@
 
     def rollout(self, actions, hold_done=True, keep=("reward", "done", "info"), auto_reset=False, count=True):
         ar = self._auto_reset(auto_reset, True)
+        self._acting_ok = False
         rec = self.batch.rollout(actions, keep=keep, hold_done=hold_done and ar is None,
                                  is_continuous=self.is_continuous,
                                  trainer_deactivate=True, seed=self.seed, counter=0, counter_dev=self.counter,
@@ -101,6 +119,7 @@
         elif not self.is_continuous:
             raise ValueError("policy_rollout: the Actor drives continuous-action envs")
         ar = self._auto_reset(auto_reset, False)
+        self._acting_ok = False
         rec = self.batch.policy_rollout(pack, K, self.obs_cur, keep=keep, hold_done=hold_done and ar is None,
                                         step_dev=self.counter,
                                         eps=eps, policy_seed=policy_seed, trainer_deactivate=True, seed=self.seed,
@@ -117,6 +136,7 @@
     def auto_reset(self, counted=False, events=None):
         b = self.batch
         d = 1 if counted else 0
+        self._acting_ok = False
         if events is not None:
             events[0].record()
         if self.fused_reset and b.robot_params is None and self.max_groups <= 0:
@@ -140,6 +160,7 @@
             self.obs[0].copy_(self.obs[1])
             self.cnt[0].copy_(self.cnt[1])
         if not counted:
+            self._acting_ok = False
             self.counter += 1
 
     def advance_host(self):
diff --git a/distributional_rl_decision_and_control_amd/vec_trainer.py b/distributional_rl_decision_and_control_amd/vec_trainer.py
--- a/distributional_rl_decision_and_control_amd/vec_trainer.py
+++ b/distributional_rl_decision_and_control_amd/vec_trainer.py
@@ -198,12 +198,29 @@
                          env.batch.reward, env.batch.done, snap=snap, counter_inc=env.counter)
         return True
 
+    fused_step = True
+
+    def _fused_step(self):
+        return self.fused_step and self.per is None and self._paa_arg is not True and self.env.can_step_push_reset()
+
+    def _step_push_reset(self, snap=None, after_push=None):
+        env = self.env
+        if self._fused_step():
+            env.step_push_reset(self.actions, self.replay, self.action_dim, snap=snap)
+            if after_push is not None:
+                after_push()
+            env.advance_device(True)
+            return
+        env.step(self.actions)
+        counted = self._push(snap)
+        if after_push is not None:
+            after_push()
+        env.auto_reset(counted)
+        env.advance_device(counted)
+
     def rollout(self, snap=None):
         self.act()
-        self.env.step(self.actions)
-        counted = self._push(snap)
-        self.env.auto_reset(counted)
-        self.env.advance_device(counted)
+        self._step_push_reset(snap)
 
     def _collect_buffers(self, K):
         bufs = getattr(self, "_collect_bufs", None)
@@ -302,11 +319,7 @@
         with torch.cuda.stream(s_roll):
             self.act()
             ev_act.record(s_roll)
-            env = self.env
-            env.step(self.actions)
-            counted = self._push()
-            env.auto_reset(counted)
-            env.advance_device(counted)
+            self._step_push_reset()
         out = self.learn(state=self.ring_snap, guard=self.E * self.R, actor_wait=ev_act)
         main.wait_stream(s_roll)
         return out
@@ -368,7 +381,8 @@
         ev_env = [torch.cuda.Event() for _ in range(U)]
         ev_actor = [torch.cuda.Event() for _ in range(U)]
         self._chain_events = (ev_act, ev_snap, ev_learn, ev_env, ev_actor)
-        tae, paa = self.target_after_env, self.push_after_actor
+        fused = self._fused_step()
+        tae, paa = self.target_after_env, self.push_after_actor and not fused
         s_roll.wait_stream(main)
         out = None
 
@@ -384,11 +398,16 @@
                     s_roll.wait_event(ev_learn[k - 1])
                 self.act()
                 ev_act[k].record(s_roll)
-                self.env.step(self.actions)
-                if tae:
-                    ev_env[k].record(s_roll)
-                if not paa:
-                    push_reset(k)
+                if fused:
+                    self._step_push_reset(self.ring_snap2[k % 2], lambda: ev_snap[k].record(s_roll))
+                    if tae:
+                        ev_env[k].record(s_roll)
+                else:
+                    self.env.step(self.actions)
+                    if tae:
+                        ev_env[k].record(s_roll)
+                    if not paa:
+                        push_reset(k)
             if k > 0:
                 main.wait_event(ev_snap[k - 1])
             out = self.learn(state=self.ring_snap2[(k - 1) % 2], guard=self.E * self.R, actor_wait=ev_act[k],
diff --git a/include/asvrl.h b/include/asvrl.h
--- a/include/asvrl.h
+++ b/include/asvrl.h
@@ -723,6 +723,28 @@
                              int64_t* counter_inc, int64_t counter_by, void* stream);
 
 
+#define ASVRL_ACTING_STRIDE(n_envs) (((n_envs) + 15) & ~15)
+typedef struct AsvStepPush {
+  AsvResetCfg cfg;
+  uint64_t reset_counter, obs_counter;
+  const float* obs_prev;
+  float* ring;
+  int64_t capacity;
+  int64_t* ring_state;
+  int32_t* work;
+  int64_t* snap;
+  int64_t* counter_inc;
+  uint8_t* acting;
+  int32_t action_dim;
+  int32_t _pad0;
+} AsvStepPush;
+
+int asvrl_env_step_push_ar(const AsvParams* params, const AsvEnvState* state, const double* actions,
+                           const AsvStepCtl* ctl, const AsvStepOut* out, const AsvStepPush* sp,
+                           const AsvEnvLaunch* launch , void* stream);
+int64_t asvrl_step_push_struct_size(void);
+
+
 typedef struct AsvEvalMetrics {
   int32_t n_steps;
   int32_t n_envs;
```

Result: slower. 14.93 million env-steps/s (-10.0%).
